# Multi-resolution-diffusion-recommender/SDRM

Measured on AMD Instinct MI355X. Metric: denoising-steps/sec (train+sample) on ML-1M latents, higher is better.
Workload: dtype f32; 1 GPU; ML-1M/MLP shaped synthetic latents (C3/C4); latent=340, width=340, hidden_layers=1, global_batch=8192, n_sample=5429, step_mix=15 train : 78 sample per job cycle, rng=philox4x32-10 on device, sampler_row_chains=2, parallelism=user-sharded dp1, collectives=none

## Files before the change

### include/sdrm_hip_debug.h

```cpp
#ifndef SDRM_HIP_DEBUG_H
#define SDRM_HIP_DEBUG_H

#include "sdrm_hip.h"

#ifdef __cplusplus
extern "C" {
#endif

int sdrm_debug_device_check(const char* gcn_arch, int compute_units);

enum { SDRM_TILE_AUTO = -1, SDRM_TILE_COUNT = 5 };

int sdrm_debug_set_tile(sdrm_engine* e, int cfg);
int sdrm_debug_set_nt32_rows(sdrm_engine* e, int max_rows, int max_rows_train);
int sdrm_debug_set_skinny(sdrm_engine* e, int on);
int sdrm_debug_set_rowchain(sdrm_engine* e, int mode);
int sdrm_debug_set_rows48(sdrm_engine* e, int mode);
int sdrm_debug_set_rows48_split(sdrm_engine* e, int mode);
int sdrm_debug_rows48_split_available(const sdrm_engine* e);
int sdrm_debug_set_rows48_share(sdrm_engine* e, int on);
int sdrm_debug_set_sample_persist(sdrm_engine* e, int mode);
int sdrm_debug_split_skew(sdrm_engine* e, unsigned skew);
int sdrm_debug_set_wgrad_strips(sdrm_engine* e, int on);
int sdrm_debug_set_dgrad_rows(sdrm_engine* e, int mode);
int sdrm_debug_rowchain_available(const sdrm_engine* e);
int sdrm_debug_set_fused_reverse(sdrm_engine* e, int mode);
int sdrm_debug_set_chains(sdrm_engine* e, int chains);
int sdrm_debug_chains(const sdrm_engine* e);

int sdrm_debug_set_gradient_buckets(sdrm_engine* e, int buckets);

int sdrm_debug_philox_draws(sdrm_engine* e, uint64_t seed, uint32_t purpose, uint32_t step, int64_t row0, int rows, int quads,
                            float* normals, uint8_t* lowbits, void* stream);

void* sdrm_debug_comm_handle(const sdrm_engine* e);

int sdrm_debug_plan_wgrad(int rows, int n_out, int k_in, int* slices, int* rows_per_slice);

int sdrm_debug_gemm(int variant, int cfg, const float* A, const float* B, float* C, int M, int N, int K, void* stream);
int sdrm_debug_gemm_time(int variant, int cfg, int M, int N, int K, int reps, float* us_out, void* stream);

#ifdef __cplusplus
}
#endif
#endif
```

### sdrm_amd/_lib.py

```python
from __future__ import annotations

import ctypes as C
import os

from . import _build

_LIB = None

c_void_p, c_int, c_int64, c_uint64, c_float = C.c_void_p, C.c_int, C.c_int64, C.c_uint64, C.c_float


class TrainRandoms(C.Structure):
    _fields_ = [("noise", c_void_p), ("t", c_void_p), ("keep", c_void_p)]


class VaeDecoder(C.Structure):
    _fields_ = [("w1", c_void_p), ("b1", c_void_p), ("w2", c_void_p), ("b2", c_void_p), ("latent", c_int), ("hidden", c_int),
                ("n_items", c_int)]


SIGNATURES = {
    "sdrm_create": (c_int, [c_int, c_int, c_int, c_int, c_int, c_int, C.POINTER(c_void_p)]),
    "sdrm_destroy": (c_int, [c_void_p]),
    "sdrm_last_error": (C.c_char_p, [c_void_p]),
    "sdrm_param_count": (c_int64, [c_void_p]),
    "sdrm_set_schedule": (c_int, [c_void_p, c_float, c_float]),
    "sdrm_get_schedule": (c_int, [c_void_p, c_void_p, c_void_p, c_void_p]),
    "sdrm_set_params": (c_int, [c_void_p, c_void_p, c_void_p]),
    "sdrm_get_params": (c_int, [c_void_p, c_void_p, c_void_p]),
    "sdrm_params_ptr": (c_void_p, [c_void_p]),
    "sdrm_get_grads": (c_int, [c_void_p, c_void_p, c_void_p]),
    "sdrm_get_adam_state": (c_int, [c_void_p, c_void_p, c_void_p, C.POINTER(c_int64), c_void_p]),
    "sdrm_set_adam_state": (c_int, [c_void_p, c_void_p, c_void_p, c_int64, c_void_p]),
    "sdrm_adam_reset": (c_int, [c_void_p, c_void_p]),
    "sdrm_train_forward": (c_int, [c_void_p, c_void_p, c_int, c_int64, c_int, C.POINTER(TrainRandoms), c_uint64,
                                   c_uint64, c_float, c_void_p, c_void_p]),
    "sdrm_train_backward": (c_int, [c_void_p, c_void_p, c_void_p, c_void_p, c_void_p]),
    "sdrm_train_backward_begin": (c_int, [c_void_p, c_void_p, c_void_p, c_void_p, c_void_p]),
    "sdrm_train_backward_finish": (c_int, [c_void_p, c_void_p, c_void_p]),
    "sdrm_grad_buckets": (c_int, [c_void_p, C.POINTER(c_int64), C.POINTER(c_int64), C.POINTER(c_int64), C.POINTER(c_int64)]),
    "sdrm_adam_step": (c_int, [c_void_p, c_void_p, c_float, c_void_p]),
    "sdrm_train_step": (c_int, [c_void_p, c_void_p, c_int, c_float, c_int, C.POINTER(TrainRandoms), c_uint64, c_uint64,
                                c_float, c_void_p, c_void_p]),
    "sdrm_comm_unique_id": (c_int, [c_void_p]),
    "sdrm_comm_available": (c_int, []),
    "sdrm_comm_init_rank": (c_int, [c_void_p, c_int, c_int, c_void_p]),
    "sdrm_allreduce_init": (c_int, [c_void_p, c_void_p, c_void_p]),
    "sdrm_comm_info": (c_int, [c_void_p, C.POINTER(c_int), C.POINTER(c_int)]),
    "sdrm_comm_destroy": (c_int, [c_void_p]),
    "sdrm_train_step_sharded": (c_int, [c_void_p, c_void_p, c_int, c_int64, c_float, c_int, C.POINTER(TrainRandoms), c_uint64,
                                        c_uint64, c_float, c_void_p, c_void_p]),
    "sdrm_get_train_outputs": (c_int, [c_void_p, c_void_p, c_void_p]),
    "sdrm_forward": (c_int, [c_void_p, c_void_p, c_void_p, c_int, c_int, c_void_p, c_uint64, c_uint64, c_int64,
                             c_void_p, c_void_p]),
    "sdrm_sample": (c_int, [c_void_p, c_int, c_float, c_int, c_int, c_void_p, c_void_p, c_void_p, c_void_p, c_uint64,
                            c_uint64, c_int64, c_void_p, c_void_p, c_void_p]),
    "sdrm_sample_begin": (c_int, [c_void_p, c_int, c_float, c_int, c_int, c_void_p, c_void_p, c_void_p, c_void_p,
                                  c_uint64, c_uint64, c_int64, c_void_p, c_void_p]),
    "sdrm_sample_steps": (c_int, [c_void_p, c_int, c_void_p]),
    "sdrm_sample_remaining": (c_int, [c_void_p]),
    "sdrm_sample_end": (c_int, [c_void_p, c_void_p, c_void_p]),
    "sdrm_reverse_step": (c_int, [c_void_p, c_void_p, c_int, c_int, c_void_p, c_void_p, c_void_p]),
    "sdrm_perturb_input": (c_int, [c_void_p, c_void_p, c_void_p, c_void_p, c_int, c_void_p, c_void_p]),
    "sdrm_get_preacts": (c_int, [c_void_p, c_int, c_void_p, c_void_p]),
    "sdrm_profile_begin": (c_int, [c_void_p, c_int]),
    "sdrm_debug_set_gradient_buckets": (c_int, [c_void_p, c_int]),
    "sdrm_profile_only": (c_int, [c_void_p, c_int]),
    "sdrm_profile_end": (c_int, [c_void_p, c_void_p]),
    "sdrm_profile_classes": (c_int, []),
    "sdrm_profile_name": (C.c_char_p, [c_int]),
    "sdrm_profile_get": (c_int, [c_void_p, c_int, C.POINTER(C.c_double), C.POINTER(c_int64), C.POINTER(C.c_double)]),
    "sdrm_launch_count": (c_int64, [c_void_p]),
    "sdrm_build_info": (C.c_char_p, []),
    "sdrm_csr_rows_to_dense": (c_int, [c_void_p, c_void_p, c_void_p, c_void_p, c_int64, c_void_p, c_int64, c_int, c_int, c_void_p, c_void_p]),
    "sdrm_feed_status": (c_int, [c_void_p, c_void_p]),
    "sdrm_vae_decode": (c_int, [c_void_p, C.POINTER(VaeDecoder), c_void_p, c_int, c_void_p, c_void_p]),
    "sdrm_equal_sparsity": (c_int, [c_void_p, c_void_p, c_int64, C.c_double, c_void_p, c_void_p, c_void_p]),
    "sdrm_rank_metrics": (c_int, [c_void_p, c_void_p, c_int, c_int, c_void_p, c_void_p, c_void_p, c_void_p, c_void_p, c_int,
                                  c_void_p, c_void_p, c_void_p, c_void_p, c_void_p]),
    "sdrm_source_hash": (C.c_char_p, []),
    "sdrm_debug_philox_draws": (c_int, [c_void_p, c_uint64, C.c_uint32, C.c_uint32, c_int64, c_int, c_int, c_void_p, c_void_p, c_void_p]),
    "sdrm_debug_device_check": (c_int, [C.c_char_p, c_int]),
    "sdrm_debug_set_tile": (c_int, [c_void_p, c_int]),
    "sdrm_debug_set_nt32_rows": (c_int, [c_void_p, c_int, c_int]),
    "sdrm_debug_set_chains": (c_int, [c_void_p, c_int]),
    "sdrm_debug_chains": (c_int, [c_void_p]),
    "sdrm_debug_set_fused_reverse": (c_int, [c_void_p, c_int]),
    "sdrm_debug_set_skinny": (c_int, [c_void_p, c_int]),
    "sdrm_debug_set_rowchain": (c_int, [c_void_p, c_int]),
    "sdrm_debug_set_rows48": (c_int, [c_void_p, c_int]),
    "sdrm_debug_set_rows48_split": (c_int, [c_void_p, c_int]),
    "sdrm_debug_rows48_split_available": (c_int, [c_void_p]),
    "sdrm_debug_split_skew": (c_int, [c_void_p, C.c_uint32]),
    "sdrm_debug_set_sample_persist": (c_int, [c_void_p, c_int]),
    "sdrm_debug_set_rows48_share": (c_int, [c_void_p, c_int]),
    "sdrm_debug_rowchain_available": (c_int, [c_void_p]),
    "sdrm_debug_set_wgrad_strips": (c_int, [c_void_p, c_int]),
    "sdrm_debug_set_dgrad_rows": (c_int, [c_void_p, c_int]),
    "sdrm_debug_comm_handle": (c_void_p, [c_void_p]),
    "sdrm_debug_plan_wgrad": (c_int, [c_int, c_int, c_int, C.POINTER(c_int), C.POINTER(c_int)]),
    "sdrm_debug_gemm_time": (c_int, [c_int, c_int, c_int, c_int, c_int, c_int, C.POINTER(c_float), c_void_p]),
    "sdrm_debug_gemm": (c_int, [c_int, c_int, c_void_p, c_void_p, c_void_p, c_int, c_int, c_int, c_void_p]),
}

RNG_EXPLICIT, RNG_PHILOX = 0, 1
STATUS = {0: "SDRM_OK", -1: "SDRM_ERR_ARG", -2: "SDRM_ERR_SHAPE", -3: "SDRM_ERR_HIP", -4: "SDRM_ERR_STATE",
          -5: "SDRM_ERR_NOMEM", -6: "SDRM_ERR_RCCL", -7: "SDRM_ERR_DEVICE"}


def lib_path() -> str:
    return _build.LIB_PATH


def load(build_if_missing: bool = True):
    global _LIB
    if _LIB is not None:
        return _LIB
    try:
        import torch
    except ImportError:
        pass
    path = lib_path()
    override = os.environ.get("SDRM_LIB")
    if override:
        lib = C.CDLL(os.path.abspath(override))
        missing = [name for name in SIGNATURES if not hasattr(lib, name)]
        if missing:
            raise RuntimeError(f"SDRM_LIB={override}: not this ABI, missing {', '.join(missing[:6])}{' ...' if len(missing) > 6 else ''}")
        for name, (res, args) in SIGNATURES.items():
            fn = getattr(lib, name)
            fn.restype, fn.argtypes = res, args
        import sys
        print(f"sdrm_amd: SDRM_LIB override {override} (sources {lib.sdrm_source_hash().decode()[:16]}; in-tree sources "
              f"{_build.source_hash()[:16]})", file=sys.stderr)
        _LIB = lib
        return lib
    if _build.is_stale():
        if not build_if_missing:
            what = "is missing" if not os.path.exists(path) else "was built from different sources than csrc/ + include/"
            raise RuntimeError(f"{path} {what}: run `python -c 'import __graft_entry__ as g; g.build()'`")
        _build.build_library()
    try:
        lib = C.CDLL(path)
    except OSError as exc:
        raise RuntimeError(f"cannot load {path}: {exc}") from exc
    for name, (res, args) in SIGNATURES.items():
        fn = getattr(lib, name)
        fn.restype, fn.argtypes = res, args
    got, want = lib.sdrm_source_hash().decode(), _build.source_hash()
    if got != want:
        raise RuntimeError(f"{path} carries source hash {got[:16]}, the sources hash to {want[:16]}")
    _LIB = lib
    return lib
```

### sdrm_amd/csrc/sdrm_hip.hip

```cpp
#include <hip/hip_runtime.h>

#include <algorithm>
#include <cmath>
#include <cstdio>
#include <cstdlib>
#include <cstring>
#include <mutex>
#include <set>
#include <string>
#include <vector>

#include "../../include/sdrm_hip.h"
#include "../../include/sdrm_hip_debug.h"
#include "decode.h"
#include "elementwise.h"
#include "exchange.h"
#include "feed.h"
#include "gemm.h"
#include "rank.h"
#include "rowchain.h"
#include "rows48.h"
#include "sample_persist.h"
#include "select.h"
#include "skinny.h"
#include "skinny_step.h"
#include "skinny_fwd4.h"
#include "tail.h"
#include "dgrad_rows.h"
#include "wgrad2.h"

using namespace sdrm;

namespace {

constexpr int BM = 64;
constexpr int S_MAX = 64;
constexpr int LOSS_BLOCKS = 256;

inline int round_up(int v, int m) { return (v + m - 1) / m * m; }

}

struct Tuning {
  int force_cfg = -1;
  int chains = -1;
  int detach = 1;
  int hold_early = 1;
  int fuse_rev = 1;
  int skinny = 1;
  int nt32_max_rows = 4096;
  int nt32_max_rows_train = 8192;
  int wgrad_blocks = 2816;
  int wgrad_round = 1280;
  int wgrad_slices = 0;
  int ar_buckets = 1;
  int dgrad_rows = 1;
  int strips = 1;
  int rows48 = 1;
  int rows48_share = 7;
  int smp_persist = 1;
  int split = 1;
  int rowchain = 1;
};

struct sdrm_engine {
  int L, W, T, H, max_rows, device;
  Tuning tune;
  int LP, WP, TP, K0, MPmax;
  int64_t P;
  int64_t off_we, off_be, off_w0, off_b0, off_a0, off_wh, off_bh, off_ah, off_wo, off_bo;
  float *p = nullptr, *m = nullptr, *v = nullptr, *g = nullptr;
  float *W0c = nullptr, *b0c = nullptr, *Whc = nullptr, *bhc = nullptr, *Woc = nullptr, *boc = nullptr;
  float *WhcT = nullptr, *WocT = nullptr;
  float *WhfT = nullptr, *WofT = nullptr;
  float *W0f = nullptr, *Whf = nullptr, *Wof = nullptr;
  bool cur_grouped = false;
  bool cur_sk = false;
  bool cur_g16 = false;
  int cur_rows = 0;
  bool cur_skip_pre = false;
  int cur_parts = 1;
  unsigned *xcntF = nullptr, *xcntC = nullptr;
  unsigned *xabort_host = nullptr, *xabort_dev = nullptr;
  uint32_t xepochF = 0, xepochC = 0;
  int xgeoF = 0, xgeoC = 0;
  bool xcd_ok = false;
  unsigned* xcntS = nullptr;
  uint32_t xphaseS = 0;
  unsigned xskew = 0;
  int cur_sk_np = 0;
  bool tables_fresh = false;
  float* act = nullptr;
  bool cur_act = false;
  int ones_col = -1;
  bool bwd_strips = false;
  float *temb = nullptr, *tembP = nullptr, *B0tab = nullptr;
  float *sched = nullptr;
  float *Us = nullptr;
  float *smp_pre = nullptr, *smp_Y = nullptr;
  float *U = nullptr, *pre = nullptr, *Y = nullptr, *dY = nullptr, *dA = nullptr, *X = nullptr;
  float *slab0 = nullptr, *slabH = nullptr, *slabO = nullptr, *db0s = nullptr, *dbHs = nullptr, *dbOs = nullptr;
  float *alpha_part = nullptr;
  int alpha_part_stride = 0;
  double *loss_part = nullptr, *sums = nullptr;
  float *WeP = nullptr, *W0eP = nullptr;
  int TPe = 0;
  float *Mred = nullptr, *snap = nullptr;
  int *tdev = nullptr;
  int64_t *Tj_dev = nullptr;
  int *rowid_dev = nullptr;
  const float* grad_src = nullptr;
  float *rev_dev = nullptr;
  SelectState* sel = nullptr;
  float* one_dev = nullptr;
  unsigned* feed_flag = nullptr;
  std::vector<int> smp_nact, smp_perm;
  std::vector<int64_t> smp_tj_sorted, smp_tj_orig;
  std::vector<float> h_beta, h_alpha, h_alphabar;
  int64_t adam_t = 0;
  int cur_B = 0, cur_MP = 0;
  const float* cur_x0 = nullptr;
  bool fwd_done = false;
  int last_S = 1, last_dgrad_blocks = 0;
  bool bwd_begun = false;
  bool fold_sums = false;
  int bwd_S0 = 1, bwd_SH = 1, bwd_SO = 1, bwd_kc0 = 0, bwd_kcH = 0, bwd_kcO = 0, bwd_dgrad_blocks = 0;
  int bwd_hidden_apps = 0;
  int bwd_cfg_w = 0;
  float* dec_buf[6] = {nullptr, nullptr, nullptr, nullptr, nullptr, nullptr};
  size_t dec_cap[6] = {0, 0, 0, 0, 0, 0};
  Exchange xch;
  mutable int64_t n_launches = 0;
  float* smp_w = nullptr;
  size_t smp_off[7] = {0, 0, 0, 0, 0, 0, 0};
  struct SampleStateT {
    bool active; int n, MP, multires, mode, i_next; float nd; const float* z; const uint8_t* keep;
    uint64_t seed, call_id; int64_t row0;
    const float* xT; bool skinny; bool skinny_launched; int i_start;
  } smp = {false, 0, 0, 0, 0, 0, 1.f, nullptr, nullptr, 0, 0, 0, nullptr, false, false, 0};
  hipStream_t aux[3] = {nullptr, nullptr, nullptr};
  hipEvent_t ev_fork = nullptr, ev_join[3] = {nullptr, nullptr, nullptr};
  hipEvent_t ev_hold = nullptr;
  int n_chains = 1, chain_chunk = 0;
  int n_aux = 0;
  bool detach_armed = false;
  bool hold_needed = false;
  bool chains_pending = false;
  bool hold_recorded = false;
  bool train_since_sample = false;
  bool prof_on = false;
  int prof_cap = 0;
  int prof_only = -1;
  std::vector<hipEvent_t> prof_ev;
  std::vector<int> prof_cls;
  std::vector<double> prof_flops;
  double prof_ms[16] = {0};
  double prof_fl[16] = {0};
  int64_t prof_n[16] = {0};
  std::string err;
};

typedef sdrm_engine::SampleStateT SampleState;

enum ProfClass { PC_FWD_L0 = 0, PC_FWD_HIDDEN, PC_FWD_OUT, PC_DGRAD, PC_WGRAD, PC_WGRAD_L0, PC_SMP_L0, PC_SMP_HIDDEN,
                 PC_SMP_OUT, PC_ROW_FWD, PC_WGRAD_STRIPS, PC_DGRAD_ROWS, PC_SMP_PERSIST, PC_COUNT };
static const char* kProfNames[PC_COUNT] = {
    "train: gemm_kernel<0,0,0,0,9> fwd layer0 (row-table bias)", "train: gemm_kernel<0,0,1,0,0> fwd hidden (prelu-in, bias)",
    "train: gemm_kernel<0,0,1,0,1> fwd out (prelu-in, tanh)",
    "train: gemm_kernel<0,0,0,0,3> dgrad (prelu' epilogue)",
    "train: gemm_batch_kernel<1,1,0,1,4> wgrad of all layers in one launch (prelu-in, split-K slabs)",
    "train: gemm_kernel<1,1,0,0,4> wgrad layer0 (split-K slabs)",
    "sample: gemm_kernel<0,0,0,0,10> fwd layer0 (bias table, prelu epilogue)", "sample: gemm_kernel<0,0,0,0,10> fwd hidden (bias, prelu epilogue)",
    "sample: gemm_kernel<0,0,0,0,1> fwd out (tanh)",
    "train: k_row_fwd row-owned forward (staging + all layers + loss partial sums, one work-group per CU)",
    "train: k_wgrad_strips weight gradients of all layers (strip-owned split-K, one work-group per CU)",
    "train: k_dgrad_chain / k_dgrad_rows input gradients (row-owned, prelu' epilogue, one work-group per CU; the chain: loss seeds + every layer in one launch)",
    "sample: k_sample_persist reverse steps without kernel boundaries (all layers + reverse update per step, row tiles synchronised through one XCD's L2)"};

namespace {

#define HIP_TRY(e, call)                                                                   \
  do {                                                                                     \
    hipError_t _st = (call);                                                               \
    if (_st != hipSuccess) {                                                               \
      (e)->err = std::string(#call) + ": " + hipGetErrorString(_st);                       \
      return SDRM_ERR_HIP;                                                                 \
    }                                                                                      \
  } while (0)

#define SDRM_LAUNCH(eng, ...)                      \
  do {                                             \
    if (eng) ++(eng)->n_launches;                  \
    hipLaunchKernelGGL(__VA_ARGS__);               \
  } while (0)

int fail(sdrm_engine* e, int code, const std::string& msg) {
  if (e) e->err = msg;
  return code;
}

constexpr size_t SLACK = 4096;

constexpr int LDS_MAX_BYTES = 160 * 1024;
hipError_t allow_full_lds(const void* kernel) {
  static std::mutex mu;
  static std::set<const void*> done;
  std::lock_guard<std::mutex> lock(mu);
  if (done.count(kernel)) return hipSuccess;
  const hipError_t st = hipFuncSetAttribute(kernel, hipFuncAttributeMaxDynamicSharedMemorySize, LDS_MAX_BYTES);
  if (st == hipSuccess) done.insert(kernel);
  return st;
}

template <typename Tp>
hipError_t dalloc(Tp** p, size_t n) {
  hipError_t st = hipMalloc((void**)p, (n + SLACK) * sizeof(Tp));
  if (st != hipSuccess) return st;
  return hipMemset(*p, 0, (n + SLACK) * sizeof(Tp));
}

float* pre_buf(sdrm_engine* e, int k) { return e->pre + (size_t)k * e->MPmax * e->WP; }
float* smp_buf(sdrm_engine* e, int k) { return e->smp_pre + (size_t)k * e->MPmax * e->WP; }
float* dpre_buf(sdrm_engine* e, int k) { return e->dA + (size_t)k * e->MPmax * e->WP; }
const float* slope_ptr(sdrm_engine* e, int layer) { return e->p + (layer == 0 ? e->off_a0 : e->off_ah); }

struct Prof { sdrm_engine* e; int cls; double flops; };

#ifdef SDRM_STAMPS
unsigned long long* g_wgrad_stamps = nullptr;
int g_wgrad_stamps_cap = 0, g_wgrad_stamps_n = 0;
int g_stamp_class = -1;
#endif


typedef TileCfg<64, 64, 2, 2, 4, 16> Cfg0;
typedef TileCfg<64, 64, 2, 2, 4, 32, 32, 1> Cfg1;
typedef TileCfg<64, 128, 2, 2, 4, 16> Cfg2;
typedef TileCfg<128, 128, 2, 2, 4, 16> Cfg3;
typedef TileCfg<32, 32, 2, 2, 4, 32, 16> Cfg4;
constexpr int N_TILE_CFGS = 5;
const int kCfgBM[N_TILE_CFGS] = {64, 64, 64, 128, 32};
const int kCfgBN[N_TILE_CFGS] = {64, 64, 128, 128, 32};
constexpr int FUSE_REV_MAX_ROWS = 4096;

int pick_cfg(const Tuning& t) { return (t.force_cfg >= 0 && t.force_cfg < N_TILE_CFGS) ? t.force_cfg : 0; }

int choose_cfg(const Tuning& t, int M, int nt32_rows) {
  if (t.force_cfg >= 0 && t.force_cfg < N_TILE_CFGS) return t.force_cfg;
  return M <= nt32_rows ? 4 : 0;
}

int max_gemm_blocks(int M, int N) {
  int best = 0;
  for (int c = 0; c < N_TILE_CFGS; ++c) {
    const int b = ((M + kCfgBM[c] - 1) / kCfgBM[c]) * ((N + kCfgBN[c] - 1) / kCfgBN[c]);
    if (b > best) best = b;
  }
  return best;
}

template <class Cfg, int LA, int LB, int XA, int XB, int EPI>
hipError_t launch_gemm_cfg(GemmArgs& a, int M, int N, int splits, hipStream_t st, Prof pr) {
  const int tiles_m = (M + Cfg::BM - 1) / Cfg::BM, tiles_n = (N + Cfg::BN - 1) / Cfg::BN;
  if (!gemm_set_grid(a, tiles_m, tiles_n, splits)) return hipErrorInvalidValue;
  {
    const uint64_t kc = (uint64_t)std::max(a.kchunk, 1) + 64;
    const uint64_t spanA = LA == LD_KCONTIG ? ((uint64_t)Cfg::BM * a.lda + kc) : kc * a.lda;
    const uint64_t spanB = LB == LD_KCONTIG ? ((uint64_t)Cfg::BN * a.ldb + kc) : kc * a.ldb;
    if (spanA * 4 >= (1ull << 32) || spanB * 4 >= (1ull << 32)) return hipErrorInvalidValue;
  }
  dim3 grid(EPI == EPI_SLAB ? (unsigned)(a.nblocks * splits) : (unsigned)a.nblocks, 1, 1);
  sdrm_engine* e = pr.e;
  const bool rec = e && e->prof_on && (int)e->prof_cls.size() < e->prof_cap && (e->prof_only < 0 || e->prof_only == pr.cls);
  size_t slot = 0;
  if (rec) {
    slot = e->prof_cls.size();
    e->prof_cls.push_back(pr.cls);
    e->prof_flops.push_back(pr.flops);
    hipError_t st0 = hipEventRecord(e->prof_ev[2 * slot], st);
    if (st0 != hipSuccess) return st0;
  }
#ifdef SDRM_STAMPS
  if (g_wgrad_stamps && g_stamp_class >= 0 && pr.e && pr.cls == g_stamp_class && (int)grid.x <= g_wgrad_stamps_cap) {
    a.stamps = g_wgrad_stamps;
    g_wgrad_stamps_n = (int)grid.x;
  }
#endif
  SDRM_LAUNCH(pr.e, (gemm_kernel<Cfg, LA, LB, XA, XB, EPI>), grid, dim3(NTHREADS), 0, st, a);
  hipError_t rc = hipGetLastError();
  if (rec && rc == hipSuccess) rc = hipEventRecord(e->prof_ev[2 * slot + 1], st);
  return rc;
}

template <int LA, int LB, int XA, int XB, int EPI>
hipError_t launch_gemm(GemmArgs& a, int M, int N, int splits, hipStream_t st, Prof pr, int cfg) {
  switch (cfg) {
    case 1: return launch_gemm_cfg<Cfg1, LA, LB, XA, XB, EPI>(a, M, N, splits, st, pr);
    case 2: return launch_gemm_cfg<Cfg2, LA, LB, XA, XB, EPI>(a, M, N, splits, st, pr);
    case 3: return launch_gemm_cfg<Cfg3, LA, LB, XA, XB, EPI>(a, M, N, splits, st, pr);
    case 4: return launch_gemm_cfg<Cfg4, LA, LB, XA, XB, EPI>(a, M, N, splits, st, pr);
    default: return launch_gemm_cfg<Cfg0, LA, LB, XA, XB, EPI>(a, M, N, splits, st, pr);
  }
}

template <int XA, int EPI>
hipError_t gemm_forward(GemmArgs a, const float* A, int lda, const float* Wc, int ldw, int M, int N, int K,
                        hipStream_t st, Prof pr, int cfg) {
  a.A = A; a.lda = lda; a.limA = M;
  a.B = Wc; a.ldb = ldw; a.limB = N;
  a.K = K; a.kchunk = K;
  return launch_gemm<LD_KCONTIG, LD_KCONTIG, XA, XF_NONE, EPI>(a, M, N, 1, st, pr, cfg);
}

hipError_t gemm_dgrad(sdrm_engine* e, const float* dC, int lddc, const float* WT, int ldwt, int M, int Nout, int Kin,
                      float* out, const float* aux, const float* slopeE, float* partial, hipStream_t st, double flops,
                      int cfg) {
  GemmArgs a{};
  a.A = dC; a.lda = lddc; a.limA = M;
  a.B = WT; a.ldb = ldwt; a.limB = Kin;
  a.C = out; a.ldc = e->WP;
  a.K = Nout; a.kchunk = Nout;
  a.aux = aux; a.ldaux = e->WP; a.slopeE = slopeE; a.slope_partial = partial;
  return launch_gemm<LD_KCONTIG, LD_KCONTIG, XF_NONE, XF_NONE, EPI_DPRELU>(a, M, Kin, 1, st, Prof{e, PC_DGRAD, flops}, cfg);
}

template <int XB>
hipError_t gemm_wgrad(const float* dC, int lddc, int Nout, const float* Act, int ldact, int Kin, const float* slopeB,
                      int Mrows, int S, int kchunk, float* slab, float* dbias, hipStream_t st, Prof pr, int cfg) {
  GemmArgs a{};
  a.A = dC; a.lda = lddc; a.limA = Nout;
  a.B = Act; a.ldb = ldact; a.limB = Kin;
  a.C = slab; a.ldc = Kin;
  a.K = Mrows; a.kchunk = kchunk;
  a.slopeB = slopeB;
  a.slab_stride = (size_t)Nout * Kin;
  a.dbias = dbias; a.dbias_stride = Nout;
  return launch_gemm<LD_MCONTIG, LD_MCONTIG, XF_NONE, XB, EPI_SLAB>(a, Nout, Kin, S, st, pr, cfg);
}

struct WgradSpec {
  const float* dC; int lddc, Nout; const float* Act; int ldact, Kin; const float* slopeB; int S, kchunk; float* slab; float* dbias;
};

hipError_t launch_wgrad_batch(sdrm_engine* e, const WgradSpec* w, int n, int Mrows, hipStream_t st, Prof pr, bool plain_b = false) {
  GemmBatch b{};
  b.n = n;
  int grid = 0;
  for (int k = 0; k < n; ++k) {
    GemmArgs& a = b.p[k];
    a.A = w[k].dC; a.lda = w[k].lddc; a.limA = w[k].Nout;
    a.B = w[k].Act; a.ldb = w[k].ldact; a.limB = w[k].Kin;
    a.C = w[k].slab; a.ldc = w[k].Kin;
    a.K = Mrows; a.kchunk = w[k].kchunk;
    a.slopeB = w[k].slopeB;
    a.slab_stride = (size_t)w[k].Nout * w[k].Kin;
    a.dbias = w[k].dbias; a.dbias_stride = w[k].Nout;
    const int tiles_m = (w[k].Nout + Cfg0::BM - 1) / Cfg0::BM, tiles_n = (w[k].Kin + Cfg0::BN - 1) / Cfg0::BN;
    if (!gemm_set_grid(a, tiles_m, tiles_n, w[k].S)) return hipErrorInvalidValue;
    if (((uint64_t)std::max(a.kchunk, 1) + 64) * (uint64_t)std::max(a.lda, a.ldb) * 4 >= (1ull << 32)) return hipErrorInvalidValue;
    b.start[k] = grid;
#ifdef SDRM_STAMPS
    a.stamps = (g_wgrad_stamps && g_stamp_class < 0) ? g_wgrad_stamps + 8 * (size_t)grid : nullptr;
#endif
    grid += round_up(a.nblocks * w[k].S, 8);
  }
  b.start[n] = grid;
#ifdef SDRM_STAMPS
  if (grid > g_wgrad_stamps_cap) for (int k = 0; k < n; ++k) b.p[k].stamps = nullptr;
  else if (g_stamp_class < 0) g_wgrad_stamps_n = grid;
#endif
  const bool rec = e->prof_on && (int)e->prof_cls.size() < e->prof_cap && (e->prof_only < 0 || e->prof_only == pr.cls);
  size_t slot = 0;
  if (rec) {
    slot = e->prof_cls.size();
    e->prof_cls.push_back(pr.cls);
    e->prof_flops.push_back(pr.flops);
    hipError_t st0 = hipEventRecord(e->prof_ev[2 * slot], st);
    if (st0 != hipSuccess) return st0;
  }
  if (plain_b)
    SDRM_LAUNCH(e, (gemm_batch_kernel<Cfg0, LD_MCONTIG, LD_MCONTIG, XF_NONE, XF_NONE, EPI_SLAB>), dim3((unsigned)grid),
                       dim3(NTHREADS), 0, st, b);
  else
    SDRM_LAUNCH(e, (gemm_batch_kernel<Cfg0, LD_MCONTIG, LD_MCONTIG, XF_NONE, XF_PRELU, EPI_SLAB>), dim3((unsigned)grid),
                       dim3(NTHREADS), 0, st, b);
  hipError_t rc = hipGetLastError();
  if (rec && rc == hipSuccess) rc = hipEventRecord(e->prof_ev[2 * slot + 1], st);
  return rc;
}

void pick_splits(const Tuning& tn, int Mrows, int tiles_total, int& S, int& kchunk) {
  const int BK = 32;
  int max_by_rows = Mrows / (4 * BK);
  if (max_by_rows < 1) max_by_rows = 1;
  const int tiles = tiles_total < 1 ? 1 : tiles_total;
  S = tn.wgrad_round / tiles;
  if (S < 8 || round_up((Mrows + S - 1) / S, BK) > 1024) S = tn.wgrad_blocks / tiles;
  if (S < 1) S = 1;
  if (tn.wgrad_slices > 0) S = tn.wgrad_slices;
  if (S > S_MAX) S = S_MAX;
  if (S > max_by_rows) S = max_by_rows;
  kchunk = round_up((Mrows + S - 1) / S, BK);
  S = (Mrows + kchunk - 1) / kchunk;
}

int wgrad_tiles(const Tuning& tn, int Nout, int Kin) {
  const int c = pick_cfg(tn);
  return ((Nout + kCfgBM[c] - 1) / kCfgBM[c]) * ((Kin + kCfgBN[c] - 1) / kCfgBN[c]);
}

void build_jobs(sdrm_engine* e, JobTable& tab) {
  const int L = e->L, W = e->W, T = e->T, H = e->H;
  int n = 0;
  auto add = [&](int64_t off, int rows, int cols, int flat_ld, int ncols, float* dst, int dst_ld, float* dstT = nullptr, int dstT_ld = 0) -> Job& {
    Job& j = tab.j[n++];
    j.flat_off = off; j.rows = rows; j.cols = cols; j.flat_ld = flat_ld; j.ncols = ncols;
    j.dst = dst; j.dst_ld = dst_ld; j.dstT = dstT; j.dstT_ld = dstT_ld; j.dst2 = nullptr; j.dst2_ld = 0;
    j.dstF = nullptr; j.dstFT = nullptr; j.fnct = e->WP / 16; j.fklast = -1; j.fklastT = -1;
    return j;
  };
  add(e->off_we, T, T, T, e->WeP ? T : 0, e->WeP, e->TPe);
  add(e->off_be, 1, T, T, 0, nullptr, 0);
  {
    Job& j = add(e->off_w0, W, L + T, L + T, L, e->W0c, e->K0);
    j.dstF = e->W0f; j.fklast = rc_light_klast(L, e->LP);
    j.dst2 = e->W0eP; j.dst2_ld = e->TPe;
  }
  add(e->off_b0, 1, W, W, W, e->b0c, 0);
  add(e->off_a0, 1, 1, 1, 1, nullptr, 0);
  if (H >= 1) {
    Job& j = add(e->off_wh, W, W, W, W, e->Whc, e->WP, e->WhcT, e->WP);
    j.dstF = e->Whf; j.dstFT = e->WhfT; j.fklast = j.fklastT = rc_light_klast(W, e->WP);
    add(e->off_bh, 1, W, W, W, e->bhc, 0);
    add(e->off_ah, 1, 1, 1, 1, nullptr, 0);
  }
  {
    Job& j = add(e->off_wo, L, W, W, W, e->Woc, e->WP, e->WocT, e->LP);
    j.dstF = e->Wof; j.dstFT = e->WofT; j.fklast = rc_light_klast(W, e->WP); j.fklastT = rc_light_klast(L, e->LP);
  }
  add(e->off_bo, 1, L, L, L, e->boc, 0);
  tab.n = n;
}

void adam_scalars(const sdrm_engine* e, float lr, float& step_size, float& bc2_sqrt) {
  const double k = (double)e->adam_t;
  const double bc1 = 1.0 - std::pow(0.9, k), bc2 = 1.0 - std::pow(0.999, k);
  step_size = (float)((double)lr / bc1);
  bc2_sqrt = (float)std::sqrt(bc2);
}

int launch_adam(sdrm_engine* e, const float* grad, float lr, int update, hipStream_t st) {
  JobTable tab;
  build_jobs(e, tab);
  AdamArgs a{};
  a.p = e->p; a.m = e->m; a.v = e->v; a.g = grad ? grad : e->g;
  a.b1 = 0.9f; a.b2 = 0.999f; a.eps = 1e-8f; a.wd = 1e-4f; a.update = update;
  if (update) adam_scalars(e, lr, a.step_size, a.bc2_sqrt);
  int64_t biggest = 0;
  for (int k = 0; k < tab.n; ++k) biggest = std::max<int64_t>(biggest, (int64_t)tab.j[k].rows * tab.j[k].cols);
  const int gx = (int)std::min<int64_t>(1024, std::max<int64_t>(1, (biggest + 511) / 512));
  dim3 grid(gx, tab.n);
  SDRM_LAUNCH(e, k_adam, grid, dim3(256), 0, st, tab, a);
  HIP_TRY(e, hipGetLastError());
  e->tables_fresh = false;
  return SDRM_OK;
}

bool use_strips(const sdrm_engine* e) {
  return (e->cur_grouped || e->cur_g16) && e->cur_act && e->ones_col >= 0 && e->tune.strips > 0 && e->H + 2 <= WG2_MAX_PROBLEMS && e->WP >= 128 && e->WP <= 352;
}

template <int NT>
int launch_wgrad_strips_nt(sdrm_engine* e, const Wg2Args& a, double flops, hipStream_t st) {
  const bool rec = e->prof_on && (int)e->prof_cls.size() < e->prof_cap && (e->prof_only < 0 || e->prof_only == PC_WGRAD_STRIPS);
  size_t slot = 0;
  if (rec) {
    slot = e->prof_cls.size();
    e->prof_cls.push_back(PC_WGRAD_STRIPS);
    e->prof_flops.push_back(flops);
    HIP_TRY(e, hipEventRecord(e->prof_ev[2 * slot], st));
  }
  SDRM_LAUNCH(e, (k_wgrad_strips<NT>), dim3((unsigned)(a.units * a.slices)), dim3(NTHREADS), 0, st, a);
  HIP_TRY(e, hipGetLastError());
  if (rec) HIP_TRY(e, hipEventRecord(e->prof_ev[2 * slot + 1], st));
  return SDRM_OK;
}

int launch_wgrad_strips(sdrm_engine* e, int MP, double flops, hipStream_t st) {
  const int H = e->H;
  Wg2Args a{};
  int ktiles[WG2_MAX_PROBLEMS], n = 0;
  auto problem = [&](const float* A, int lda, const float* B, int ldb, float* slab, int kin, size_t slab_rows) {
    a.p[n].A = A; a.p[n].lda = lda; a.p[n].B = B; a.p[n].ldb = ldb; a.p[n].slab = slab; a.p[n].ldc = kin;
    a.p[n].slab_stride = slab_rows * (size_t)kin;
    ktiles[n++] = kin / 32;
  };
  auto actk = [&](int k) { return e->act + (size_t)k * e->MPmax * e->WP; };
  problem(dpre_buf(e, 0), e->WP, e->U, e->K0, e->slab0, e->K0, (size_t)e->WP);
  problem(e->dY, e->LP, actk(H), e->WP, e->slabO, e->WP, (size_t)e->LP);
  const int units = [&] { int t = e->K0 / 32 + (H + 1) * (e->WP / 32); return (t + 3) / 4; }();
  int S = 256 / units;
  if (S < 1) S = 1;
  if (S > S_MAX) S = S_MAX;
  MP = e->cur_rows;
  const int kchunk = round_up((MP + S - 1) / S, WG2_BK);
  const int slices = (MP + kchunk - 1) / kchunk;
  for (int k = H; k >= 1; --k)
    problem(dpre_buf(e, k), e->WP, actk(k - 1), e->WP, e->slabH + (size_t)(k - 1) * slices * e->WP * e->WP, e->WP, (size_t)e->WP);
  if (wg2_plan(ktiles, n, a) != units) return fail(e, SDRM_ERR_SHAPE, "strip-owned weight gradients: plan does not fit");
  a.slices = slices; a.rows = MP; a.kchunk = kchunk;
  e->bwd_S0 = e->bwd_SH = e->bwd_SO = slices;
  e->bwd_strips = true;
  switch (e->WP / 32) {
    case 4: return launch_wgrad_strips_nt<4>(e, a, flops, st);
    case 5: return launch_wgrad_strips_nt<5>(e, a, flops, st);
    case 6: return launch_wgrad_strips_nt<6>(e, a, flops, st);
    case 7: return launch_wgrad_strips_nt<7>(e, a, flops, st);
    case 8: return launch_wgrad_strips_nt<8>(e, a, flops, st);
    case 9: return launch_wgrad_strips_nt<9>(e, a, flops, st);
    case 10: return launch_wgrad_strips_nt<10>(e, a, flops, st);
    default: return launch_wgrad_strips_nt<11>(e, a, flops, st);
  }
}

EmbTabArgs emb_args(sdrm_engine* e) {
  EmbTabArgs a{};
  a.temb = e->temb; a.We = e->p + e->off_we; a.be = e->p + e->off_be; a.W0 = e->p + e->off_w0; a.b0 = e->p + e->off_b0;
  a.W0c = e->W0c; a.B0tab = e->B0tab;
  a.L = e->L; a.W = e->W; a.T = e->T; a.LP = e->LP; a.WP = e->WP; a.K0 = e->K0;
  a.ones_col = e->ones_col;
  return a;
}

int emb_tables(sdrm_engine* e, hipStream_t st, const float* warm = nullptr, size_t warm_floats = 0) {
  EmbTabArgs a = emb_args(e);
  a.warm = warm; a.warm_lines = warm ? (unsigned)std::min<size_t>(warm_floats / 32, 1u << 24) : 0u;
  SDRM_LAUNCH(e, k_emb_tables, dim3(e->T + 1), dim3(1024), 2 * e->T * sizeof(float), st, a);
  HIP_TRY(e, hipGetLastError());
  e->tables_fresh = true;
  return SDRM_OK;
}
int ensure_tables(sdrm_engine* e, hipStream_t st) { return e->tables_fresh ? SDRM_OK : emb_tables(e, st); }

bool skinny_net(const sdrm_engine* e) { return e->tune.skinny && e->LP <= 64 && e->WP <= 64; }

bool row_dgrads_follow(const sdrm_engine* e, bool g16, int MP) {
  if (!e->WhfT || e->tune.dgrad_rows <= 0 || e->LP != e->WP || e->WP < 128 || e->WP > 352) return false;
  return g16 ? e->H + 1 <= DR_MAX_LAYERS : MP % RC_ROWS == 0;
}
bool use_dgrad_rows(const sdrm_engine* e, int MP) {
  return e->cur_grouped && e->WhfT && e->tune.dgrad_rows > 0 && e->LP == e->WP && MP % RC_ROWS == 0 && e->WP >= 128 && e->WP <= 352;
}

template <int CT>
int launch_dgrad_rows_ct(sdrm_engine* e, const DgradRowsArgs& a, int G, double flops, hipStream_t st) {
  const bool rec = e->prof_on && (int)e->prof_cls.size() < e->prof_cap && (e->prof_only < 0 || e->prof_only == PC_DGRAD_ROWS);
  size_t slot = 0;
  if (rec) {
    slot = e->prof_cls.size();
    e->prof_cls.push_back(PC_DGRAD_ROWS);
    e->prof_flops.push_back(flops);
    HIP_TRY(e, hipEventRecord(e->prof_ev[2 * slot], st));
  }
  if (rc_light_klast(e->W, e->WP) >= 0) SDRM_LAUNCH(e, (k_dgrad_rows<CT, true>), dim3((unsigned)G), dim3(NTHREADS), 0, st, a);
  else SDRM_LAUNCH(e, (k_dgrad_rows<CT, false>), dim3((unsigned)G), dim3(NTHREADS), 0, st, a);
  HIP_TRY(e, hipGetLastError());
  if (rec) HIP_TRY(e, hipEventRecord(e->prof_ev[2 * slot + 1], st));
  return SDRM_OK;
}

DgradRowsArgs dgrad_rows_args(const sdrm_engine* e, const float* G, const float* WfT, const float* pre, const float* slope, float* out,
                              float* partial) {
  DgradRowsArgs a{};
  a.G = G; a.ldg = e->WP; a.WfT = WfT; a.pre = pre; a.ldp = e->WP; a.slope = slope; a.out = out; a.ldo = e->WP; a.slope_part = partial;
  a.act = e->act ? e->act + (pre - e->pre) : nullptr; a.from_act = (e->cur_act && e->cur_skip_pre && a.act) ? 1 : 0;
  return a;
}

int launch_dgrad_rows(sdrm_engine* e, const float* G, const float* WfT, const float* pre, const float* slope, float* out, float* partial,
                      int MP, double flops, hipStream_t st) {
  const DgradRowsArgs a = dgrad_rows_args(e, G, WfT, pre, slope, out, partial);
  const int Gn = MP / RC_ROWS;
  switch (e->WP / 32) {
    case 4: return launch_dgrad_rows_ct<4>(e, a, Gn, flops, st);
    case 5: return launch_dgrad_rows_ct<5>(e, a, Gn, flops, st);
    case 6: return launch_dgrad_rows_ct<6>(e, a, Gn, flops, st);
    case 7: return launch_dgrad_rows_ct<7>(e, a, Gn, flops, st);
    case 8: return launch_dgrad_rows_ct<8>(e, a, Gn, flops, st);
    case 9: return launch_dgrad_rows_ct<9>(e, a, Gn, flops, st);
    case 10: return launch_dgrad_rows_ct<10>(e, a, Gn, flops, st);
    default: return launch_dgrad_rows_ct<11>(e, a, Gn, flops, st);
  }
}

template <int CT>
int launch_dgrad_chain_ct(sdrm_engine* e, const DgradChainArgs& a, int G, double flops, hipStream_t st) {
  const bool rec = e->prof_on && (int)e->prof_cls.size() < e->prof_cap && (e->prof_only < 0 || e->prof_only == PC_DGRAD_ROWS);
  size_t slot = 0;
  if (rec) {
    slot = e->prof_cls.size();
    e->prof_cls.push_back(PC_DGRAD_ROWS);
    e->prof_flops.push_back(flops);
    HIP_TRY(e, hipEventRecord(e->prof_ev[2 * slot], st));
  }
  if (rc_light_klast(e->W, e->WP) >= 0) SDRM_LAUNCH(e, (k_dgrad_chain<CT, true>), dim3((unsigned)G), dim3(NTHREADS), 0, st, a);
  else SDRM_LAUNCH(e, (k_dgrad_chain<CT, false>), dim3((unsigned)G), dim3(NTHREADS), 0, st, a);
  HIP_TRY(e, hipGetLastError());
  if (rec) HIP_TRY(e, hipEventRecord(e->prof_ev[2 * slot + 1], st));
  return SDRM_OK;
}

int launch_dgrad_chain(sdrm_engine* e, const DgradChainArgs& a, int MP, double flops, hipStream_t st) {
  const int Gn = MP / RC_ROWS;
  switch (e->WP / 32) {
    case 4: return launch_dgrad_chain_ct<4>(e, a, Gn, flops, st);
    case 5: return launch_dgrad_chain_ct<5>(e, a, Gn, flops, st);
    case 6: return launch_dgrad_chain_ct<6>(e, a, Gn, flops, st);
    case 7: return launch_dgrad_chain_ct<7>(e, a, Gn, flops, st);
    case 8: return launch_dgrad_chain_ct<8>(e, a, Gn, flops, st);
    case 9: return launch_dgrad_chain_ct<9>(e, a, Gn, flops, st);
    case 10: return launch_dgrad_chain_ct<10>(e, a, Gn, flops, st);
    default: return launch_dgrad_chain_ct<11>(e, a, Gn, flops, st);
  }
}

bool use_rowchain(const sdrm_engine* e, int B) {
  if (!e->W0f || e->tune.rowchain <= 0 || e->tune.force_cfg >= 0) return false;
  if (e->tune.rowchain >= 2) return true;
  const int G = (B + RC_USERS - 1) / RC_USERS;
  const int rounds = (G + 255) / 256;
  return rounds == 1 ? G >= 154 : G * 6 >= rounds * 256 * 5;
}

inline unsigned xabort_read(const sdrm_engine* e) { return e->xabort_host ? *(volatile const unsigned*)e->xabort_host : 0u; }

int rows48_grid(int groups, int parts) { return parts == 1 ? groups : 8 * parts * ((groups + 7) / 8); }
int rows48_parts(const sdrm_engine* e, int B) {
  if (!e->W0f || e->tune.rows48 <= 0 || e->tune.force_cfg >= 0 || e->tune.rowchain >= 2) return 0;
  const int G = (B + R48_USERS - 1) / R48_USERS;
  const bool can_split = e->xcd_ok && e->tune.split > 0 && e->xabort_host && xabort_read(e) == 0u;
  if (can_split && e->tune.split >= 2) {
    const int parts = e->tune.split >= 4 ? 4 : 2;
    if (rows48_grid(G, parts) <= 256) return parts;
    if (parts == 4 && rows48_grid(G, 2) <= 256) return 2;
  }
  if (e->tune.rows48 >= 2) return 1;
  const bool beside_sampler = e->smp.active && (e->detach_armed || (e->chains_pending && e->n_aux == e->n_chains));
  if (can_split && e->tune.split == 1 && G > 80 && rows48_grid(G, 2) <= 256) return beside_sampler ? 0 : 2;
  return (G >= 160 && G <= 256) ? 1 : 0;
}

int split_sync(sdrm_engine* e, bool chain, int groups, int parts, int phases, hipStream_t st, unsigned** cnt, unsigned* base) {
  unsigned*& c = chain ? e->xcntC : e->xcntF;
  uint32_t& epoch = chain ? e->xepochC : e->xepochF;
  int& geo = chain ? e->xgeoC : e->xgeoF;
  const int now = (parts << 16) | groups | (phases << 24);
  if (geo != now || epoch >= 0x7fffffffu / (uint32_t)(phases * parts + 1)) {
    HIP_TRY(e, hipMemsetAsync(c, 0, (size_t)256 * 32 * sizeof(unsigned), st));
    epoch = 0; geo = now;
  }
  *cnt = c;
  *base = epoch * (uint32_t)(phases * parts) + e->xskew;
  if (e->xskew) { e->xskew = 0; geo = 0; }
  ++epoch;
  return SDRM_OK;
}

int split_status(sdrm_engine* e) {
  if (xabort_read(e) == 0u) return SDRM_OK;
  *(volatile unsigned*)e->xabort_host = 0u;
  e->xgeoF = e->xgeoC = 0;
  e->tune.split = 0;
  e->fwd_done = false;
  return fail(e, SDRM_ERR_HIP, "a column-split row-group launch (csrc/rows48.h) timed out waiting for a work-group of its group: the results of "
                               "that train step are invalid; the path is switched off for this handle");
}

template <int CT, int PARTS>
int launch_rows48_forward_ctp(sdrm_engine* e, const RowChainArgs& a, int grid, hipStream_t st) {
  if constexpr (PARTS == 1 && CT % 2 == 1) {
    if (e->tune.rows48_share & 1) {
      if (a.light) SDRM_LAUNCH(e, (k_rows48_fwd<CT, true, 1, true>), dim3((unsigned)grid), dim3(NTHREADS), 0, st, a);
      else SDRM_LAUNCH(e, (k_rows48_fwd<CT, false, 1, true>), dim3((unsigned)grid), dim3(NTHREADS), 0, st, a);
      return SDRM_OK;
    }
  }
  if (a.light) SDRM_LAUNCH(e, (k_rows48_fwd<CT, true, PARTS>), dim3((unsigned)grid), dim3(NTHREADS), 0, st, a);
  else SDRM_LAUNCH(e, (k_rows48_fwd<CT, false, PARTS>), dim3((unsigned)grid), dim3(NTHREADS), 0, st, a);
  return SDRM_OK;
}

template <int CT>
int launch_rows48_forward_ct(sdrm_engine* e, RowChainArgs& a, int G, int parts, hipStream_t st) {
  const double flops = 2.0 * 3 * a.B * ((double)e->W * e->L + (double)e->H * e->W * e->W + (double)e->L * e->W);
  const bool rec = e->prof_on && (int)e->prof_cls.size() < e->prof_cap && (e->prof_only < 0 || e->prof_only == PC_ROW_FWD);
  size_t slot = 0;
  if (parts > 1) {
    if (int rc = split_sync(e, false, G, parts, e->H + 1, st, &a.xcnt, &a.xbase)) return rc;
    a.xabort = e->xabort_dev; a.ngroups = G;
  }
  if (rec) {
    slot = e->prof_cls.size();
    e->prof_cls.push_back(PC_ROW_FWD);
    e->prof_flops.push_back(flops);
    HIP_TRY(e, hipEventRecord(e->prof_ev[2 * slot], st));
  }
  const int grid = rows48_grid(G, parts);
  if (parts == 4) launch_rows48_forward_ctp<CT, 4>(e, a, grid, st);
  else if (parts == 2) launch_rows48_forward_ctp<CT, 2>(e, a, grid, st);
  else launch_rows48_forward_ctp<CT, 1>(e, a, grid, st);
  HIP_TRY(e, hipGetLastError());
  if (rec) HIP_TRY(e, hipEventRecord(e->prof_ev[2 * slot + 1], st));
  return SDRM_OK;
}

template <int CT, int PARTS>
int launch_rows48_chain_ctp(sdrm_engine* e, const DgradChain48Args& a, int grid, hipStream_t st) {
  if constexpr (PARTS == 1 && CT % 2 == 1) {
    if (e->tune.rows48_share & 2) {
      if (rc_light_klast(e->W, e->WP) >= 0) SDRM_LAUNCH(e, (k_rows48_dgrad_chain<CT, true, 1, true>), dim3((unsigned)grid), dim3(NTHREADS), 0, st, a);
      else SDRM_LAUNCH(e, (k_rows48_dgrad_chain<CT, false, 1, true>), dim3((unsigned)grid), dim3(NTHREADS), 0, st, a);
      return SDRM_OK;
    }
  }
  if (rc_light_klast(e->W, e->WP) >= 0) SDRM_LAUNCH(e, (k_rows48_dgrad_chain<CT, true, PARTS>), dim3((unsigned)grid), dim3(NTHREADS), 0, st, a);
  else SDRM_LAUNCH(e, (k_rows48_dgrad_chain<CT, false, PARTS>), dim3((unsigned)grid), dim3(NTHREADS), 0, st, a);
  return SDRM_OK;
}

template <int CT>
int launch_rows48_chain_ct(sdrm_engine* e, DgradChain48Args& a, int G, int parts, double flops, hipStream_t st) {
  const bool rec = e->prof_on && (int)e->prof_cls.size() < e->prof_cap && (e->prof_only < 0 || e->prof_only == PC_DGRAD_ROWS);
  size_t slot = 0;
  if (parts > 1) {
    if (int rc = split_sync(e, true, G, parts, std::max(1, a.c.nlayers - 1), st, &a.xcnt, &a.xbase)) return rc;
    a.xabort = e->xabort_dev; a.ngroups = G;
  }
  if (rec) {
    slot = e->prof_cls.size();
    e->prof_cls.push_back(PC_DGRAD_ROWS);
    e->prof_flops.push_back(flops);
    HIP_TRY(e, hipEventRecord(e->prof_ev[2 * slot], st));
  }
  const int grid = rows48_grid(G, parts);
  if (parts == 4) launch_rows48_chain_ctp<CT, 4>(e, a, grid, st);
  else if (parts == 2) launch_rows48_chain_ctp<CT, 2>(e, a, grid, st);
  else launch_rows48_chain_ctp<CT, 1>(e, a, grid, st);
  HIP_TRY(e, hipGetLastError());
  if (rec) HIP_TRY(e, hipEventRecord(e->prof_ev[2 * slot + 1], st));
  return SDRM_OK;
}

int launch_rows48_chain(sdrm_engine* e, DgradChain48Args& a, int G, int parts, double flops, hipStream_t st) {
  switch (e->WP / 32) {
    case 4: return launch_rows48_chain_ct<4>(e, a, G, parts, flops, st);
    case 5: return launch_rows48_chain_ct<5>(e, a, G, parts, flops, st);
    case 6: return launch_rows48_chain_ct<6>(e, a, G, parts, flops, st);
    case 7: return launch_rows48_chain_ct<7>(e, a, G, parts, flops, st);
    case 8: return launch_rows48_chain_ct<8>(e, a, G, parts, flops, st);
    case 9: return launch_rows48_chain_ct<9>(e, a, G, parts, flops, st);
    case 10: return launch_rows48_chain_ct<10>(e, a, G, parts, flops, st);
    default: return launch_rows48_chain_ct<11>(e, a, G, parts, flops, st);
  }
}

template <int CT>
int launch_row_forward_ct(sdrm_engine* e, const RowChainArgs& a, int G, hipStream_t st) {
  const double flops = 2.0 * 3 * a.B * ((double)e->W * e->L + (double)e->H * e->W * e->W + (double)e->L * e->W);
  const bool rec = e->prof_on && (int)e->prof_cls.size() < e->prof_cap && (e->prof_only < 0 || e->prof_only == PC_ROW_FWD);
  size_t slot = 0;
  if (rec) {
    slot = e->prof_cls.size();
    e->prof_cls.push_back(PC_ROW_FWD);
    e->prof_flops.push_back(flops);
    HIP_TRY(e, hipEventRecord(e->prof_ev[2 * slot], st));
  }
  if (a.light) SDRM_LAUNCH(e, (k_row_fwd<CT, true>), dim3((unsigned)G), dim3(NTHREADS), 0, st, a);
  else SDRM_LAUNCH(e, (k_row_fwd<CT, false>), dim3((unsigned)G), dim3(NTHREADS), 0, st, a);
  HIP_TRY(e, hipGetLastError());
  if (rec) HIP_TRY(e, hipEventRecord(e->prof_ev[2 * slot + 1], st));
  return SDRM_OK;
}

int launch_row_forward(sdrm_engine* e, const float* x0, int B, int64_t row0, int mode, const sdrm_train_randoms* rnd, uint64_t seed,
                       uint64_t step, float nd, int G, hipStream_t st, int rows48_parts_ = 0) {
  const int n = e->T + 1;
  RowChainArgs a{};
  a.x0 = x0;
  if (mode == SDRM_RNG_EXPLICIT) { a.noise = rnd->noise; a.t = rnd->t; a.keep = rnd->keep; }
  a.sqrt_ab = e->sched + 3 * n; a.one_minus_ab = e->sched + 4 * n; a.tembP = e->tembP;
  a.B = B; a.L = e->L; a.T = e->T; a.H = e->H;
  a.mode = mode; a.seed_lo = (uint32_t)seed; a.seed_hi = (uint32_t)(seed >> 32); a.step = (uint32_t)step; a.row0 = row0; a.nd = nd;
  a.W0f = e->W0f; a.Whf = e->Whf; a.Wof = e->Wof; a.bh = e->bhc; a.bo = e->boc; a.B0tab = e->B0tab; a.ldtab = e->WP;
  a.slope0 = slope_ptr(e, 0); a.slopeh = e->H > 0 ? slope_ptr(e, 1) : slope_ptr(e, 0);
  a.U = e->U; a.K0 = e->K0; a.LPs = e->LP; a.tdev = e->tdev; a.ones_col = e->ones_col;
  a.light = rc_light_klast(e->W, e->WP) >= 0 ? 1 : 0;
  a.pre = e->pre; a.pre_stride = (size_t)e->MPmax * e->WP; a.ldp = e->WP; a.Y = e->Y; a.ldy = e->LP;
  a.act = e->act;
  a.loss_part = e->loss_part;
  a.sweep = (e->tune.rows48_share & 4) ? 1 : 0;
  {
    const int MPg = rows48_parts_ > 0 ? round_up(G * R48_ROWS, BM) : round_up(G * RC_ROWS, BM);
    a.skip_pre = row_dgrads_follow(e, rows48_parts_ > 0, MPg) ? 1 : 0;
    e->cur_skip_pre = a.skip_pre != 0;
  }
  if (rows48_parts_ > 0) {
    switch (e->WP / 32) {
      case 4: return launch_rows48_forward_ct<4>(e, a, G, rows48_parts_, st);
      case 5: return launch_rows48_forward_ct<5>(e, a, G, rows48_parts_, st);
      case 6: return launch_rows48_forward_ct<6>(e, a, G, rows48_parts_, st);
      case 7: return launch_rows48_forward_ct<7>(e, a, G, rows48_parts_, st);
      case 8: return launch_rows48_forward_ct<8>(e, a, G, rows48_parts_, st);
      case 9: return launch_rows48_forward_ct<9>(e, a, G, rows48_parts_, st);
      case 10: return launch_rows48_forward_ct<10>(e, a, G, rows48_parts_, st);
      case 11: return launch_rows48_forward_ct<11>(e, a, G, rows48_parts_, st);
      default: return fail(e, SDRM_ERR_SHAPE, "row-owned forward: padded width outside 128..352");
    }
  }
  switch (e->WP / 32) {
    case 4: return launch_row_forward_ct<4>(e, a, G, st);
    case 5: return launch_row_forward_ct<5>(e, a, G, st);
    case 6: return launch_row_forward_ct<6>(e, a, G, st);
    case 7: return launch_row_forward_ct<7>(e, a, G, st);
    case 8: return launch_row_forward_ct<8>(e, a, G, st);
    case 9: return launch_row_forward_ct<9>(e, a, G, st);
    case 10: return launch_row_forward_ct<10>(e, a, G, st);
    case 11: return launch_row_forward_ct<11>(e, a, G, st);
    default: return fail(e, SDRM_ERR_SHAPE, "row-owned forward: padded width outside 128..352");
  }
}

SkStepArgs sk_step_args(sdrm_engine* e, int B) {
  SkStepArgs a{};
  const int n = e->T + 1;
  a.W0c = e->W0c; a.K0 = e->K0; a.Whc = e->Whc; a.Woc = e->Woc; a.bh = e->bhc; a.bo = e->boc;
  a.WhcT = e->WhcT; a.WocT = e->WocT; a.B0tab = e->B0tab;
  a.WeP = e->WeP; a.W0eP = e->W0eP; a.be = e->p + e->off_be; a.b0 = e->b0c; a.TPe = e->TPe; a.intab = e->WeP ? 1 : 0;
  a.slope0 = slope_ptr(e, 0); a.slopeh = e->H > 0 ? slope_ptr(e, 1) : slope_ptr(e, 0);
  a.sqrt_ab = e->sched + 3 * n; a.one_minus_ab = e->sched + 4 * n; a.tembP = e->tembP;
  a.B = B; a.L = e->L; a.W = e->W; a.T = e->T; a.H = e->H; a.G = (B + SK_USERS - 1) / SK_USERS;
  a.LPs = e->LP; a.WPs = e->WP; a.TPs = e->TP;
  a.U = e->U; a.tdev = e->tdev; a.pre = e->pre; a.pre_stride = (size_t)e->MPmax * e->WP; a.Y = e->Y;
  a.loss_part = e->loss_part; a.NP = a.G;
  a.slab0 = e->slab0; a.slabH = e->slabH; a.slabO = e->slabO; a.db0s = e->db0s; a.dbHs = e->dbHs; a.dbOs = e->dbOs;
  a.alpha_part = e->alpha_part; a.alpha_part_stride = e->alpha_part_stride;
  return a;
}

template <int NL, int NW>
int launch_sk_step_nlnw(sdrm_engine* e, const SkStepArgs& ka, int which, int grid, hipStream_t st) {
  typedef SkCfg<NL, NW> C;
  const size_t lds = (which == 0 ? sk_fwd_lds_floats<NL, NW>(ka.intab ? ka.TPe : 0) : sk_bwd_lds_floats<NL, NW>(ka.TPs)) * sizeof(float);
  if (lds > 48 * 1024) HIP_TRY(e, allow_full_lds(which == 0 ? (const void*)k_skinny_fwd<NL, NW> : (const void*)k_skinny_bwd<NL, NW>));
  if (which == 0) SDRM_LAUNCH(e, (k_skinny_fwd<NL, NW>), dim3((unsigned)grid), dim3(C::NTHR), lds, st, ka);
  else SDRM_LAUNCH(e, (k_skinny_bwd<NL, NW>), dim3((unsigned)grid), dim3(C::NTHR), lds, st, ka);
  HIP_TRY(e, hipGetLastError());
  return SDRM_OK;
}

template <int NL, int NW>
int launch_sk_fwd4_nlnw(sdrm_engine* e, const SkStepArgs& ka, hipStream_t st, bool* done) {
  const size_t lds = sk4_fwd_lds_floats<NL, NW>(ka.intab ? ka.TPe : 0) * sizeof(float);
  *done = false;
  if (lds > 160 * 1024) return SDRM_OK;
  if (lds > 48 * 1024) HIP_TRY(e, allow_full_lds((const void*)k_skinny_fwd4<NL, NW>));
  SDRM_LAUNCH(e, (k_skinny_fwd4<NL, NW>), dim3((unsigned)std::min(ka.NP, 8192)), dim3(SK4_THREADS), lds, st, ka);
  HIP_TRY(e, hipGetLastError());
  *done = true;
  return SDRM_OK;
}

int launch_sk_fwd4(sdrm_engine* e, const SkStepArgs& ka, hipStream_t st, bool* done) {
  const int NL = (e->L + 15) / 16, NW = (e->W + 15) / 16;
#define SK4_ROW(nl)                                                           \
  switch (NW) {                                                               \
    case 1: return launch_sk_fwd4_nlnw<nl, 1>(e, ka, st, done);               \
    case 2: return launch_sk_fwd4_nlnw<nl, 2>(e, ka, st, done);               \
    case 3: return launch_sk_fwd4_nlnw<nl, 3>(e, ka, st, done);               \
    default: return launch_sk_fwd4_nlnw<nl, 4>(e, ka, st, done);              \
  }
  switch (NL) {
    case 1: SK4_ROW(1)
    case 2: SK4_ROW(2)
    case 3: SK4_ROW(3)
    default: SK4_ROW(4)
  }
#undef SK4_ROW
}

int launch_sk_step(sdrm_engine* e, const SkStepArgs& ka, int which, int grid, hipStream_t st) {
  const int NL = (e->L + 15) / 16, NW = (e->W + 15) / 16;
#define SK_ROW(nl)                                                                  \
  switch (NW) {                                                                     \
    case 1: return launch_sk_step_nlnw<nl, 1>(e, ka, which, grid, st);              \
    case 2: return launch_sk_step_nlnw<nl, 2>(e, ka, which, grid, st);              \
    case 3: return launch_sk_step_nlnw<nl, 3>(e, ka, which, grid, st);              \
    default: return launch_sk_step_nlnw<nl, 4>(e, ka, which, grid, st);             \
  }
  switch (NL) {
    case 1: SK_ROW(1)
    case 2: SK_ROW(2)
    case 3: SK_ROW(3)
    default: SK_ROW(4)
  }
#undef SK_ROW
}

struct NetView { const float *W0c, *Whc, *Woc, *bhc, *boc, *B0tab, *slope0, *slopeh; };
NetView snapshot_view(const sdrm_engine* e) {
  const float* b = e->smp_w;
  return NetView{b + e->smp_off[0], b + e->smp_off[1], b + e->smp_off[2], b + e->smp_off[3], b + e->smp_off[4], b + e->smp_off[5],
                 b + e->smp_off[6], b + e->smp_off[6] + 1};
}

int hidden_forward(sdrm_engine* e, int MP, int rows, hipStream_t st, int cfg, int r0 = 0, int cls = PC_FWD_HIDDEN,
                   bool post_act = false, const NetView* nv = nullptr) {
  const double fl = 2.0 * rows * (double)e->W * e->W;
  const size_t ro = (size_t)r0 * e->WP;
  for (int k = 1; k <= e->H; ++k) {
    if (post_act) {
      GemmArgs a{};
      a.C = (nv ? smp_buf(e, k) : pre_buf(e, k)) + ro; a.ldc = e->WP; a.bias = nv ? nv->bhc : e->bhc; a.slopeE = nv ? nv->slopeh : slope_ptr(e, k);
      HIP_TRY(e, (gemm_forward<XF_NONE, EPI_BIAS_PRELU>(a, (nv ? smp_buf(e, k - 1) : pre_buf(e, k - 1)) + ro, e->WP, nv ? nv->Whc : e->Whc, e->WP, MP, e->WP, e->WP,
                                                         st, Prof{e, cls, fl}, cfg)));
      continue;
    }
    GemmArgs a{};
    a.C = pre_buf(e, k) + ro; a.ldc = e->WP; a.bias = e->bhc; a.slopeA = slope_ptr(e, k - 1);
    HIP_TRY(e, (gemm_forward<XF_PRELU, EPI_BIAS>(a, pre_buf(e, k - 1) + ro, e->WP, e->Whc, e->WP, MP, e->WP, e->WP, st,
                                                 Prof{e, cls, fl}, cfg)));
  }
  return SDRM_OK;
}

int join_chains(sdrm_engine* e, hipStream_t st) {
  e->bwd_begun = false;
  if (!e->chains_pending) return SDRM_OK;
  for (int c = 0; c < e->n_aux; ++c) {
    HIP_TRY(e, hipEventRecord(e->ev_join[c], e->aux[c]));
    HIP_TRY(e, hipStreamWaitEvent(st, e->ev_join[c], 0));
  }
  e->chains_pending = false;
  return SDRM_OK;
}

int hold_chains(sdrm_engine* e, hipStream_t st) {
  if (!e->chains_pending) return SDRM_OK;
  if (e->hold_recorded) {
    for (int c = 0; c < e->n_aux; ++c) HIP_TRY(e, hipStreamWaitEvent(e->aux[c], e->ev_hold, 0));
    e->hold_recorded = false;
    return SDRM_OK;
  }
  HIP_TRY(e, hipEventRecord(e->ev_fork, st));
  for (int c = 0; c < e->n_aux; ++c) HIP_TRY(e, hipStreamWaitEvent(e->aux[c], e->ev_fork, 0));
  return SDRM_OK;
}
int hold_point(sdrm_engine* e, hipStream_t st) {
  if (!e->chains_pending || !e->tune.hold_early || !e->hold_needed) return SDRM_OK;
  HIP_TRY(e, hipEventRecord(e->ev_hold, st));
  e->hold_recorded = true;
  return SDRM_OK;
}

int chains_for(const Tuning& t, int n, int WP) {
  if (t.chains >= 1) return t.chains > 4 ? 4 : t.chains;
  return (size_t)n * (size_t)WP >= (size_t)2560 * 352 ? 2 : 1;
}

int upload_schedule(sdrm_engine* e, float beta1, float beta2) {
  const int T = e->T, n = T + 1;
  std::vector<float> b(n), al(n), ab(n), sq(n), om(n);
  const float step = 1.0f / (float)T;
  float run = 0.f;
  for (int i = 0; i < n; ++i) {
    const float lin = (i < n / 2) ? (0.f + step * (float)i) : (1.f - step * (float)(n - 1 - i));
    b[i] = (beta2 - beta1) * lin + beta1;
    al[i] = 1.f - b[i];
    run += std::log(al[i]);
    ab[i] = std::exp(run);
  }
  ab[0] = 1.f;
  for (int i = 0; i < n; ++i) { sq[i] = std::sqrt(ab[i]); om[i] = 1.f - ab[i]; }
  e->h_beta = b; e->h_alpha = al; e->h_alphabar = ab;
  HIP_TRY(e, hipMemcpy(e->sched + 0 * n, b.data(), n * 4, hipMemcpyHostToDevice));
  HIP_TRY(e, hipMemcpy(e->sched + 1 * n, al.data(), n * 4, hipMemcpyHostToDevice));
  HIP_TRY(e, hipMemcpy(e->sched + 2 * n, ab.data(), n * 4, hipMemcpyHostToDevice));
  HIP_TRY(e, hipMemcpy(e->sched + 3 * n, sq.data(), n * 4, hipMemcpyHostToDevice));
  HIP_TRY(e, hipMemcpy(e->sched + 4 * n, om.data(), n * 4, hipMemcpyHostToDevice));
  if (e->rev_dev) {
    std::vector<float> rev(3 * (size_t)n, 0.f);
    for (int i = 1; i < n; ++i) {
      rev[i] = (1.f - al[i]) / std::sqrt(1.f - ab[i]);
      rev[n + i] = std::sqrt(al[i]);
      rev[2 * n + i] = std::sqrt(b[i]);
    }
    HIP_TRY(e, hipMemcpy(e->rev_dev, rev.data(), rev.size() * 4, hipMemcpyHostToDevice));
  }
  return SDRM_OK;
}

int upload_temb(sdrm_engine* e) {
  const int T = e->T, half = T / 2;
  std::vector<float> tab((size_t)(T + 1) * T, 0.f), freqs(half);
  const float nl = -(float)std::log(10000.0);
  for (int k = 0; k < half; ++k) freqs[k] = std::exp(nl * (float)k / (float)half);
  for (int t = 0; t <= T; ++t)
    for (int k = 0; k < half; ++k) {
      const float arg = (float)t * freqs[k];
      tab[(size_t)t * T + k] = std::cos(arg);
      tab[(size_t)t * T + half + k] = std::sin(arg);
    }
  HIP_TRY(e, hipMemcpy(e->temb, tab.data(), tab.size() * 4, hipMemcpyHostToDevice));
  HIP_TRY(e, hipMemcpy2D(e->tembP, (size_t)e->TP * 4, tab.data(), (size_t)T * 4, (size_t)T * 4, (size_t)(T + 1), hipMemcpyHostToDevice));
  return SDRM_OK;
}

void reverse_coeffs(const sdrm_engine* e, int i, float& c1, float& sa, float& sb) {
  const float a = e->h_alpha[i], ab = e->h_alphabar[i], b = e->h_beta[i];
  c1 = (1.f - a) / std::sqrt(1.f - ab);
  sa = std::sqrt(a);
  sb = std::sqrt(b);
}

}

extern "C" {

int sdrm_debug_set_rowchain(sdrm_engine* e, int mode) {
  if (!e) return SDRM_ERR_ARG;
  if (e->bwd_begun) return fail(e, SDRM_ERR_STATE, "sdrm_debug_set_rowchain: a two-call backward is in progress");
  e->fwd_done = false;
  e->tune.rowchain = mode < 0 ? 0 : (mode > 2 ? 2 : mode);
  return SDRM_OK;
}

int sdrm_debug_set_rows48(sdrm_engine* e, int mode) {
  if (!e) return SDRM_ERR_ARG;
  if (e->bwd_begun) return fail(e, SDRM_ERR_STATE, "sdrm_debug_set_rows48: between sdrm_train_backward_begin and _finish");
  e->fwd_done = false;
  e->tune.rows48 = mode < 0 ? 0 : (mode > 2 ? 2 : mode);
  return SDRM_OK;
}

int sdrm_debug_set_rows48_split(sdrm_engine* e, int mode) {
  if (!e) return SDRM_ERR_ARG;
  if (e->bwd_begun) return fail(e, SDRM_ERR_STATE, "sdrm_debug_set_rows48_split: between sdrm_train_backward_begin and _finish");
  if (mode != 0 && mode != 1 && mode != 2 && mode != 4) return fail(e, SDRM_ERR_ARG, "sdrm_debug_set_rows48_split: 0, 1, 2 or 4");
  e->fwd_done = false;
  e->tune.split = mode;
  return SDRM_OK;
}

int sdrm_debug_rows48_split_available(const sdrm_engine* e) { return e && e->W0f && e->xcd_ok ? 1 : 0; }

int sdrm_debug_set_rows48_share(sdrm_engine* e, int on) {
  if (!e) return SDRM_ERR_ARG;
  e->tune.rows48_share = on == 1 ? 7 : (on == 2 ? 5 : (on == 3 ? 2 : 0));
  return SDRM_OK;
}

int sdrm_debug_set_sample_persist(sdrm_engine* e, int mode) {
  if (!e) return SDRM_ERR_ARG;
  if (e->smp.active) return fail(e, SDRM_ERR_STATE, "sdrm_debug_set_sample_persist: inside a sampling call");
  e->tune.smp_persist = mode < 0 ? 0 : (mode > 2 ? 2 : mode);
  return SDRM_OK;
}

int sdrm_debug_split_skew(sdrm_engine* e, unsigned skew) {
  if (!e) return SDRM_ERR_ARG;
  e->xskew = skew;
  return SDRM_OK;
}

int sdrm_debug_rowchain_available(const sdrm_engine* e) { return e && e->W0f ? 1 : 0; }

int sdrm_debug_set_wgrad_strips(sdrm_engine* e, int on) {
  if (!e) return SDRM_ERR_ARG;
  e->tune.strips = on ? 1 : 0;
  return SDRM_OK;
}

int sdrm_debug_set_dgrad_rows(sdrm_engine* e, int on) {
  if (!e) return SDRM_ERR_ARG;
  e->fwd_done = false;
  e->tune.dgrad_rows = on < 0 ? 0 : (on > 2 ? 2 : on);
  return SDRM_OK;
}

int sdrm_debug_set_skinny(sdrm_engine* e, int on) {
  if (!e) return SDRM_ERR_ARG;
  e->tune.skinny = on < 0 ? 0 : (on > 2 ? 2 : on);
  return SDRM_OK;
}

int sdrm_debug_plan_wgrad(int rows, int n_out, int k_in, int* slices, int* rows_per_slice) {
  if (!slices || !rows_per_slice || rows < 1 || n_out < 1 || k_in < 1) return SDRM_ERR_ARG;
  pick_splits(Tuning{}, rows, wgrad_tiles(Tuning{}, n_out, k_in), *slices, *rows_per_slice);
  return SDRM_OK;
}

int sdrm_debug_philox_draws(sdrm_engine* e, uint64_t seed, uint32_t purpose, uint32_t step, int64_t row0, int rows, int quads,
                            float* normals, uint8_t* lowbits, void* stream) {
  if (!e || !normals || rows < 1 || quads < 1) return fail(e, SDRM_ERR_ARG, "sdrm_debug_philox_draws: bad argument");
  const size_t total = (size_t)rows * quads;
  SDRM_LAUNCH(e, k_philox_draws, dim3((unsigned)std::min<size_t>(8192, (total + 255) / 256)), dim3(256), 0, (hipStream_t)stream,
              (uint32_t)seed, (uint32_t)(seed >> 32), purpose, step, row0, rows, quads, normals, lowbits);
  HIP_TRY(e, hipGetLastError());
  return SDRM_OK;
}

int sdrm_debug_set_fused_reverse(sdrm_engine* e, int mode) {
  if (!e) return SDRM_ERR_ARG;
  e->tune.fuse_rev = mode < 0 ? 0 : (mode > 2 ? 2 : mode);
  return SDRM_OK;
}

int sdrm_debug_set_gradient_buckets(sdrm_engine* e, int buckets) {
  if (!e || (buckets != 1 && buckets != 2)) return SDRM_ERR_ARG;
  e->tune.ar_buckets = buckets;
  return SDRM_OK;
}

int sdrm_debug_set_chains(sdrm_engine* e, int chains) {
  if (!e) return SDRM_ERR_ARG;
  e->tune.chains = chains;
  return SDRM_OK;
}

int sdrm_debug_chains(const sdrm_engine* e) { return e ? e->n_chains : 0; }

int sdrm_debug_set_tile(sdrm_engine* e, int cfg) {
  if (!e) return SDRM_ERR_ARG;
  if (e->bwd_begun || e->smp.active)
    return fail(e, SDRM_ERR_STATE, "sdrm_debug_set_tile: a two-call backward or a sampling call is in progress");
  e->fwd_done = false;
  e->tune.force_cfg = cfg;
  return SDRM_OK;
}

int sdrm_debug_set_nt32_rows(sdrm_engine* e, int max_rows, int max_rows_train) {
  if (!e) return SDRM_ERR_ARG;
  if (max_rows >= 0) e->tune.nt32_max_rows = max_rows;
  if (max_rows_train >= 0) e->tune.nt32_max_rows_train = max_rows_train;
  return SDRM_OK;
}

#ifndef SDRM_SOURCE_HASH
#define SDRM_SOURCE_HASH "unhashed"
#endif
static const char kSourceHashMarker[] = "SDRM_SOURCE_HASH=" SDRM_SOURCE_HASH;
const char* sdrm_source_hash(void) { return kSourceHashMarker + sizeof("SDRM_SOURCE_HASH=") - 1; }

const char* sdrm_build_info(void) {
  return "gfx950 fp32 v_mfma_f32_32x32x2_f32; block tile 64x64x16 (32x32x32 on v_mfma_f32_16x16x4_f32 for NT launches of at "
         "most 4096 rows, 8192 stacked rows in the train step), 4 waves, two LDS stages + register-double-buffered fragments, "
         "pipeline pieces in the MFMA shadows, k-minor LDS + ds_read_b128 for NT; split-K slabs for wgrad; persistent "
         "LDS-resident kernels for widths <= 64; one-round grids sized for 256 compute units in 8 XCDs (sdrm_create refuses any "
         "other device); sources " SDRM_SOURCE_HASH;
}

const char* sdrm_last_error(const sdrm_engine* e) { return e ? e->err.c_str() : "null engine"; }

constexpr int SDRM_TARGET_CUS = 256;
int sdrm_debug_device_check(const char* gcn_arch, int compute_units) {
  if (!gcn_arch) return SDRM_ERR_ARG;
  if (std::strncmp(gcn_arch, "gfx950", 6) != 0 || (gcn_arch[6] != '\0' && gcn_arch[6] != ':')) return SDRM_ERR_DEVICE;
  return compute_units == SDRM_TARGET_CUS ? SDRM_OK : SDRM_ERR_DEVICE;
}
int64_t sdrm_param_count(const sdrm_engine* e) { return e ? e->P : -1; }

int sdrm_create(int L, int W, int T, int H, int max_rows, int device_id, sdrm_engine** out) {
  if (!out) return SDRM_ERR_ARG;
  *out = nullptr;
  if (L < 1 || L > 4096 || W < 1 || W > 4096 || T < 2 || T > 1024 || H < 0 || H > 16 || max_rows < 1 ||
      max_rows > (1 << 22))
    return SDRM_ERR_SHAPE;
  if (tail_emb_lds_floats(T, round_up(T + 1, 32)) * sizeof(float) > 160 * 1024) return SDRM_ERR_SHAPE;
  sdrm_engine* e = new sdrm_engine();
  if (const char* env = std::getenv("SDRM_TILE")) e->tune.force_cfg = std::atoi(env);
  if (const char* env = std::getenv("SDRM_CHAINS")) e->tune.chains = std::atoi(env);
  if (const char* env = std::getenv("SDRM_HOLD_EARLY")) e->tune.hold_early = std::atoi(env);
  if (const char* env = std::getenv("SDRM_DETACH")) e->tune.detach = std::atoi(env);
  if (const char* env = std::getenv("SDRM_FUSE_REV")) e->tune.fuse_rev = std::atoi(env);
  if (const char* env = std::getenv("SDRM_NT32_MAX_ROWS")) e->tune.nt32_max_rows = std::atoi(env);
  if (const char* env = std::getenv("SDRM_NT32_MAX_ROWS_TRAIN")) e->tune.nt32_max_rows_train = std::atoi(env);
  if (const char* env = std::getenv("SDRM_WGRAD_BLOCKS")) e->tune.wgrad_blocks = std::max(1, std::atoi(env));
  if (const char* env = std::getenv("SDRM_WGRAD_ROUND")) e->tune.wgrad_round = std::max(1, std::atoi(env));
  if (const char* env = std::getenv("SDRM_AR_BUCKETS")) e->tune.ar_buckets = std::atoi(env);
  if (const char* env = std::getenv("SDRM_WGRAD_SLICES")) e->tune.wgrad_slices = std::min(S_MAX, std::max(0, std::atoi(env)));
  if (const char* env = std::getenv("SDRM_ROWCHAIN")) e->tune.rowchain = std::atoi(env);
  if (const char* env = std::getenv("SDRM_ROWS48")) e->tune.rows48 = std::atoi(env);
  if (const char* env = std::getenv("SDRM_ROWS48_SPLIT")) e->tune.split = std::atoi(env);
  if (const char* env = std::getenv("SDRM_SAMPLE_PERSIST")) e->tune.smp_persist = std::atoi(env);
  if (const char* env = std::getenv("SDRM_ROWS48_SHARE")) e->tune.rows48_share = std::atoi(env);
  if (const char* env = std::getenv("SDRM_WGRAD_STRIPS")) e->tune.strips = std::atoi(env);
  if (const char* env = std::getenv("SDRM_DGRAD_ROWS")) e->tune.dgrad_rows = std::atoi(env);
  e->L = L; e->W = W; e->T = T; e->H = H; e->max_rows = max_rows; e->device = device_id;
  e->LP = round_up(L, 32); e->WP = round_up(W, 32); e->TP = round_up(T + 1, 32); e->K0 = e->LP + e->TP;
  e->MPmax = round_up(RC_ROWS * ((max_rows + RC_USERS - 1) / RC_USERS), 128);
  int64_t o = 0;
  e->off_we = o; o += (int64_t)T * T;
  e->off_be = o; o += T;
  e->off_w0 = o; o += (int64_t)W * (L + T);
  e->off_b0 = o; o += W;
  e->off_a0 = o; o += 1;
  if (H >= 1) {
    e->off_wh = o; o += (int64_t)W * W;
    e->off_bh = o; o += W;
    e->off_ah = o; o += 1;
  } else {
    e->off_wh = e->off_bh = e->off_ah = -1;
  }
  e->off_wo = o; o += (int64_t)L * W;
  e->off_bo = o; o += L;
  e->P = o;
  *out = e;
  HIP_TRY(e, hipSetDevice(device_id));
  {
    hipDeviceProp_t prop;
    HIP_TRY(e, hipGetDeviceProperties(&prop, device_id));
    const char* any = std::getenv("SDRM_ALLOW_ANY_DEVICE");
    const bool lifted = any && std::atoi(any) != 0;
    if (sdrm_debug_device_check(prop.gcnArchName, lifted ? SDRM_TARGET_CUS : prop.multiProcessorCount) != SDRM_OK)
      return fail(e, SDRM_ERR_DEVICE, std::string("sdrm_create: device ") + std::to_string(device_id) + " is " + prop.gcnArchName + " with " +
                                          std::to_string(prop.multiProcessorCount) + " compute units; this library is built for gfx950 with " +
                                          std::to_string(SDRM_TARGET_CUS) + " (MI355X, SPX mode): its one-round grids and XCD mapping assume them");
  }
  const size_t MP = e->MPmax;
  const int n = T + 1;
  HIP_TRY(e, dalloc(&e->p, e->P)); HIP_TRY(e, dalloc(&e->m, e->P));
  HIP_TRY(e, dalloc(&e->v, e->P)); HIP_TRY(e, dalloc(&e->g, e->P));
  HIP_TRY(e, dalloc(&e->W0c, (size_t)round_up(e->WP, 128) * e->K0)); HIP_TRY(e, dalloc(&e->b0c, e->WP));
  HIP_TRY(e, dalloc(&e->Whc, (size_t)round_up(e->WP, 128) * e->WP)); HIP_TRY(e, dalloc(&e->bhc, e->WP));
  HIP_TRY(e, dalloc(&e->Woc, (size_t)round_up(e->LP, 128) * e->WP)); HIP_TRY(e, dalloc(&e->boc, e->LP));
  HIP_TRY(e, dalloc(&e->WhcT, (size_t)round_up(e->WP, 128) * e->WP)); HIP_TRY(e, dalloc(&e->WocT, (size_t)round_up(e->WP, 128) * e->LP));
  if (L == W && e->WP >= 128 && e->WP <= 352) {
    HIP_TRY(e, dalloc(&e->W0f, (size_t)e->WP * e->WP)); HIP_TRY(e, dalloc(&e->Whf, (size_t)e->WP * e->WP));
    HIP_TRY(e, dalloc(&e->Wof, (size_t)e->WP * e->WP));
    HIP_TRY(e, dalloc(&e->WhfT, (size_t)e->WP * e->WP)); HIP_TRY(e, dalloc(&e->WofT, (size_t)e->WP * e->WP));
    HIP_TRY(e, dalloc(&e->act, (size_t)(H + 1) * e->MPmax * e->WP));
    if (round_up(W, 4) < e->WP) e->ones_col = round_up(W, 4);
  }
  HIP_TRY(e, dalloc(&e->temb, (size_t)n * T)); HIP_TRY(e, dalloc(&e->tembP, (size_t)n * e->TP));
  HIP_TRY(e, dalloc(&e->B0tab, (size_t)n * e->WP)); HIP_TRY(e, dalloc(&e->sched, (size_t)8 * n));
  HIP_TRY(e, dalloc(&e->rev_dev, (size_t)3 * n));
  {
    const size_t sz[7] = {(size_t)round_up(e->WP, 128) * e->K0, (size_t)round_up(e->WP, 128) * e->WP, (size_t)round_up(e->LP, 128) * e->WP,
                          (size_t)e->WP, (size_t)e->LP, (size_t)n * e->WP, 4};
    size_t tot = 0;
    for (int k = 0; k < 7; ++k) { e->smp_off[k] = tot; tot += (sz[k] + 63) / 64 * 64; }
    HIP_TRY(e, dalloc(&e->smp_w, tot));
  }
  HIP_TRY(e, dalloc(&e->sel, 1));
  HIP_TRY(e, dalloc(&e->one_dev, 4));
  HIP_TRY(e, dalloc(&e->feed_flag, 4));
  if (e->W0f) {
    HIP_TRY(e, dalloc(&e->xcntF, (size_t)256 * 32)); HIP_TRY(e, dalloc(&e->xcntC, (size_t)256 * 32));
    HIP_TRY(e, dalloc(&e->xcntS, (size_t)256 * 32));
    HIP_TRY(e, hipHostMalloc((void**)&e->xabort_host, sizeof(unsigned), hipHostMallocMapped));
    *e->xabort_host = 0u;
    HIP_TRY(e, hipHostGetDevicePointer((void**)&e->xabort_dev, e->xabort_host, 0));
    unsigned* probe = nullptr;
    constexpr int NPROBE = 512;
    HIP_TRY(e, dalloc(&probe, NPROBE));
    hipLaunchKernelGGL(k_xcc_probe, dim3(NPROBE), dim3(64), 0, 0, probe);
    std::vector<unsigned> xcc(NPROBE);
    HIP_TRY(e, hipMemcpy(xcc.data(), probe, NPROBE * sizeof(unsigned), hipMemcpyDeviceToHost));
    HIP_TRY(e, hipFree(probe));
    bool ok = true;
    std::set<unsigned> ids;
    for (int b = 0; b < NPROBE; ++b) ok = ok && (xcc[b] & 0xfu) == (xcc[b & 7] & 0xfu);
    for (int x = 0; x < 8; ++x) ids.insert(xcc[x] & 0xfu);
    e->xcd_ok = ok && ids.size() == 8;
  }
  {
    const float one = 1.0f;
    HIP_TRY(e, hipMemcpy(e->one_dev, &one, 4, hipMemcpyHostToDevice));
    if (e->ones_col >= 0) HIP_TRY(e, hipMemcpy(e->bhc + e->ones_col, &one, 4, hipMemcpyHostToDevice));
  }
  HIP_TRY(e, dalloc(&e->U, MP * e->K0)); HIP_TRY(e, dalloc(&e->pre, (size_t)(H + 1) * MP * e->WP));
  HIP_TRY(e, dalloc(&e->Y, MP * e->LP)); HIP_TRY(e, dalloc(&e->dY, MP * e->LP));
  HIP_TRY(e, dalloc(&e->dA, (size_t)(H + 1) * MP * e->WP));
  HIP_TRY(e, dalloc(&e->X, MP * e->LP)); HIP_TRY(e, dalloc(&e->Us, MP * e->LP));
  HIP_TRY(e, dalloc(&e->smp_pre, (size_t)(H + 1) * MP * e->WP)); HIP_TRY(e, dalloc(&e->smp_Y, MP * e->LP));
  HIP_TRY(e, dalloc(&e->slab0, (size_t)S_MAX * e->WP * e->K0)); HIP_TRY(e, dalloc(&e->db0s, (size_t)S_MAX * e->WP));
  HIP_TRY(e, dalloc(&e->slabO, (size_t)S_MAX * e->LP * e->WP)); HIP_TRY(e, dalloc(&e->dbOs, (size_t)S_MAX * e->LP));
  if (H >= 1) {
    HIP_TRY(e, dalloc(&e->slabH, (size_t)H * S_MAX * e->WP * e->WP));
    HIP_TRY(e, dalloc(&e->dbHs, (size_t)H * S_MAX * e->WP));
  }
  e->alpha_part_stride = std::max(max_gemm_blocks((int)MP, e->WP), (int)MP / 16);
  HIP_TRY(e, dalloc(&e->alpha_part, (size_t)(H + 1) * e->alpha_part_stride));
  HIP_TRY(e, dalloc(&e->loss_part, (size_t)4 * std::max<size_t>(LOSS_BLOCKS, 4 * (MP / SK_ROWS + 1)))); HIP_TRY(e, dalloc(&e->sums, 8));
  if (e->LP <= 64 && e->WP <= 64 && T <= 128) {
    e->TPe = round_up(T, 16);
    HIP_TRY(e, dalloc(&e->WeP, (size_t)e->TPe * e->TPe)); HIP_TRY(e, dalloc(&e->W0eP, (size_t)e->WP * e->TPe));
  }
  HIP_TRY(e, dalloc(&e->Mred, (size_t)W * e->TP)); HIP_TRY(e, dalloc(&e->snap, (size_t)T * T + T + (size_t)W * T));
  HIP_TRY(e, allow_full_lds((const void*)k_tail_emb));
  HIP_TRY(e, dalloc(&e->tdev, max_rows)); HIP_TRY(e, dalloc(&e->Tj_dev, max_rows)); HIP_TRY(e, dalloc(&e->rowid_dev, max_rows));
  HIP_TRY(e, hipEventCreateWithFlags(&e->ev_fork, hipEventDisableTiming));
  HIP_TRY(e, hipEventCreateWithFlags(&e->ev_hold, hipEventDisableTiming));
  for (int c = 0; c < 3; ++c) {
    HIP_TRY(e, hipStreamCreateWithFlags(&e->aux[c], hipStreamNonBlocking));
    HIP_TRY(e, hipEventCreateWithFlags(&e->ev_join[c], hipEventDisableTiming));
  }
  int rc = upload_schedule(e, 1e-4f, 0.02f);
  if (rc) return rc;
  rc = upload_temb(e);
  if (rc) return rc;
  HIP_TRY(e, hipDeviceSynchronize());
  return SDRM_OK;
}

int sdrm_destroy(sdrm_engine* e) {
  if (!e) return SDRM_ERR_ARG;
  (void)hipSetDevice(e->device);
  void* bufs[] = {e->p, e->m, e->v, e->g, e->W0c, e->b0c, e->Whc, e->bhc, e->Woc, e->boc, e->temb, e->tembP, e->B0tab,
                  e->sched, e->U, e->pre, e->Y, e->dY, e->dA, e->X, e->slab0, e->slabH, e->slabO, e->db0s,
                  e->dbHs, e->dbOs, e->alpha_part, e->loss_part, e->sums, e->Mred, e->snap, e->WeP, e->W0eP, e->tdev, e->Tj_dev, e->rowid_dev, e->rev_dev, e->Us, e->WhcT, e->WocT, e->sel, e->one_dev, e->feed_flag, e->smp_w, e->W0f, e->Whf, e->Wof, e->act, e->WhfT, e->WofT, e->smp_pre, e->smp_Y};
  for (void* b : bufs)
    if (b) (void)hipFree(b);
  if (e->xcntF) (void)hipFree(e->xcntF);
  if (e->xcntC) (void)hipFree(e->xcntC);
  if (e->xcntS) (void)hipFree(e->xcntS);
  for (hipEvent_t ev : e->prof_ev) (void)hipEventDestroy(ev);
  (void)hipDeviceSynchronize();
  if (e->xabort_host) (void)hipHostFree(e->xabort_host);
  (void)sdrm_comm_destroy(e);
  for (float* b : e->dec_buf)
    if (b) (void)hipFree(b);
  if (e->ev_fork) (void)hipEventDestroy(e->ev_fork);
  if (e->ev_hold) (void)hipEventDestroy(e->ev_hold);
  for (int c = 0; c < 3; ++c) {
    if (e->ev_join[c]) (void)hipEventDestroy(e->ev_join[c]);
    if (e->aux[c]) (void)hipStreamDestroy(e->aux[c]);
  }
  delete e;
  return SDRM_OK;
}

int sdrm_set_schedule(sdrm_engine* e, float beta1, float beta2) {
  if (!e) return SDRM_ERR_ARG;
  HIP_TRY(e, hipSetDevice(e->device));
  HIP_TRY(e, hipDeviceSynchronize());
  return upload_schedule(e, beta1, beta2);
}

int sdrm_get_schedule(const sdrm_engine* e, float* b, float* a, float* ab) {
  if (!e || !b || !a || !ab) return SDRM_ERR_ARG;
  const size_t n = (size_t)e->T + 1;
  std::memcpy(b, e->h_beta.data(), n * 4);
  std::memcpy(a, e->h_alpha.data(), n * 4);
  std::memcpy(ab, e->h_alphabar.data(), n * 4);
  return SDRM_OK;
}

int sdrm_set_params(sdrm_engine* e, const float* flat, void* stream) {
  if (!e || !flat) return fail(e, SDRM_ERR_ARG, "sdrm_set_params: null pointer");
  hipStream_t st = (hipStream_t)stream;
  if (int jr = join_chains(e, st)) return jr;
  HIP_TRY(e, hipMemcpyAsync(e->p, flat, e->P * 4, hipMemcpyDeviceToDevice, st));
  return launch_adam(e, nullptr, 0.f, 0, st);
}

int sdrm_get_params(const sdrm_engine* e, float* flat, void* stream) {
  if (!e || !flat) return SDRM_ERR_ARG;
  sdrm_engine* me = const_cast<sdrm_engine*>(e);
  HIP_TRY(me, hipMemcpyAsync(flat, e->p, e->P * 4, hipMemcpyDeviceToDevice, (hipStream_t)stream));
  return SDRM_OK;
}

const float* sdrm_params_ptr(const sdrm_engine* e) { return e ? e->p : nullptr; }

int sdrm_get_grads(const sdrm_engine* e, float* flat, void* stream) {
  if (!e || !flat) return SDRM_ERR_ARG;
  sdrm_engine* me = const_cast<sdrm_engine*>(e);
  HIP_TRY(me, hipMemcpyAsync(flat, e->grad_src ? e->grad_src : e->g, e->P * 4, hipMemcpyDeviceToDevice, (hipStream_t)stream));
  return SDRM_OK;
}

int sdrm_get_adam_state(const sdrm_engine* e, float* m, float* v, int64_t* step_host, void* stream) {
  if (!e) return SDRM_ERR_ARG;
  sdrm_engine* me = const_cast<sdrm_engine*>(e);
  if (m) HIP_TRY(me, hipMemcpyAsync(m, e->m, e->P * 4, hipMemcpyDeviceToDevice, (hipStream_t)stream));
  if (v) HIP_TRY(me, hipMemcpyAsync(v, e->v, e->P * 4, hipMemcpyDeviceToDevice, (hipStream_t)stream));
  if (step_host) *step_host = e->adam_t;
  return SDRM_OK;
}

int sdrm_set_adam_state(sdrm_engine* e, const float* m, const float* v, int64_t step, void* stream) {
  if (!e || step < 0) return fail(e, SDRM_ERR_ARG, "sdrm_set_adam_state: bad argument");
  if (m) HIP_TRY(e, hipMemcpyAsync(e->m, m, e->P * 4, hipMemcpyDeviceToDevice, (hipStream_t)stream));
  if (v) HIP_TRY(e, hipMemcpyAsync(e->v, v, e->P * 4, hipMemcpyDeviceToDevice, (hipStream_t)stream));
  e->adam_t = step;
  return SDRM_OK;
}

int sdrm_adam_reset(sdrm_engine* e, void* stream) {
  if (!e) return SDRM_ERR_ARG;
  HIP_TRY(e, hipMemsetAsync(e->m, 0, e->P * 4, (hipStream_t)stream));
  HIP_TRY(e, hipMemsetAsync(e->v, 0, e->P * 4, (hipStream_t)stream));
  e->adam_t = 0;
  return SDRM_OK;
}

namespace {
bool sample_persist_fits(const sdrm_engine* e, const SampleState& s);
}
int sdrm_train_forward(sdrm_engine* e, const float* x0, int B, int64_t row0, int mode, const sdrm_train_randoms* rnd,
                       uint64_t seed, uint64_t step, float nd, double* sums, void* stream) {
  if (!e || !x0) return fail(e, SDRM_ERR_ARG, "sdrm_train_forward: null pointer");
  if (B < 1 || B > e->max_rows) return fail(e, SDRM_ERR_SHAPE, "sdrm_train_forward: B outside [1, max_rows]");
  if (mode == SDRM_RNG_EXPLICIT && (!rnd || !rnd->noise || !rnd->t || !rnd->keep))
    return fail(e, SDRM_ERR_ARG, "sdrm_train_forward: EXPLICIT mode needs noise, t and keep");
  if (mode != SDRM_RNG_EXPLICIT && mode != SDRM_RNG_PHILOX) return fail(e, SDRM_ERR_ARG, "bad rng mode");
  hipStream_t st = (hipStream_t)stream;
  e->bwd_begun = false;
  if (!e->train_since_sample) e->hold_needed = false;
  e->train_since_sample = true; e->hold_recorded = false;
  if (e->tune.detach > 0 && e->smp.active && !e->smp.skinny && e->smp.i_next >= 1 && e->n_chains == 1 && e->n_aux == 0 && !e->detach_armed &&
      !e->prof_on && !sample_persist_fits(e, e->smp)) {
    HIP_TRY(e, hipEventRecord(e->ev_fork, st));
    e->detach_armed = true;
  }
  const int MP = round_up(3 * B, BM), n = e->T + 1;
  const int cfg = choose_cfg(e->tune, MP, e->tune.nt32_max_rows_train);
  e->fwd_done = false;

  e->cur_grouped = false; e->cur_act = false; e->cur_sk = false; e->cur_g16 = false; e->cur_rows = MP; e->cur_parts = 1; e->cur_skip_pre = false;
  if (int xs = split_status(e)) return xs;
  if (skinny_net(e)) {
    int rc = e->WeP ? SDRM_OK : ensure_tables(e, st);
    if (rc) return rc;
    SkStepArgs ka = sk_step_args(e, B);
    ka.x0 = x0;
    if (mode == SDRM_RNG_EXPLICIT) { ka.noise = rnd->noise; ka.t = rnd->t; ka.keep = rnd->keep; }
    ka.mode = mode; ka.seed_lo = (uint32_t)seed; ka.seed_hi = (uint32_t)(seed >> 32); ka.step = (uint32_t)step;
    ka.row0 = row0; ka.nd = nd;
    bool done4 = false;
    if (e->tune.skinny == 1) {
      ka.NP = 4 * ka.G;
      rc = launch_sk_fwd4(e, ka, st, &done4);
      if (rc) return rc;
    }
    if (!done4) {
      ka.NP = ka.G;
      rc = launch_sk_step(e, ka, 0, ka.G, st);
      if (rc) return rc;
    }
    e->cur_sk_np = ka.NP;
    if (!e->fold_sums) {
      SDRM_LAUNCH(e, k_loss_sums, dim3(1), dim3(256), 0, st, (const double*)e->loss_part, ka.NP, (double)B * (double)e->L,
                         sums ? sums : e->sums);
      HIP_TRY(e, hipGetLastError());
    }
    e->cur_B = B; e->cur_MP = round_up(SK_ROWS * ka.G, BM); e->cur_rows = SK_ROWS * ka.G; e->cur_x0 = x0; e->cur_sk = true; e->fwd_done = true;
    return SDRM_OK;
  }

  if (use_rowchain(e, B)) {
    int rc = emb_tables(e, st, x0, (size_t)B * e->L);
    if (rc) return rc;
    const int G = (B + RC_USERS - 1) / RC_USERS, MPg = round_up(G * RC_ROWS, BM);
    rc = launch_row_forward(e, x0, B, row0, mode, rnd, seed, step, nd, G, st);
    if (rc) return rc;
    if (!e->fold_sums) {
      SDRM_LAUNCH(e, k_loss_sums, dim3(1), dim3(256), 0, st, (const double*)e->loss_part, G, (double)B * (double)e->L,
                         sums ? sums : e->sums);
      HIP_TRY(e, hipGetLastError());
    }
    e->cur_B = B; e->cur_MP = MPg; e->cur_rows = G * RC_ROWS; e->cur_x0 = x0; e->cur_grouped = true; e->cur_act = true; e->fwd_done = true;
    e->hold_needed = true;
    return SDRM_OK;
  }

  if (const int parts = rows48_parts(e, B)) {
    int rc = emb_tables(e, st, x0, (size_t)B * e->L);
    if (rc) return rc;
    const int G = (B + R48_USERS - 1) / R48_USERS, MPg = round_up(G * R48_ROWS, BM);
    rc = launch_row_forward(e, x0, B, row0, mode, rnd, seed, step, nd, G, st, parts);
    if (rc) return rc;
    if (!e->fold_sums) {
      SDRM_LAUNCH(e, k_loss_sums, dim3(1), dim3(256), 0, st, (const double*)e->loss_part, G * parts, (double)B * (double)e->L,
                         sums ? sums : e->sums);
      HIP_TRY(e, hipGetLastError());
    }
    e->cur_B = B; e->cur_MP = MPg; e->cur_rows = G * R48_ROWS; e->cur_x0 = x0; e->cur_g16 = true; e->cur_parts = parts; e->cur_act = true;
    e->hold_needed = true;
    e->fwd_done = true;
    return SDRM_OK;
  }

  PrepTrainArgs pa{};
  pa.x0 = x0;
  if (mode == SDRM_RNG_EXPLICIT) { pa.noise = rnd->noise; pa.t = rnd->t; pa.keep = rnd->keep; }
  pa.sqrt_ab = e->sched + 3 * n; pa.one_minus_ab = e->sched + 4 * n; pa.tembP = e->tembP;
  pa.U = e->U; pa.tdev = e->tdev;
  pa.B = B; pa.L = e->L; pa.LP = e->LP; pa.K0 = e->K0; pa.T = e->T; pa.MP = MP;
  pa.mode = mode; pa.seed_lo = (uint32_t)seed; pa.seed_hi = (uint32_t)(seed >> 32); pa.step = (uint32_t)step;
  pa.row0 = row0; pa.nd = nd;
  {
    pa.emb = emb_args(e);
    e->tables_fresh = true;
    pa.emb_row0 = B + (MP - 3 * B);
    pa.emb_chunks = (e->WP + 63) / 64;
    pa.emb_blocks = (e->T + 1) * pa.emb_chunks;
    const int main_blocks = (int)(((int64_t)pa.emb_row0 * (e->K0 / 4) + 255) / 256);
    SDRM_LAUNCH(e, k_prep_train, dim3(pa.emb_blocks + main_blocks), dim3(256), 2 * e->T * sizeof(float), st, pa);
    HIP_TRY(e, hipGetLastError());
  }
  {
    GemmArgs a{};
    a.C = pre_buf(e, 0); a.ldc = e->WP; a.bias = e->B0tab; a.ldtab = e->WP; a.trow = e->tdev; a.trow_B = B;
    HIP_TRY(e, (gemm_forward<XF_NONE, EPI_BIAS_ROWTAB>(a, e->U, e->K0, e->W0c, e->K0, MP, e->WP, e->LP, st,
                                                       Prof{e, PC_FWD_L0, 2.0 * 3 * B * (double)e->W * e->L}, cfg)));
  }
  int rc = hidden_forward(e, MP, 3 * B, st, cfg);
  if (rc) return rc;
  {
    GemmArgs a{};
    a.C = e->Y; a.ldc = e->LP; a.bias = e->boc; a.slopeA = slope_ptr(e, e->H);
    a.rows_valid = MP; a.cols_valid = e->LP;
    HIP_TRY(e, (gemm_forward<XF_PRELU, EPI_BIAS_TANH>(a, pre_buf(e, e->H), e->WP, e->Woc, e->WP, MP, e->LP, e->WP, st,
                                                      Prof{e, PC_FWD_OUT, 2.0 * 3 * B * (double)e->L * e->W}, cfg)));
  }
  LossArgs la{};
  la.Y = e->Y; la.x0 = x0; la.B = B; la.L = e->L; la.LP = e->LP; la.part = e->loss_part;
  SDRM_LAUNCH(e, k_loss_partials, dim3(LOSS_BLOCKS), dim3(1024), 0, st, la);
  HIP_TRY(e, hipGetLastError());
  if (!e->fold_sums) {
    SDRM_LAUNCH(e, k_loss_sums, dim3(1), dim3(256), 0, st, (const double*)e->loss_part, LOSS_BLOCKS,
                       (double)B * (double)e->L, sums ? sums : e->sums);
    HIP_TRY(e, hipGetLastError());
  }
  e->cur_B = B; e->cur_MP = MP; e->cur_x0 = x0; e->fwd_done = true;
  return SDRM_OK;
}

namespace {

int backward_chain(sdrm_engine* e, const double* sums, float* loss, hipStream_t st, bool with_wgrad0) {
  const int B = e->cur_B, MP = e->cur_MP, H = e->H;
  e->bwd_strips = false;
  SeedArgs sa{};
  sa.sums = e->fold_sums ? nullptr : (sums ? sums : e->sums); sa.Y = e->Y; sa.x0 = e->cur_x0; sa.dY = e->dY; sa.loss = loss;
  sa.B = B; sa.L = e->L; sa.LP = e->LP; sa.MP = MP; sa.grouped = (e->cur_sk || e->cur_g16) ? 2 : (e->cur_grouped ? 1 : 0);
  sa.part = e->loss_part;
  sa.nblk = e->cur_grouped ? (B + RC_USERS - 1) / RC_USERS : (e->cur_g16 ? e->cur_parts * ((B + R48_USERS - 1) / R48_USERS) : LOSS_BLOCKS);
  sa.count = (double)B * (double)e->L;
  const bool chain48 = e->cur_g16 && e->WhfT && e->tune.dgrad_rows > 0 && e->LP == e->WP && H + 1 <= DR_MAX_LAYERS;
  const bool chain = chain48 || (use_dgrad_rows(e, MP) && e->tune.dgrad_rows == 1 && H + 1 <= DR_MAX_LAYERS);
  if (!chain && !e->cur_sk) {
    const int nslots = e->cur_grouped ? RC_USERS * ((B + RC_USERS - 1) / RC_USERS) : (e->cur_g16 ? R48_USERS * ((B + R48_USERS - 1) / R48_USERS) : B);
    const unsigned need = (unsigned)(((size_t)(nslots + (MP - 3 * nslots)) * (e->LP / 4) + 255) / 256);
    dim3 grid(std::min(need, 2048u));
    SDRM_LAUNCH(e, k_loss_seed, grid, dim3(256), 0, st, sa);
    HIP_TRY(e, hipGetLastError());
  }
  int S0, SH, SO, kc0, kcH, kcO;
  pick_splits(e->tune, MP, wgrad_tiles(e->tune, e->WP, e->K0) + H * wgrad_tiles(e->tune, e->WP, e->WP) + wgrad_tiles(e->tune, e->LP, e->WP),
              S0, kc0);
  SH = SO = S0; kcH = kcO = kc0;
  const int cfg_d = choose_cfg(e->tune, MP, e->tune.nt32_max_rows_train);
  const int cfg_w = pick_cfg(e->tune);
  e->bwd_cfg_w = cfg_w;
  const int dgrad_blocks = ((MP + kCfgBM[cfg_d] - 1) / kCfgBM[cfg_d]) * ((e->WP + kCfgBN[cfg_d] - 1) / kCfgBN[cfg_d]);
  const double flO = 2.0 * 3 * B * (double)e->L * e->W, flH = 2.0 * 3 * B * (double)e->W * e->W;
  const double fl0 = 2.0 * 3 * B * (double)e->W * (e->L + e->T);
  e->bwd_hidden_apps = H;
  if (e->cur_sk) {
    SkStepArgs ka = sk_step_args(e, B);
    ka.NP = e->cur_sk_np;
    ka.x0 = e->cur_x0; ka.sums = sa.sums; ka.count = sa.count; ka.loss = loss;
    const int S = std::min(ka.G, S_MAX);
    int rc = launch_sk_step(e, ka, 1, S, st);
    if (rc) return rc;
    e->bwd_S0 = e->bwd_SH = e->bwd_SO = S; e->bwd_hidden_apps = 1; e->bwd_dgrad_blocks = S;
    e->bwd_kc0 = e->bwd_kcH = e->bwd_kcO = 0;
    return SDRM_OK;
  }
  if (chain48) {
    DgradChain48Args c8{};
    DgradChainArgs& ca = c8.c;
    ca.seed = sa; ca.nlayers = H + 1;
    ca.layer[0] = dgrad_rows_args(e, e->dY, e->WofT, pre_buf(e, H), slope_ptr(e, H), dpre_buf(e, H), e->alpha_part + (size_t)H * e->alpha_part_stride);
    for (int k = H; k >= 1; --k)
      ca.layer[H + 1 - k] = dgrad_rows_args(e, dpre_buf(e, k), e->WhfT, pre_buf(e, k - 1), slope_ptr(e, k - 1), dpre_buf(e, k - 1),
                                            e->alpha_part + (size_t)(k - 1) * e->alpha_part_stride);
    const int Gn = e->cur_rows / R48_ROWS;
    c8.pad_rows = MP - e->cur_rows;
    int rc = launch_rows48_chain(e, c8, Gn, e->cur_parts, flO + H * flH, st);
    if (rc) return rc;
    if (with_wgrad0)
      HIP_TRY(e, (gemm_wgrad<XF_NONE>(dpre_buf(e, 0), e->WP, e->WP, e->U, e->K0, e->K0, nullptr, MP, S0, kc0, e->slab0, e->db0s, st,
                                      Prof{e, PC_WGRAD_L0, fl0}, cfg_w)));
    e->bwd_kc0 = kc0;
    e->bwd_S0 = S0; e->bwd_SH = SH; e->bwd_SO = SO; e->bwd_dgrad_blocks = Gn * e->cur_parts;
    e->bwd_kcH = kcH; e->bwd_kcO = kcO;
    return SDRM_OK;
  }
  if (use_dgrad_rows(e, MP)) {
    int rc = SDRM_OK;
    if (chain) {
      DgradChainArgs ca{};
      ca.seed = sa; ca.nlayers = H + 1;
      ca.layer[0] = dgrad_rows_args(e, e->dY, e->WofT, pre_buf(e, H), slope_ptr(e, H), dpre_buf(e, H), e->alpha_part + (size_t)H * e->alpha_part_stride);
      for (int k = H; k >= 1; --k)
        ca.layer[H + 1 - k] = dgrad_rows_args(e, dpre_buf(e, k), e->WhfT, pre_buf(e, k - 1), slope_ptr(e, k - 1), dpre_buf(e, k - 1),
                                              e->alpha_part + (size_t)(k - 1) * e->alpha_part_stride);
      rc = launch_dgrad_chain(e, ca, MP, flO + H * flH, st);
    } else {
      rc = launch_dgrad_rows(e, e->dY, e->WofT, pre_buf(e, H), slope_ptr(e, H), dpre_buf(e, H),
                             e->alpha_part + (size_t)H * e->alpha_part_stride, MP, flO, st);
      for (int k = H; k >= 1 && !rc; --k)
        rc = launch_dgrad_rows(e, dpre_buf(e, k), e->WhfT, pre_buf(e, k - 1), slope_ptr(e, k - 1), dpre_buf(e, k - 1),
                               e->alpha_part + (size_t)(k - 1) * e->alpha_part_stride, MP, flH, st);
    }
    if (rc) return rc;
    if (with_wgrad0)
      HIP_TRY(e, (gemm_wgrad<XF_NONE>(dpre_buf(e, 0), e->WP, e->WP, e->U, e->K0, e->K0, nullptr, MP, S0, kc0, e->slab0, e->db0s, st,
                                      Prof{e, PC_WGRAD_L0, fl0}, cfg_w)));
    e->bwd_kc0 = kc0;
    e->bwd_S0 = S0; e->bwd_SH = SH; e->bwd_SO = SO; e->bwd_dgrad_blocks = MP / RC_ROWS;
    e->bwd_kcH = kcH; e->bwd_kcO = kcO;
    return SDRM_OK;
  }
  HIP_TRY(e, gemm_dgrad(e, e->dY, e->LP, e->WocT, e->LP, MP, e->LP, e->WP, dpre_buf(e, H), pre_buf(e, H), slope_ptr(e, H),
                        e->alpha_part + (size_t)H * e->alpha_part_stride, st, flO, cfg_d));
  for (int k = H; k >= 1; --k)
    HIP_TRY(e, gemm_dgrad(e, dpre_buf(e, k), e->WP, e->WhcT, e->WP, MP, e->WP, e->WP, dpre_buf(e, k - 1), pre_buf(e, k - 1),
                          slope_ptr(e, k - 1), e->alpha_part + (size_t)(k - 1) * e->alpha_part_stride, st, flH, cfg_d));
  if (with_wgrad0)
    HIP_TRY(e, (gemm_wgrad<XF_NONE>(dpre_buf(e, 0), e->WP, e->WP, e->U, e->K0, e->K0, nullptr, MP, S0, kc0, e->slab0, e->db0s, st,
                                    Prof{e, PC_WGRAD_L0, fl0}, cfg_w)));
  e->bwd_kc0 = kc0;
  e->bwd_S0 = S0; e->bwd_SH = SH; e->bwd_SO = SO; e->bwd_dgrad_blocks = dgrad_blocks;
  e->bwd_kcH = kcH; e->bwd_kcO = kcO;
  return SDRM_OK;
}

int backward_wgrads(sdrm_engine* e, hipStream_t st, bool with_wgrad0) {
  if (e->cur_sk) return SDRM_OK;
  const int B = e->cur_B, MP = e->cur_MP, H = e->H, SH = e->bwd_SH, SO = e->bwd_SO;
  const double flO = 2.0 * 3 * B * (double)e->L * e->W, flH = 2.0 * 3 * B * (double)e->W * e->W;
  const double fl0 = 2.0 * 3 * B * (double)e->W * (e->L + e->T);
  if (e->bwd_cfg_w > 0) {
    const int cfg_w = e->bwd_cfg_w;
    if (with_wgrad0)
      HIP_TRY(e, (gemm_wgrad<XF_NONE>(dpre_buf(e, 0), e->WP, e->WP, e->U, e->K0, e->K0, nullptr, MP, e->bwd_S0, e->bwd_kc0, e->slab0,
                                      e->db0s, st, Prof{e, PC_WGRAD_L0, fl0}, cfg_w)));
    HIP_TRY(e, (gemm_wgrad<XF_PRELU>(e->dY, e->LP, e->LP, pre_buf(e, H), e->WP, e->WP, slope_ptr(e, H), MP, SO, e->bwd_kcO,
                                     e->slabO, e->dbOs, st, Prof{e, PC_WGRAD, flO}, cfg_w)));
    for (int k = H; k >= 1; --k)
      HIP_TRY(e, (gemm_wgrad<XF_PRELU>(dpre_buf(e, k), e->WP, e->WP, pre_buf(e, k - 1), e->WP, e->WP, slope_ptr(e, k - 1), MP, SH,
                                       e->bwd_kcH, e->slabH + (size_t)(k - 1) * SH * e->WP * e->WP,
                                       e->dbHs + (size_t)(k - 1) * SH * e->WP, st, Prof{e, PC_WGRAD, flH}, cfg_w)));
    return SDRM_OK;
  }
  if (with_wgrad0 && use_strips(e)) return launch_wgrad_strips(e, MP, fl0 + flO + H * flH, st);
  std::vector<WgradSpec> w;
  std::vector<double> fl;
  if (with_wgrad0) {
    w.push_back(WgradSpec{dpre_buf(e, 0), e->WP, e->WP, e->U, e->K0, e->K0, e->one_dev, e->bwd_S0, e->bwd_kc0, e->slab0, e->db0s});
    fl.push_back(fl0);
  }
  const bool plain = e->cur_act;
  auto opnd = [&](int k) { return plain ? e->act + (size_t)k * e->MPmax * e->WP : pre_buf(e, k); };
  w.push_back(WgradSpec{e->dY, e->LP, e->LP, opnd(H), e->WP, e->WP, slope_ptr(e, H), SO, e->bwd_kcO, e->slabO, e->dbOs});
  fl.push_back(flO);
  for (int k = H; k >= 1; --k) {
    w.push_back(WgradSpec{dpre_buf(e, k), e->WP, e->WP, opnd(k - 1), e->WP, e->WP, slope_ptr(e, k - 1), SH, e->bwd_kcH,
                          e->slabH + (size_t)(k - 1) * SH * e->WP * e->WP, e->dbHs + (size_t)(k - 1) * SH * e->WP});
    fl.push_back(flH);
  }
  for (size_t lo = 0; lo < w.size(); lo += GEMM_BATCH_MAX) {
    const int n = (int)std::min<size_t>(GEMM_BATCH_MAX, w.size() - lo);
    double f = 0.0;
    for (int k = 0; k < n; ++k) f += fl[lo + k];
    HIP_TRY(e, launch_wgrad_batch(e, w.data() + lo, n, MP, st, Prof{e, PC_WGRAD, f}, plain));
  }
  return SDRM_OK;
}

enum { BUCKET_FIRST = 1, BUCKET_SECOND = 2, BUCKET_BOTH = 3 };

int backward_tail(sdrm_engine* e, float* gout, int which, bool update, float lr, hipStream_t st) {
  const int L = e->L, W = e->W, T = e->T, H = e->H;
  const int S0 = e->bwd_S0, SH = e->bwd_SH, SO = e->bwd_SO;
  const int bias_col = e->bwd_strips ? e->ones_col : -1;
  TailArgs a{};
  int n = 0, blocks = 0;
  auto add = [&](int kind, int64_t off, int rows, int cols, int flat_ld, const float* src, int src_ld, size_t slab_stride, int nslabs,
                 int nblocks) -> TailJob& {
    TailJob& j = a.j[n];
    j.kind = kind; j.flat_off = off; j.rows = rows; j.cols = cols; j.flat_ld = flat_ld;
    j.src = src; j.src_ld = src_ld; j.slab_stride = slab_stride; j.nslabs = nslabs; j.inner = 1; j.nblocks = nblocks; j.lanes = 4;
    j.red = nullptr; j.red_ld = 0;
    j.dst = j.dstT = j.dstF = j.dstFT = nullptr; j.dst_ld = j.dstT_ld = 0; j.fnct = e->WP / 16; j.fklast = j.fklastT = -1;
    a.start[n++] = blocks;
    blocks += nblocks;
    return j;
  };
  auto mat = [&](int64_t off, int rows, int cols, int flat_ld, const float* src, int src_ld, size_t slab_stride, int nslabs) -> TailJob& {
    const int lanes = nslabs > 32 ? 4 : (nslabs > 8 ? 2 : 1), tsr = lanes == 1 ? 32 : 16, tsc = lanes == 4 ? 16 : 32;
    TailJob& j = add(TJ_MAT, off, rows, cols, flat_ld, src, src_ld, slab_stride, nslabs, ((rows + tsr - 1) / tsr) * ((cols + tsc - 1) / tsc));
    j.lanes = lanes;
    return j;
  };
  auto vec = [&](int64_t off, int len, const float* col_src, int col_ld, size_t col_stride, const float* sum_src, size_t sum_stride, int nslabs,
                 float* dst) -> TailJob& {
    TailJob& j = bias_col >= 0 ? add(TJ_VEC, off, len, 1, 1, col_src + bias_col, col_ld, col_stride, nslabs, (len + 63) / 64)
                               : add(TJ_VEC, off, len, 1, 1, sum_src, 1, sum_stride, nslabs, (len + 63) / 64);
    j.dst = dst;
    return j;
  };
  auto snap = [&](int64_t off, int rows, int cols, int flat_ld, float* dst, int dst_ld) {
    TailJob& j = add(TJ_SNAP, off, rows, cols, flat_ld, nullptr, 0, 0, 0, rows * ((cols + TAIL_THREADS * 8 - 1) / (TAIL_THREADS * 8)));
    j.red = dst; j.red_ld = dst_ld;
  };
  if (which & BUCKET_FIRST) {
    {
      TailJob& j = mat(e->off_w0, W, L, L + T, e->slab0, e->K0, (size_t)e->WP * e->K0, S0);
      j.dst = e->W0c; j.dst_ld = e->K0; j.dstF = e->W0f; j.fklast = rc_light_klast(L, e->LP);
    }
    vec(e->off_b0, W, e->slab0, e->K0, (size_t)e->WP * e->K0, e->db0s, (size_t)e->WP, S0, e->b0c);
    {
      TailJob& j = mat(0, W, T, 0, e->slab0 + e->LP, e->K0, (size_t)e->WP * e->K0, S0);
      j.red = e->Mred; j.red_ld = e->TP;
    }
    snap(e->off_we, 1, T * T + T, 0, e->snap, 0);
    snap(e->off_w0 + L, W, T, L + T, e->snap + (size_t)T * T + T, T);
  }
  if (which & BUCKET_SECOND) {
    {
      TailJob& j = add(TJ_SCALAR, e->off_a0, 1, 1, 1, e->alpha_part, 0, (size_t)e->alpha_part_stride, 1, 1);
      j.inner = e->bwd_dgrad_blocks;
    }
    if (H >= 1) {
      const int HS = e->bwd_hidden_apps * SH;
      TailJob& j = mat(e->off_wh, W, W, W, e->slabH, e->WP, (size_t)e->WP * e->WP, HS);
      j.dst = e->Whc; j.dst_ld = e->WP; j.dstT = e->WhcT; j.dstT_ld = e->WP; j.dstF = e->Whf; j.dstFT = e->WhfT;
      j.fklast = j.fklastT = rc_light_klast(W, e->WP);
      vec(e->off_bh, W, e->slabH, e->WP, (size_t)e->WP * e->WP, e->dbHs, (size_t)e->WP, HS, e->bhc);
      TailJob& s = add(TJ_SCALAR, e->off_ah, 1, 1, 1, e->alpha_part + e->alpha_part_stride, 0, (size_t)e->alpha_part_stride, H, 1);
      s.inner = e->bwd_dgrad_blocks;
    }
    {
      TailJob& j = mat(e->off_wo, L, W, W, e->slabO, e->WP, (size_t)e->LP * e->WP, SO);
      j.dst = e->Woc; j.dst_ld = e->WP; j.dstT = e->WocT; j.dstT_ld = e->LP; j.dstF = e->Wof; j.dstFT = e->WofT;
      j.fklast = rc_light_klast(W, e->WP); j.fklastT = rc_light_klast(L, e->LP);
    }
    vec(e->off_bo, L, e->slabO, e->WP, (size_t)e->LP * e->WP, e->dbOs, (size_t)e->LP, SO, e->boc);
  }
  a.start[n] = blocks;
  a.n = n;
  a.p = e->p; a.m = e->m; a.v = e->v; a.g = gout;
  a.L = L; a.W = W; a.T = T; a.LP = e->LP; a.TP = e->TP;
  a.off_we = e->off_we; a.off_be = e->off_be; a.off_w0 = e->off_w0; a.off_b0 = e->off_b0;
  a.Mred = e->Mred; a.snap = e->snap; a.WeP = e->WeP; a.W0eP = e->W0eP; a.TPe = e->TPe;
  a.b1 = 0.9f; a.b2 = 0.999f; a.eps = 1e-8f; a.wd = 1e-4f; a.update = update ? 1 : 0;
  if (update) adam_scalars(e, lr, a.step_size, a.bc2_sqrt);
  int per_lane = 0;
  for (int q = 0; q < n; ++q)
    if (a.j[q].kind == TJ_MAT) per_lane = std::max(per_lane, (a.j[q].nslabs + a.j[q].lanes - 1) / a.j[q].lanes);
  if (per_lane <= 8) SDRM_LAUNCH(e, k_tail<8>, dim3((unsigned)blocks), dim3(TAIL_THREADS), 0, st, a);
  else SDRM_LAUNCH(e, k_tail<16>, dim3((unsigned)blocks), dim3(TAIL_THREADS), 0, st, a);
  HIP_TRY(e, hipGetLastError());
  if (update) e->tables_fresh = false;
  if (which & BUCKET_FIRST) {
    const int eb = tail_emb_blocks_a(W, T) + tail_emb_blocks_b(T) + tail_emb_blocks_c(T);
    SDRM_LAUNCH(e, k_tail_emb, dim3((unsigned)eb), dim3(256), tail_emb_lds_floats(T, e->TP) * sizeof(float), st, a);
    HIP_TRY(e, hipGetLastError());
  }
  return SDRM_OK;
}

}

int sdrm_train_backward_begin(sdrm_engine* e, const double* sums, float* grad, float* loss, void* stream) {
  if (!e) return SDRM_ERR_ARG;
  if (!e->fwd_done) return fail(e, SDRM_ERR_STATE, "sdrm_train_backward: no forward to back-propagate");
  hipStream_t st = (hipStream_t)stream;
  e->bwd_begun = false;
  float* gout = grad ? grad : e->g;
  e->grad_src = gout;
  int rc = backward_chain(e, sums, loss, st, true);
  if (!rc) rc = backward_tail(e, gout, BUCKET_FIRST, false, 0.f, st);
  if (rc) return rc;
  e->bwd_begun = true;
  return SDRM_OK;
}

int sdrm_train_backward_finish(sdrm_engine* e, float* grad, void* stream) {
  if (!e) return SDRM_ERR_ARG;
  if (!e->fwd_done || !e->bwd_begun) return fail(e, SDRM_ERR_STATE, "sdrm_train_backward_finish: sdrm_train_backward_begin not run");
  hipStream_t st = (hipStream_t)stream;
  float* gout = grad ? grad : e->g;
  if (gout != e->grad_src) return fail(e, SDRM_ERR_ARG, "sdrm_train_backward_finish: different gradient buffer than begin");
  int rc = backward_wgrads(e, st, false);
  if (!rc) rc = hold_point(e, st);
  if (!rc) rc = backward_tail(e, gout, BUCKET_SECOND, false, 0.f, st);
  e->bwd_begun = false;
  return rc;
}

static int train_backward_impl(sdrm_engine* e, const double* sums, float* grad, float* loss, hipStream_t st, const float* fused_lr) {
  e->bwd_begun = false;
  float* gout = grad ? grad : e->g;
  e->grad_src = gout;
  int rc = backward_chain(e, sums, loss, st, false);
  if (!rc) rc = backward_wgrads(e, st, true);
  if (!rc) rc = hold_point(e, st);
  if (!rc) rc = backward_tail(e, gout, BUCKET_BOTH, fused_lr != nullptr, fused_lr ? *fused_lr : 0.f, st);
  return rc;
}

int sdrm_train_backward(sdrm_engine* e, const double* sums, float* grad, float* loss, void* stream) {
  if (!e) return SDRM_ERR_ARG;
  if (!e->fwd_done) return fail(e, SDRM_ERR_STATE, "sdrm_train_backward: no forward to back-propagate");
  return train_backward_impl(e, sums, grad, loss, (hipStream_t)stream, nullptr);
}

int sdrm_grad_buckets(const sdrm_engine* e, int64_t* first_off, int64_t* first_len, int64_t* second_off, int64_t* second_len) {
  if (!e || !first_off || !first_len || !second_off || !second_len) return SDRM_ERR_ARG;
  *first_off = 0; *first_len = e->off_a0;
  *second_off = e->off_a0; *second_len = e->P - e->off_a0;
  return SDRM_OK;
}

int sdrm_adam_step(sdrm_engine* e, const float* grad, float lr, void* stream) {
  if (!e) return SDRM_ERR_ARG;
  if (int jr = join_chains(e, (hipStream_t)stream)) return jr;
  e->adam_t += 1;
  return launch_adam(e, grad, lr, 1, (hipStream_t)stream);
}

int sdrm_train_step(sdrm_engine* e, const float* x0, int B, float lr, int mode, const sdrm_train_randoms* rnd,
                    uint64_t seed, uint64_t step, float nd, float* loss, void* stream) {
  if (!e) return SDRM_ERR_ARG;
  e->fold_sums = true;
  int rc = sdrm_train_forward(e, x0, B, 0, mode, rnd, seed, step, nd, nullptr, stream);
  e->fold_sums = false;
  if (rc) return rc;
  e->fold_sums = true;
  e->adam_t += 1;
  rc = train_backward_impl(e, nullptr, nullptr, loss, (hipStream_t)stream, &lr);
  e->fold_sums = false;
  if (rc) e->adam_t -= 1;
  return rc;
}

#define NCCL_TRY(e, api, call)                                                                  \
  do {                                                                                          \
    ncclResult_t _r = (call);                                                                   \
    if (_r != ncclSuccess) {                                                                    \
      (e)->err = std::string(#call) + ": " + (api)->GetErrorString(_r);                         \
      return SDRM_ERR_RCCL;                                                                     \
    }                                                                                           \
  } while (0)

int sdrm_comm_available(void) { return rccl_api(nullptr) != nullptr ? 1 : 0; }

int sdrm_comm_unique_id(void* id_host) {
  if (!id_host) return SDRM_ERR_ARG;
  const RcclApi* api = rccl_api(nullptr);
  if (!api) return SDRM_ERR_RCCL;
  static_assert(sizeof(ncclUniqueId) == SDRM_COMM_ID_BYTES, "ncclUniqueId size");
  ncclUniqueId id;
  if (api->GetUniqueId(&id) != ncclSuccess) return SDRM_ERR_RCCL;
  std::memcpy(id_host, &id, sizeof(id));
  return SDRM_OK;
}

namespace {
int exchange_streams(sdrm_engine* e, void* aux_stream) {
  Exchange& x = e->xch;
  if (aux_stream) { x.aux = (hipStream_t)aux_stream; x.aux_owned = false; }
  else { HIP_TRY(e, hipStreamCreateWithFlags(&x.aux, hipStreamNonBlocking)); x.aux_owned = true; }
  HIP_TRY(e, hipEventCreateWithFlags(&x.ev_bucket, hipEventDisableTiming));
  HIP_TRY(e, hipEventCreateWithFlags(&x.ev_done, hipEventDisableTiming));
  return SDRM_OK;
}
}

int sdrm_comm_init_rank(sdrm_engine* e, int nranks, int rank, const void* id_host) {
  if (!e || !id_host || nranks < 1 || rank < 0 || rank >= nranks) return fail(e, SDRM_ERR_ARG, "sdrm_comm_init_rank: bad argument");
  if (e->xch.comm) return fail(e, SDRM_ERR_STATE, "sdrm_comm_init_rank: this engine already has a communicator");
  std::string why;
  const RcclApi* api = rccl_api(&why);
  if (!api) return fail(e, SDRM_ERR_RCCL, why);
  HIP_TRY(e, hipSetDevice(e->device));
  ncclUniqueId id;
  std::memcpy(&id, id_host, sizeof(id));
  ncclComm_t comm = nullptr;
  NCCL_TRY(e, api, api->CommInitRank(&comm, nranks, id, rank));
  e->xch.comm = comm; e->xch.comm_owned = true; e->xch.nranks = nranks; e->xch.rank = rank;
  return exchange_streams(e, nullptr);
}

int sdrm_allreduce_init(sdrm_engine* e, void* rccl_comm, void* aux_stream) {
  if (!e || !rccl_comm) return fail(e, SDRM_ERR_ARG, "sdrm_allreduce_init: null pointer");
  if (e->xch.comm) return fail(e, SDRM_ERR_STATE, "sdrm_allreduce_init: this engine already has a communicator");
  std::string why;
  const RcclApi* api = rccl_api(&why);
  if (!api) return fail(e, SDRM_ERR_RCCL, why);
  ncclComm_t comm = (ncclComm_t)rccl_comm;
  int n = 0, r = -1;
  NCCL_TRY(e, api, api->CommCount(comm, &n));
  NCCL_TRY(e, api, api->CommUserRank(comm, &r));
  e->xch.comm = comm; e->xch.comm_owned = false; e->xch.nranks = n; e->xch.rank = r;
  return exchange_streams(e, aux_stream);
}

int sdrm_comm_info(const sdrm_engine* e, int* nranks, int* rank) {
  if (!e) return SDRM_ERR_ARG;
  if (nranks) *nranks = e->xch.comm ? e->xch.nranks : 0;
  if (rank) *rank = e->xch.comm ? e->xch.rank : -1;
  return SDRM_OK;
}

void* sdrm_debug_comm_handle(const sdrm_engine* e) { return e ? (void*)e->xch.comm : nullptr; }

int sdrm_comm_destroy(sdrm_engine* e) {
  if (!e) return SDRM_ERR_ARG;
  Exchange& x = e->xch;
  if (!x.comm) return SDRM_OK;
  (void)hipSetDevice(e->device);
  (void)hipDeviceSynchronize();
  if (x.comm_owned)
    if (const RcclApi* api = rccl_api(nullptr)) (void)api->CommDestroy(x.comm);
  if (x.ev_bucket) (void)hipEventDestroy(x.ev_bucket);
  if (x.ev_done) (void)hipEventDestroy(x.ev_done);
  if (x.aux && x.aux_owned) (void)hipStreamDestroy(x.aux);
  x = Exchange{};
  return SDRM_OK;
}

int sdrm_train_step_sharded(sdrm_engine* e, const float* x0, int B, int64_t row0, float lr, int mode,
                            const sdrm_train_randoms* rnd, uint64_t seed, uint64_t step, float nd, float* loss, void* stream) {
  if (!e) return SDRM_ERR_ARG;
  Exchange& x = e->xch;
  if (!x.comm) return fail(e, SDRM_ERR_STATE, "sdrm_train_step_sharded: no communicator (sdrm_comm_init_rank / sdrm_allreduce_init)");
  const RcclApi* api = rccl_api(nullptr);
  if (!api) return fail(e, SDRM_ERR_RCCL, "librccl is gone");
  hipStream_t st = (hipStream_t)stream;
  int rc = sdrm_train_forward(e, x0, B, row0, mode, rnd, seed, step, nd, e->sums, stream);
  if (rc) return rc;
  NCCL_TRY(e, api, api->AllReduce(e->sums, e->sums, 5, ncclDouble, ncclSum, x.comm, st));
  const int buckets = e->tune.ar_buckets == 2 ? 2 : 1;
  if (buckets == 1) {
    rc = sdrm_train_backward(e, e->sums, nullptr, loss, stream);
    if (rc) return rc;
    NCCL_TRY(e, api, api->AllReduce(e->g, e->g, (size_t)e->P, ncclFloat, ncclSum, x.comm, st));
    return sdrm_adam_step(e, nullptr, lr, stream);
  }
  rc = sdrm_train_backward_begin(e, e->sums, nullptr, loss, stream);
  if (rc) return rc;
  const int64_t n0 = e->off_a0, n1 = e->P - e->off_a0;
  HIP_TRY(e, hipEventRecord(x.ev_bucket, st));
  HIP_TRY(e, hipStreamWaitEvent(x.aux, x.ev_bucket, 0));
  NCCL_TRY(e, api, api->AllReduce(e->g, e->g, (size_t)n0, ncclFloat, ncclSum, x.comm, x.aux));
  rc = sdrm_train_backward_finish(e, nullptr, stream);
  if (rc) return rc;
  HIP_TRY(e, hipEventRecord(x.ev_bucket, st));
  HIP_TRY(e, hipStreamWaitEvent(x.aux, x.ev_bucket, 0));
  NCCL_TRY(e, api, api->AllReduce(e->g + n0, e->g + n0, (size_t)n1, ncclFloat, ncclSum, x.comm, x.aux));
  HIP_TRY(e, hipEventRecord(x.ev_done, x.aux));
  HIP_TRY(e, hipStreamWaitEvent(st, x.ev_done, 0));
  return sdrm_adam_step(e, nullptr, lr, stream);
}

int sdrm_get_train_outputs(const sdrm_engine* e, float* psq, void* stream) {
  if (!e || !psq) return SDRM_ERR_ARG;
  sdrm_engine* me = const_cast<sdrm_engine*>(e);
  if (!e->fwd_done) return fail(me, SDRM_ERR_STATE, "sdrm_get_train_outputs: no forward yet");
  SDRM_LAUNCH(e, k_unpad_psq, dim3(256), dim3(256), 0, (hipStream_t)stream, (const float*)e->Y, e->cur_B, e->L,
                     e->LP, (e->cur_sk || e->cur_g16) ? 2 : (e->cur_grouped ? 1 : 0), psq);
  HIP_TRY(me, hipGetLastError());
  return SDRM_OK;
}

static int forward_rows(sdrm_engine* e, const float* x, const int64_t* t, int t_uniform, int n, int mode,
                        const uint8_t* keep, uint64_t seed, uint64_t step, int64_t row0, float* out, int ldout,
                        int cols_valid, hipStream_t st) {
  if (int jr = join_chains(e, st)) return jr;
  const int MP = round_up(n, BM);
  const int cfg = choose_cfg(e->tune, MP, e->tune.nt32_max_rows);
  PrepFwdArgs pa{};
  pa.x = x; pa.t = t; pa.t_uniform = t_uniform; pa.keep = keep; pa.U = e->U;
  pa.n = n; pa.L = e->L; pa.LP = e->LP; pa.K0 = e->K0; pa.T = e->T; pa.MP = MP;
  pa.mode = mode; pa.seed_lo = (uint32_t)seed; pa.seed_hi = (uint32_t)(seed >> 32); pa.step = (uint32_t)step;
  pa.row0 = row0;
  pa.bpr = (e->K0 / 2 + 255) / 256;
  dim3 grid((unsigned)((size_t)pa.bpr * MP));
  SDRM_LAUNCH(e, k_prep_forward, grid, dim3(256), 0, st, pa);
  HIP_TRY(e, hipGetLastError());
  int rc = ensure_tables(e, st);
  if (rc) return rc;
  {
    GemmArgs a{};
    a.C = pre_buf(e, 0); a.ldc = e->WP; a.bias = e->b0c;
    HIP_TRY(e, (gemm_forward<XF_NONE, EPI_BIAS>(a, e->U, e->K0, e->W0c, e->K0, MP, e->WP, e->K0, st,
                                                Prof{e, PC_FWD_L0, 2.0 * n * (double)e->W * (e->L + e->T)}, cfg)));
  }
  rc = hidden_forward(e, MP, n, st, cfg);
  if (rc) return rc;
  GemmArgs a{};
  a.C = out; a.ldc = ldout; a.bias = e->boc; a.slopeA = slope_ptr(e, e->H);
  a.rows_valid = n; a.cols_valid = cols_valid;
  HIP_TRY(e, (gemm_forward<XF_PRELU, EPI_BIAS_TANH_G>(a, pre_buf(e, e->H), e->WP, e->Woc, e->WP, MP, e->LP, e->WP, st,
                                                    Prof{e, PC_FWD_OUT, 2.0 * n * (double)e->L * e->W}, cfg)));
  return SDRM_OK;
}

int sdrm_forward(sdrm_engine* e, const float* x, const int64_t* t, int n, int mode, const uint8_t* keep, uint64_t seed,
                 uint64_t step, int64_t row0, float* out, void* stream) {
  if (!e || !x || !t || !out) return fail(e, SDRM_ERR_ARG, "sdrm_forward: null pointer");
  if (n < 1 || n > 3 * e->max_rows) return fail(e, SDRM_ERR_SHAPE, "sdrm_forward: n outside [1, 3*max_rows]");
  if (mode == SDRM_RNG_EXPLICIT && !keep) return fail(e, SDRM_ERR_ARG, "sdrm_forward: EXPLICIT mode needs keep");
  e->fwd_done = false;
  return forward_rows(e, x, t, 0, n, mode, keep, seed, step, row0, out, e->L, e->L, (hipStream_t)stream);
}

int sdrm_reverse_step(sdrm_engine* e, float* x, int n, int i, const float* z, const uint8_t* keep, void* stream) {
  if (!e || !x || !keep) return fail(e, SDRM_ERR_ARG, "sdrm_reverse_step: null pointer");
  if (n < 1 || n > 3 * e->max_rows) return fail(e, SDRM_ERR_SHAPE, "sdrm_reverse_step: n outside [1, 3*max_rows]");
  if (i < 1 || i > e->T) return fail(e, SDRM_ERR_ARG, "sdrm_reverse_step: step outside [1, T]");
  hipStream_t st = (hipStream_t)stream;
  e->fwd_done = false;
  int rc = forward_rows(e, x, nullptr, i, n, SDRM_RNG_EXPLICIT, keep, 0, 0, 0, e->Y, e->LP, e->LP, st);
// ... 676 lines not shown
```

### sdrm_amd/csrc/wgrad2.h

```cpp
#pragma once
#include <hip/hip_runtime.h>
#include <stdint.h>

#include "bufres.h"
#include "gemm.h"

#ifndef WG2_DIAG
#define WG2_DIAG 0
#endif

namespace sdrm {

constexpr int WG2_MAX_PROBLEMS = 8;
constexpr int WG2_MAX_UNITS = 32;
constexpr int WG2_BK = 16;

struct Wg2Problem {
  const float* A; int lda;
  const float* B; int ldb;
  float* slab; int ldc;
  size_t slab_stride;
};

struct Wg2Strip { int8_t problem; int8_t ktile; };

struct Wg2Args {
  Wg2Problem p[WG2_MAX_PROBLEMS];
  Wg2Strip strip[WG2_MAX_UNITS][4];
  int units, slices, rows, kchunk;
};

__device__ __forceinline__ Wg2Problem wg2_problem(const Wg2Args& a, int idx) {
  Wg2Problem r = a.p[0];
#pragma unroll
  for (int p = 1; p < WG2_MAX_PROBLEMS; ++p)
    if (p == idx) r = a.p[p];
  return r;
}

template <int NT>
struct Wg2Cfg {
  static constexpr int WP = 32 * NT, LDA = WP + 4, LDB = 32 + 4;
  static constexpr int A_TILE = WG2_BK * LDA, B_TILE = WG2_BK * LDB;
  static constexpr int STAGE = 2 * A_TILE + 4 * B_TILE;
  static constexpr size_t LDS_BYTES = 2 * (size_t)STAGE * 4;
  static constexpr int NA4 = WG2_BK * WP / 4, NB4 = 4 * WG2_BK * 32 / 4;
  static constexpr int NLA = (NA4 + NTHREADS - 1) / NTHREADS, NLB = NB4 / NTHREADS;
  static_assert(NLB == 2, "two B blocks per half work-group");
  static_assert(LDS_BYTES <= 160 * 1024, "stages do not fit LDS");
};

template <int NT>
__global__ __launch_bounds__(NTHREADS, 1) void k_wgrad_strips(const Wg2Args a) {
  typedef Wg2Cfg<NT> C;
  constexpr int WP = C::WP, LDA = C::LDA, LDB = C::LDB, BK = WG2_BK;
  __shared__ __attribute__((aligned(16))) float smem[2 * C::STAGE];
  const int tid = threadIdx.x, lane = tid & 63;
  const int wave = __builtin_amdgcn_readfirstlane(tid >> 6);
  const int l31 = lane & 31, lhi = lane >> 5;
  const int logical = xcd_remap((int)blockIdx.x, a.units * a.slices);
  const int slice = logical / a.units, unit = logical - slice * a.units;
  const int m_begin = slice * a.kchunk, m_end = min(m_begin + a.kchunk, a.rows);
  const int nt = (m_end - m_begin) / BK;

  const Wg2Strip st = a.strip[unit][wave];
  const int pa = a.strip[unit][0].problem;
  int pb = pa;
#pragma unroll
  for (int w = 1; w < 4; ++w)
    if (a.strip[unit][w].problem >= 0) pb = a.strip[unit][w].problem;
  const bool two = pb != pa;
  const int ai = (st.problem == pa || st.problem < 0) ? 0 : 1;
  const bool active = st.problem >= 0;

  constexpr int QA = WP / 4;
  const Wg2Problem Pa = wg2_problem(a, pa), Pb = wg2_problem(a, pb);
  const int lda_a = Pa.lda, lda_b = Pb.lda;
  auto span = [&](int ld, int skip) __attribute__((always_inline)) {
    const size_t b = ((size_t)(a.rows - m_begin) * (size_t)ld - (size_t)skip) * 4;
    return (uint32_t)(b < 0xffffffffull ? b : 0xffffffffull);
  };
  const brsrc Ra = make_brsrc(Pa.A + (size_t)m_begin * lda_a, span(lda_a, 0)), Rb = make_brsrc(Pb.A + (size_t)m_begin * lda_b, span(lda_b, 0));
  brsrc RB0, RB1; int Bld[2];
  {
    const Wg2Strip s0 = a.strip[unit][(wave >> 1)], s1 = a.strip[unit][(wave >> 1) + 2];
    const Wg2Problem P0 = wg2_problem(a, s0.problem < 0 ? pa : s0.problem), P1 = wg2_problem(a, s1.problem < 0 ? pa : s1.problem);
    Bld[0] = P0.ldb; Bld[1] = P1.ldb;
    const int c0 = 32 * (s0.problem < 0 ? 0 : s0.ktile), c1 = 32 * (s1.problem < 0 ? 0 : s1.ktile);
    RB0 = make_brsrc(P0.B + (size_t)m_begin * P0.ldb + c0, span(P0.ldb, c0));
    RB1 = make_brsrc(P1.B + (size_t)m_begin * P1.ldb + c1, span(P1.ldb, c1));
  }
  struct RSet { float4 a[C::NLA], a2[C::NLA], b[C::NLB]; };
  RSet r0, r1, r2;
  auto zero = [&](RSet& r) __attribute__((always_inline)) {
#pragma unroll
    for (int j = 0; j < C::NLA; ++j) r.a[j] = r.a2[j] = make_float4(0.f, 0.f, 0.f, 0.f);
#pragma unroll
    for (int j = 0; j < C::NLB; ++j) r.b[j] = make_float4(0.f, 0.f, 0.f, 0.f);
  };
  zero(r0); zero(r1); zero(r2);
  int rowA[C::NLA], quadA[C::NLA];
#pragma unroll
  for (int j = 0; j < C::NLA; ++j) {
    const int f = min(tid + j * NTHREADS, C::NA4 - 1);
    rowA[j] = f / QA; quadA[j] = f - rowA[j] * QA;
  }
  const int rowB = (tid & 127) >> 3, quadB = tid & 7;
  uint32_t voA[C::NLA], voA2[C::NLA], voB[2];
#pragma unroll
  for (int j = 0; j < C::NLA; ++j) {
    voA[j] = (uint32_t)((rowA[j] * lda_a + 4 * quadA[j]) * 4);
    voA2[j] = (uint32_t)((rowA[j] * lda_b + 4 * quadA[j]) * 4);
  }
#pragma unroll
  for (int j = 0; j < 2; ++j) voB[j] = (uint32_t)((rowB * Bld[j] + 4 * quadB) * 4);
  auto as4 = [](f32x4_b v) __attribute__((always_inline)) { return make_float4(v[0], v[1], v[2], v[3]); };
  auto gload_piece = [&](auto two_tag, RSet& r, int m0, int k) __attribute__((always_inline)) {
    constexpr bool TWO = decltype(two_tag)::value;
    constexpr int NA = TWO ? 2 * C::NLA : C::NLA;
    if (k < C::NLA) r.a[k] = as4(bload4(Ra, voA[k], (uint32_t)((m0 - m_begin) * lda_a) * 4u));
    else if (TWO && k < NA) r.a2[k - C::NLA] = as4(bload4(Rb, voA2[k - C::NLA], (uint32_t)((m0 - m_begin) * lda_b) * 4u));
    else if (k == NA) r.b[0] = as4(bload4(RB0, voB[0], (uint32_t)((m0 - m_begin) * Bld[0]) * 4u));
    else if (k == NA + 1) r.b[1] = as4(bload4(RB1, voB[1], (uint32_t)((m0 - m_begin) * Bld[1]) * 4u));
  };
  auto lstore_piece = [&](auto two_tag, const RSet& r, float* S, int k) __attribute__((always_inline)) {
    constexpr bool TWO = decltype(two_tag)::value;
    constexpr int NA = TWO ? 2 * C::NLA : C::NLA;
    if (k < C::NLA) *reinterpret_cast<float4*>(S + rowA[k] * LDA + 4 * quadA[k]) = r.a[k];
    else if (TWO && k < NA) *reinterpret_cast<float4*>(S + C::A_TILE + rowA[k - C::NLA] * LDA + 4 * quadA[k - C::NLA]) = r.a2[k - C::NLA];
    else if (k < NA + C::NLB)
      *reinterpret_cast<float4*>(S + 2 * C::A_TILE + ((wave >> 1) + 2 * (k - NA)) * C::B_TILE + rowB * LDB + 4 * quadB) = r.b[k - NA];
  };
  auto gload = [&](auto two_tag, RSet& r, int step) __attribute__((always_inline)) {
    constexpr int NPC = (decltype(two_tag)::value ? 2 * C::NLA : C::NLA) + C::NLB;
    const int m0 = m_begin + min(step, nt - 1) * BK;
#pragma unroll
    for (int k = 0; k < NPC; ++k) gload_piece(two_tag, r, m0, k);
  };
  auto lstore = [&](auto two_tag, const RSet& r, int stage) __attribute__((always_inline)) {
    constexpr int NPC = (decltype(two_tag)::value ? 2 * C::NLA : C::NLA) + C::NLB;
#pragma unroll
    for (int k = 0; k < NPC; ++k) lstore_piece(two_tag, r, smem + stage * C::STAGE, k);
  };

  f32x16 acc[NT];
#pragma unroll
  for (int t = 0; t < NT; ++t)
#pragma unroll
    for (int r = 0; r < 16; ++r) acc[t][r] = 0.f;

  const int aoff = ai * C::A_TILE + lhi * LDA + l31;
  const int boff = 2 * C::A_TILE + wave * C::B_TILE + lhi * LDB + l31;

  auto kstep = [&](auto two_tag, int i, RSet& nx) __attribute__((always_inline)) {
    constexpr int NPC = (decltype(two_tag)::value ? 2 * C::NLA : C::NLA) + C::NLB;
    constexpr int NSLOT = (BK / 2) * NT, HALF = NSLOT / 2;
    constexpr int STRIDE = HALF / NPC >= 1 ? HALF / NPC : 1;
    static_assert(NPC <= HALF, "more staging pieces than MFMA slots");
    const float* S = smem + (i & 1) * C::STAGE;
    float* Sn = smem + ((i + 1) & 1) * C::STAGE;
    const int m4 = m_begin + min(i + 4, nt - 1) * BK;
    float fa0[NT], fa1[NT], fb0 = 0.f, fb1 = 0.f;
#pragma unroll
    for (int t = 0; t < NT; ++t) fa0[t] = S[aoff + 32 * t];
    fb0 = S[boff];
#pragma unroll
    for (int g = 0; g < BK / 2; ++g) {
      float (&ca)[NT] = (g & 1) ? fa1 : fa0;
      float (&na)[NT] = (g & 1) ? fa0 : fa1;
      const float cb = (g & 1) ? fb1 : fb0;
      float& nb = (g & 1) ? fb0 : fb1;
#pragma unroll
      for (int t = 0; t < NT; ++t) {
        if (!(WG2_DIAG & 1)) acc[t] = __builtin_amdgcn_mfma_f32_32x32x2f32(ca[t], cb, acc[t], 0, 0, 0);
        if (g + 1 < BK / 2 && !(WG2_DIAG & 8)) {
          if (t == 0) nb = S[boff + 2 * (g + 1) * LDB];
          na[t] = S[aoff + 2 * (g + 1) * LDA + 32 * t];
        }
        const int slot = g * NT + t;
        if (slot < HALF) {
          if (slot % STRIDE == 0 && slot / STRIDE < NPC && !(WG2_DIAG & 2)) lstore_piece(two_tag, nx, Sn, slot / STRIDE);
        } else {
          const int s2 = slot - HALF;
          if (s2 % STRIDE == 0 && s2 / STRIDE < NPC && !(WG2_DIAG & 4)) gload_piece(two_tag, nx, m4, s2 / STRIDE);
        }
        __builtin_amdgcn_sched_barrier(0);
      }
    }
    __syncthreads();
  };
  auto run = [&](auto two_tag) __attribute__((always_inline)) {
    gload(two_tag, r0, 0);
    lstore(two_tag, r0, 0);
    gload(two_tag, r1, 1); gload(two_tag, r2, 2); gload(two_tag, r0, 3);
    __syncthreads();
    int i = 0;
    for (; i + 2 < nt; i += 3) {
      kstep(two_tag, i, r1);
      kstep(two_tag, i + 1, r2);
      kstep(two_tag, i + 2, r0);
    }
    if (i < nt) kstep(two_tag, i, r1);
    if (i + 1 < nt) kstep(two_tag, i + 1, r2);
  };
  if (nt > 0) {
    if (two) run(std::true_type{});
    else run(std::false_type{});
  }

  if (!active) return;
  const Wg2Problem P = wg2_problem(a, st.problem);
  float* __restrict__ dst = P.slab + (size_t)slice * P.slab_stride + (size_t)(4 * lhi) * P.ldc + 32 * st.ktile + l31;
#pragma unroll
  for (int t = 0; t < NT; ++t)
#pragma unroll
    for (int r = 0; r < 16; ++r) dst[(size_t)(32 * t + (r & 3) + 8 * (r >> 2)) * P.ldc] = acc[t][r];
}

inline int wg2_plan(const int* ktiles, int nproblems, Wg2Args& a) {
  int n = 0;
  for (int p = 0; p < nproblems; ++p) n += ktiles[p];
  const int units = (n + 3) / 4;
  if (nproblems > WG2_MAX_PROBLEMS || units > WG2_MAX_UNITS) return 0;
  int u = 0, w = 0;
  for (int p = 0; p < nproblems; ++p)
    for (int k = 0; k < ktiles[p]; ++k) {
      a.strip[u][w].problem = (int8_t)p; a.strip[u][w].ktile = (int8_t)k;
      if (++w == 4) { w = 0; ++u; }
    }
  for (; w > 0 && w < 4; ++w) { a.strip[u][w].problem = -1; a.strip[u][w].ktile = 0; }
  a.units = units;
  return units;
}

}
```

### sdrm_amd/engine.py

```python
from __future__ import annotations

import ctypes as C
import os
import weakref

import numpy as np
import torch

from . import _lib, synth


class SdrmError(RuntimeError):
    pass


def _ptr(t):
    return None if t is None else C.c_void_p(t.data_ptr())


def _stream():
    return C.c_void_p(torch.cuda.current_stream().cuda_stream)


class _ParamSpan:

    def __init__(self, ptr, n):
        self.__cuda_array_interface__ = {"shape": (n,), "typestr": "<f4", "data": (ptr, False), "version": 2}


class Engine:

    def __init__(self, L, W, T, H, max_rows, device=None):
        if not torch.cuda.is_available():
            raise SdrmError("sdrm_amd needs a ROCm device: no GPU is visible and there is no CPU fallback")
        self.lib = _lib.load()
        self.L, self.W, self.T, self.H, self.max_rows = int(L), int(W), int(T), int(H), int(max_rows)
        self.device = torch.device("cuda", torch.cuda.current_device() if device is None else int(device))
        self._h = C.c_void_p()
        rc = self.lib.sdrm_create(self.L, self.W, self.T, self.H, self.max_rows, self.device.index, C.byref(self._h))
        if rc != 0:
            msg = self.lib.sdrm_last_error(self._h).decode() if self._h else ""
            if self._h:
                self.lib.sdrm_destroy(self._h)
                self._h = C.c_void_p()
            raise SdrmError(f"sdrm_create failed: {_lib.STATUS.get(rc, rc)} {msg}")
        self.P = int(self.lib.sdrm_param_count(self._h))
        assert self.P == synth.param_count(self.L, self.W, self.T, self.H)
        self._sums = torch.zeros(8, dtype=torch.float64, device=self.device)
        self._loss = torch.zeros(1, dtype=torch.float32, device=self.device)
        self.gradient_buckets = 2 if os.environ.get("SDRM_AR_BUCKETS", "1").strip() == "2" else 1
        self._keepalive = None
        self._n_views = 0
        self._close_pending = False

    def close(self):
        if not getattr(self, "_h", None):
            return
        if self._n_views > 0:
            self._close_pending = True
            return
        torch.cuda.synchronize(self.device)
        self.lib.sdrm_destroy(self._h)
        self._h = C.c_void_p()
        self._close_pending = False

    @property
    def closed(self):
        return not getattr(self, "_h", None)

    @staticmethod
    def _view_released(eng):
        eng._n_views -= 1
        if eng._close_pending and eng._n_views <= 0:
            eng.close()

    def __del__(self):
        try:
            self.close()
        except Exception:
            pass

    def _check(self, rc, what):
        if rc != 0:
            raise SdrmError(f"{what}: {_lib.STATUS.get(rc, rc)}: {self.lib.sdrm_last_error(self._h).decode()}")

    def _dev(self, a, dtype):
        if isinstance(a, torch.Tensor):
            t = a.to(device=self.device, dtype=dtype)
        else:
            t = torch.from_numpy(np.ascontiguousarray(a)).to(device=self.device, dtype=dtype)
        return t.contiguous()

    def debug_set(self, tile=None, skinny=None, fused_reverse=None, chains=None, nt32_rows=None, nt32_rows_train=None,
                  gradient_buckets=None, rowchain=None, wgrad_strips=None, dgrad_rows=None, rows48=None, rows48_split=None, sample_persist=None, rows48_share=None):
        if rowchain is not None:
            self._check(self.lib.sdrm_debug_set_rowchain(self._h, int(rowchain)), "sdrm_debug_set_rowchain")
        if rows48_share is not None:
            self._check(self.lib.sdrm_debug_set_rows48_share(self._h, int(rows48_share)), "sdrm_debug_set_rows48_share")
        if sample_persist is not None:
            self._check(self.lib.sdrm_debug_set_sample_persist(self._h, int(sample_persist)), "sdrm_debug_set_sample_persist")
        if rows48_split is not None:
            self._check(self.lib.sdrm_debug_set_rows48_split(self._h, int(rows48_split)), "sdrm_debug_set_rows48_split")
        if rows48 is not None:
            self._check(self.lib.sdrm_debug_set_rows48(self._h, int(rows48)), "sdrm_debug_set_rows48")
        if wgrad_strips is not None:
            self._check(self.lib.sdrm_debug_set_wgrad_strips(self._h, int(bool(wgrad_strips))), "sdrm_debug_set_wgrad_strips")
        if dgrad_rows is not None:
            self._check(self.lib.sdrm_debug_set_dgrad_rows(self._h, int(dgrad_rows)), "sdrm_debug_set_dgrad_rows")
        if gradient_buckets is not None:
            self._check(self.lib.sdrm_debug_set_gradient_buckets(self._h, int(gradient_buckets)), "sdrm_debug_set_gradient_buckets")
            self.gradient_buckets = int(gradient_buckets)
        if tile is not None:
            self._check(self.lib.sdrm_debug_set_tile(self._h, int(tile)), "sdrm_debug_set_tile")
        if skinny is not None:
            self._check(self.lib.sdrm_debug_set_skinny(self._h, int(skinny)), "sdrm_debug_set_skinny")
        if fused_reverse is not None:
            self._check(self.lib.sdrm_debug_set_fused_reverse(self._h, int(fused_reverse)), "sdrm_debug_set_fused_reverse")
        if chains is not None:
            self._check(self.lib.sdrm_debug_set_chains(self._h, int(chains)), "sdrm_debug_set_chains")
        if nt32_rows is not None or nt32_rows_train is not None:
            self._check(self.lib.sdrm_debug_set_nt32_rows(self._h, -1 if nt32_rows is None else int(nt32_rows),
                                                          -1 if nt32_rows_train is None else int(nt32_rows_train)),
                        "sdrm_debug_set_nt32_rows")
        return self

    @property
    def sampler_chains(self):
        return int(self.lib.sdrm_debug_chains(self._h))

    @property
    def rows48_split_available(self):
        return bool(self.lib.sdrm_debug_rows48_split_available(self._h))

    @property
    def rowchain_available(self):
        return bool(self.lib.sdrm_debug_rowchain_available(self._h))

    def set_params(self, flat):
        flat = self._dev(flat, torch.float32).reshape(-1)
        if flat.numel() != self.P:
            raise SdrmError(f"set_params: expected {self.P} floats, got {flat.numel()}")
        self._check(self.lib.sdrm_set_params(self._h, _ptr(flat), _stream()), "sdrm_set_params")
        self._keepalive = flat

    def _flat_out(self, fn, name):
        out = torch.empty(self.P, dtype=torch.float32, device=self.device)
        self._check(fn(self._h, _ptr(out), _stream()), name)
        return out

    def get_params(self):
        return self._flat_out(self.lib.sdrm_get_params, "sdrm_get_params")

    def params_view(self):
        span = _ParamSpan(int(self.lib.sdrm_params_ptr(self._h)), self.P)
        self._n_views += 1
        weakref.finalize(span, Engine._view_released, self).atexit = False
        return torch.as_tensor(span, device=self.device)

    def philox_draws(self, seed, purpose, step, rows, quads, row0=0, with_bits=True):
        normals = torch.empty(rows, 4 * quads, dtype=torch.float32, device=self.device)
        bits = torch.empty(rows, 4 * quads, dtype=torch.uint8, device=self.device) if with_bits else None
        self._check(self.lib.sdrm_debug_philox_draws(self._h, int(seed), int(purpose), int(step), int(row0), int(rows), int(quads),
                                                     _ptr(normals), _ptr(bits), _stream()), "sdrm_debug_philox_draws")
        return normals, bits

    def get_grads(self):
        return self._flat_out(self.lib.sdrm_get_grads, "sdrm_get_grads")

    def get_adam_state(self):
        m = torch.empty(self.P, dtype=torch.float32, device=self.device)
        v = torch.empty(self.P, dtype=torch.float32, device=self.device)
        step = C.c_int64()
        self._check(self.lib.sdrm_get_adam_state(self._h, _ptr(m), _ptr(v), C.byref(step), _stream()), "sdrm_get_adam_state")
        return m, v, int(step.value)

    def set_adam_state(self, m, v, step):
        m, v = self._dev(m, torch.float32), self._dev(v, torch.float32)
        self._check(self.lib.sdrm_set_adam_state(self._h, _ptr(m), _ptr(v), int(step), _stream()), "sdrm_set_adam_state")
        self._keepalive = (m, v)

    def adam_reset(self):
        self._check(self.lib.sdrm_adam_reset(self._h, _stream()), "sdrm_adam_reset")

    def set_schedule(self, beta1=1e-4, beta2=0.02):
        self._check(self.lib.sdrm_set_schedule(self._h, beta1, beta2), "sdrm_set_schedule")

    def get_schedule(self):
        n = self.T + 1
        b, a, ab = (np.empty(n, np.float32) for _ in range(3))
        self._check(self.lib.sdrm_get_schedule(self._h, b.ctypes.data_as(C.c_void_p), a.ctypes.data_as(C.c_void_p),
                                               ab.ctypes.data_as(C.c_void_p)), "sdrm_get_schedule")
        return b, a, ab

    def _randoms(self, noise, t, keep, B):
        noise = self._dev(noise, torch.float32)
        t = self._dev(t, torch.int64)
        keep = self._dev(keep, torch.uint8)
        if tuple(noise.shape) != (B, self.L) or tuple(t.shape) != (B,) or tuple(keep.shape) != (3, B, self.L):
            raise SdrmError("explicit randoms: expected noise [B,L], t [B], keep [3,B,L]")
        self._keepalive = (noise, t, keep)
        return _lib.TrainRandoms(noise.data_ptr(), t.data_ptr(), keep.data_ptr())

    def train_forward(self, x0, noise=None, t=None, keep=None, seed=0, step=0, nd=1.0, row0=0, sums=None):
        x0 = self._dev(x0, torch.float32)
        B = x0.shape[0]
        if x0.dim() != 2 or x0.shape[1] != self.L:
            raise SdrmError(f"train_forward: x0 must be [B,{self.L}]")
        self._x0 = x0
        sums = self._sums if sums is None else sums
        if noise is not None:
            rnd = self._randoms(noise, t, keep, B)
            rc = self.lib.sdrm_train_forward(self._h, _ptr(x0), B, int(row0), _lib.RNG_EXPLICIT, C.byref(rnd), 0, 0,
                                             float(nd), _ptr(sums), _stream())
        else:
            rc = self.lib.sdrm_train_forward(self._h, _ptr(x0), B, int(row0), _lib.RNG_PHILOX, None, int(seed),
                                             int(step), float(nd), _ptr(sums), _stream())
        self._check(rc, "sdrm_train_forward")
        return sums

    def train_backward(self, sums=None, grad=None):
        sums = self._sums if sums is None else sums
        self._check(self.lib.sdrm_train_backward(self._h, _ptr(sums), _ptr(grad), _ptr(self._loss), _stream()),
                    "sdrm_train_backward")
        return self._loss

    def train_backward_begin(self, sums=None, grad=None):
        sums = self._sums if sums is None else sums
        self._check(self.lib.sdrm_train_backward_begin(self._h, _ptr(sums), _ptr(grad), _ptr(self._loss), _stream()),
                    "sdrm_train_backward_begin")
        return self._loss

    def train_backward_finish(self, grad=None):
        self._check(self.lib.sdrm_train_backward_finish(self._h, _ptr(grad), _stream()), "sdrm_train_backward_finish")

    def grad_buckets(self):
        v = [C.c_int64() for _ in range(4)]
        self._check(self.lib.sdrm_grad_buckets(self._h, *[C.byref(x) for x in v]), "sdrm_grad_buckets")
        return (int(v[0].value), int(v[1].value)), (int(v[2].value), int(v[3].value))

    def adam_step(self, lr, grad=None):
        self._check(self.lib.sdrm_adam_step(self._h, _ptr(grad), float(lr), _stream()), "sdrm_adam_step")

    def train_step(self, x0, lr, noise=None, t=None, keep=None, seed=0, step=0, nd=1.0):
        x0 = self._dev(x0, torch.float32)
        B = x0.shape[0]
        if x0.dim() != 2 or x0.shape[1] != self.L:
            raise SdrmError(f"train_step: x0 must be [B,{self.L}]")
        self._x0 = x0
        if noise is not None:
            rnd = self._randoms(noise, t, keep, B)
            rc = self.lib.sdrm_train_step(self._h, _ptr(x0), B, float(lr), _lib.RNG_EXPLICIT, C.byref(rnd), 0, 0,
                                          float(nd), _ptr(self._loss), _stream())
        else:
            rc = self.lib.sdrm_train_step(self._h, _ptr(x0), B, float(lr), _lib.RNG_PHILOX, None, int(seed), int(step),
                                          float(nd), _ptr(self._loss), _stream())
        self._check(rc, "sdrm_train_step")
        return self._loss

    @staticmethod
    def comm_available() -> bool:
        return bool(_lib.load().sdrm_comm_available())

    @staticmethod
    def comm_unique_id() -> bytes:
        buf = C.create_string_buffer(128)
        rc = _lib.load().sdrm_comm_unique_id(buf)
        if rc != 0:
            raise SdrmError(f"sdrm_comm_unique_id: {_lib.STATUS.get(rc, rc)} (librccl could not be loaded?)")
        return buf.raw

    def comm_init_rank(self, nranks: int, rank: int, unique_id: bytes):
        if len(unique_id) != 128:
            raise SdrmError("comm_init_rank: the unique id is 128 bytes")
        self._check(self.lib.sdrm_comm_init_rank(self._h, int(nranks), int(rank), C.c_char_p(unique_id)), "sdrm_comm_init_rank")
        return self

    def comm_info(self):
        n, r = C.c_int(), C.c_int()
        self._check(self.lib.sdrm_comm_info(self._h, C.byref(n), C.byref(r)), "sdrm_comm_info")
        return int(n.value), int(r.value)

    def train_step_sharded(self, x0, lr, row0=0, noise=None, t=None, keep=None, seed=0, step=0, nd=1.0):
        x0 = self._dev(x0, torch.float32)
        B = x0.shape[0]
        if x0.dim() != 2 or x0.shape[1] != self.L:
            raise SdrmError(f"train_step_sharded: x0 must be [B,{self.L}]")
        self._x0 = x0
        if noise is not None:
            rnd = self._randoms(noise, t, keep, B)
            rc = self.lib.sdrm_train_step_sharded(self._h, _ptr(x0), B, int(row0), float(lr), _lib.RNG_EXPLICIT, C.byref(rnd),
                                                  0, 0, float(nd), _ptr(self._loss), _stream())
        else:
            rc = self.lib.sdrm_train_step_sharded(self._h, _ptr(x0), B, int(row0), float(lr), _lib.RNG_PHILOX, None, int(seed),
                                                  int(step), float(nd), _ptr(self._loss), _stream())
        self._check(rc, "sdrm_train_step_sharded")
        return self._loss

    def train_outputs(self, B):
        out = torch.empty(3, B, self.L, dtype=torch.float32, device=self.device)
        self._check(self.lib.sdrm_get_train_outputs(self._h, _ptr(out), _stream()), "sdrm_get_train_outputs")
        return out

    def preacts(self, layer, B):
        out = torch.empty(3, B, self.W, dtype=torch.float32, device=self.device)
        self._check(self.lib.sdrm_get_preacts(self._h, int(layer), _ptr(out), _stream()), "sdrm_get_preacts")
        return out

    def launch_count(self):
        return int(self.lib.sdrm_launch_count(self._h))

    def profile_begin(self, capacity=4096, only=None):
        cls = -1
        if only is not None:
            names = [self.lib.sdrm_profile_name(c).decode() for c in range(self.lib.sdrm_profile_classes())]
            cls = names.index(only)
        self._check(self.lib.sdrm_profile_only(self._h, cls), "sdrm_profile_only")
        self._check(self.lib.sdrm_profile_begin(self._h, int(capacity)), "sdrm_profile_begin")

    def profile_end(self):
        self._check(self.lib.sdrm_profile_end(self._h, _stream()), "sdrm_profile_end")
        out = {}
        for c in range(self.lib.sdrm_profile_classes()):
            ms, n, fl = C.c_double(), C.c_int64(), C.c_double()
            self._check(self.lib.sdrm_profile_get(self._h, c, C.byref(ms), C.byref(n), C.byref(fl)), "sdrm_profile_get")
            if n.value:
                out[self.lib.sdrm_profile_name(c).decode()] = (ms.value, int(n.value), fl.value)
        return out

    def forward(self, x, t, keep=None, seed=0, step=0, row0=0):
        x = self._dev(x, torch.float32)
        t = self._dev(t, torch.int64)
        n = x.shape[0]
        out = torch.empty(n, self.L, dtype=torch.float32, device=self.device)
        if keep is not None:
            keep = self._dev(keep, torch.uint8)
            rc = self.lib.sdrm_forward(self._h, _ptr(x), _ptr(t), n, _lib.RNG_EXPLICIT, _ptr(keep), 0, 0, 0, _ptr(out),
                                       _stream())
        else:
            rc = self.lib.sdrm_forward(self._h, _ptr(x), _ptr(t), n, _lib.RNG_PHILOX, None, int(seed), int(step),
                                       int(row0), _ptr(out), _stream())
        self._check(rc, "sdrm_forward")
        self._keepalive = (x, t, keep)
        return out

    def sample(self, n, nd=1.0, multires=False, xT=None, z=None, keep=None, Tj=None, seed=0, call_id=0, row0=0,
               return_Tj=False):
        out = torch.empty(n, self.L, dtype=torch.float32, device=self.device)
        tj_out = torch.zeros(n, dtype=torch.int64, device=self.device) if (multires and return_Tj) else None
        if xT is not None:
            xT, z, keep = self._dev(xT, torch.float32), self._dev(z, torch.float32), self._dev(keep, torch.uint8)
            Tj = None if Tj is None else self._dev(Tj, torch.int64)
            if tuple(z.shape) != (self.T + 1, n, self.L) or tuple(keep.shape) != (self.T + 1, n, self.L):
                raise SdrmError("sample: z and keep must be [T+1,n,L]")
            rc = self.lib.sdrm_sample(self._h, n, float(nd), int(bool(multires)), _lib.RNG_EXPLICIT, _ptr(xT), _ptr(z),
                                      _ptr(keep), _ptr(Tj), 0, 0, 0, _ptr(out), _ptr(tj_out), _stream())
        else:
            rc = self.lib.sdrm_sample(self._h, n, float(nd), int(bool(multires)), _lib.RNG_PHILOX, None, None, None,
                                      None, int(seed), int(call_id), int(row0), _ptr(out), _ptr(tj_out), _stream())
        self._check(rc, "sdrm_sample")
        self._keepalive = (xT, z, keep, Tj)
        return (out, tj_out) if return_Tj else out

    def sample_begin(self, n, nd=1.0, multires=False, seed=0, call_id=0, row0=0):
        self._check(self.lib.sdrm_sample_begin(self._h, int(n), float(nd), int(bool(multires)), _lib.RNG_PHILOX, None,
                                               None, None, None, int(seed), int(call_id), int(row0), None, _stream()),
                    "sdrm_sample_begin")
        self._sample_n = int(n)

    def sample_steps(self, count):
        self._check(self.lib.sdrm_sample_steps(self._h, int(count), _stream()), "sdrm_sample_steps")
        return int(self.lib.sdrm_sample_remaining(self._h))

    def sample_end(self):
        out = torch.empty(self._sample_n, self.L, dtype=torch.float32, device=self.device)
        self._check(self.lib.sdrm_sample_end(self._h, _ptr(out), _stream()), "sdrm_sample_end")
        return out

    def reverse_step(self, x, i, z, keep):
        x = self._dev(x, torch.float32).clone()
        z = None if z is None else self._dev(z, torch.float32)
        keep = self._dev(keep, torch.uint8)
        self._check(self.lib.sdrm_reverse_step(self._h, _ptr(x), x.shape[0], int(i), _ptr(z), _ptr(keep), _stream()),
                    "sdrm_reverse_step")
        self._keepalive = (z, keep)
        return x

    def equal_sparsity(self, raw, sparsity, return_threshold=False):
        raw = self._dev(raw, torch.float32)
        out = torch.empty(raw.shape, dtype=torch.uint8, device=self.device)
        thr = torch.empty((), dtype=torch.float32, device=self.device)
        self._check(self.lib.sdrm_equal_sparsity(self._h, _ptr(raw), raw.numel(), float(sparsity), _ptr(out), _ptr(thr),
                                                 _stream()), "sdrm_equal_sparsity")
        return (out, thr) if return_threshold else out

    def _decoder(self, w1, b1, w2, b2):
        w1, b1, w2, b2 = (self._dev(t.detach() if isinstance(t, torch.Tensor) else t, torch.float32) for t in (w1, b1, w2, b2))
        hidden, latent = w1.shape
# ... 83 lines not shown
```

Baseline: 9023 denoising-steps/s.

## Add segmented time-embedding gradient kernel and rebalance strip-owned wgrad scheduling

```diff
diff --git a/include/sdrm_hip_debug.h b/include/sdrm_hip_debug.h
--- a/include/sdrm_hip_debug.h
+++ b/include/sdrm_hip_debug.h
@@ -22,6 +22,7 @@
 int sdrm_debug_set_sample_persist(sdrm_engine* e, int mode);
 int sdrm_debug_split_skew(sdrm_engine* e, unsigned skew);
 int sdrm_debug_set_wgrad_strips(sdrm_engine* e, int on);
+int sdrm_debug_set_temb_seg(sdrm_engine* e, int on);
 int sdrm_debug_set_dgrad_rows(sdrm_engine* e, int mode);
 int sdrm_debug_rowchain_available(const sdrm_engine* e);
 int sdrm_debug_set_fused_reverse(sdrm_engine* e, int mode);
diff --git a/sdrm_amd/_lib.py b/sdrm_amd/_lib.py
--- a/sdrm_amd/_lib.py
+++ b/sdrm_amd/_lib.py
@@ -97,6 +97,7 @@
     "sdrm_debug_rowchain_available": (c_int, [c_void_p]),
     "sdrm_debug_set_wgrad_strips": (c_int, [c_void_p, c_int]),
     "sdrm_debug_set_dgrad_rows": (c_int, [c_void_p, c_int]),
+    "sdrm_debug_set_temb_seg": (c_int, [c_void_p, c_int]),
     "sdrm_debug_comm_handle": (c_void_p, [c_void_p]),
     "sdrm_debug_plan_wgrad": (c_int, [c_int, c_int, c_int, C.POINTER(c_int), C.POINTER(c_int)]),
     "sdrm_debug_gemm_time": (c_int, [c_int, c_int, c_int, c_int, c_int, c_int, C.POINTER(c_float), c_void_p]),
diff --git a/sdrm_amd/csrc/sdrm_hip.hip b/sdrm_amd/csrc/sdrm_hip.hip
--- a/sdrm_amd/csrc/sdrm_hip.hip
+++ b/sdrm_amd/csrc/sdrm_hip.hip
@@ -28,6 +28,7 @@
 #include "tail.h"
 #include "dgrad_rows.h"
 #include "wgrad2.h"
+#include "temb_seg.h"
 
 using namespace sdrm;
 
@@ -36,6 +37,7 @@
 constexpr int BM = 64;
 constexpr int S_MAX = 64;
 constexpr int LOSS_BLOCKS = 256;
+constexpr int CHIP_CUS = 256;
 
 inline int round_up(int v, int m) { return (v + m - 1) / m * m; }
 
@@ -56,6 +58,7 @@
   int ar_buckets = 1;
   int dgrad_rows = 1;
   int strips = 1;
+  int temb_seg = 0;
   int rows48 = 1;
   int rows48_share = 7;
   int smp_persist = 1;
@@ -94,6 +97,8 @@
   bool cur_act = false;
   int ones_col = -1;
   bool bwd_strips = false;
+  int bwd_seg_ranges = 0;
+  float *Mslab = nullptr;
   float *temb = nullptr, *tembP = nullptr, *B0tab = nullptr;
   float *sched = nullptr;
   float *Us = nullptr;
@@ -480,9 +485,26 @@
     e->prof_flops.push_back(flops);
     HIP_TRY(e, hipEventRecord(e->prof_ev[2 * slot], st));
   }
-  SDRM_LAUNCH(e, (k_wgrad_strips<NT>), dim3((unsigned)(a.units * a.slices)), dim3(NTHREADS), 0, st, a);
+  SDRM_LAUNCH(e, (k_wgrad_strips<NT>), dim3((unsigned)wg2_grid(a)), dim3(NTHREADS), 0, st, a);
   HIP_TRY(e, hipGetLastError());
   if (rec) HIP_TRY(e, hipEventRecord(e->prof_ev[2 * slot + 1], st));
+  return SDRM_OK;
+}
+
+bool use_temb_seg(const sdrm_engine* e) {
+  return e->cur_grouped && e->Mslab && e->tune.temb_seg > 0 && e->LP % 32 == 0 && e->LP / 32 >= WG2_MIN_KTILES;
+}
+
+int launch_temb_seg(sdrm_engine* e, hipStream_t st) {
+  SegArgs a{};
+  a.dpre = dpre_buf(e, 0); a.ld = e->WP; a.tdev = e->tdev; a.tembP = e->tembP; a.TP = e->TP; a.Mslab = e->Mslab; a.WP = e->WP;
+  a.B = e->cur_B; a.G = e->cur_rows / RC_ROWS; a.T = e->T;
+  static_assert(RC_ROWS == SEG_GROUP_ROWS && RC_USERS == SEG_GROUP_USERS, "k_temb_seg walks the row-owned forward's row groups");
+  int ranges = 0;
+  a.gpr = seg_plan(a.G, e->WP / SEG_COLS, CHIP_CUS, &ranges);
+  SDRM_LAUNCH(e, k_temb_seg, dim3((unsigned)(ranges * (e->WP / SEG_COLS))), dim3(SEG_THREADS), seg_lds_floats(e->T, e->TP) * sizeof(float), st, a);
+  HIP_TRY(e, hipGetLastError());
+  e->bwd_seg_ranges = ranges;
   return SDRM_OK;
 }
 
@@ -490,24 +512,25 @@
   const int H = e->H;
   Wg2Args a{};
   int ktiles[WG2_MAX_PROBLEMS], n = 0;
-  auto problem = [&](const float* A, int lda, const float* B, int ldb, float* slab, int kin, size_t slab_rows) {
-    a.p[n].A = A; a.p[n].lda = lda; a.p[n].B = B; a.p[n].ldb = ldb; a.p[n].slab = slab; a.p[n].ldc = kin;
-    a.p[n].slab_stride = slab_rows * (size_t)kin;
+  auto problem = [&](const float* A, int lda, const float* B, int ldb, float* slab, int ldc, int kin, size_t slab_rows) {
+    a.p[n].A = A; a.p[n].lda = lda; a.p[n].B = B; a.p[n].ldb = ldb; a.p[n].slab = slab; a.p[n].ldc = ldc;
+    a.p[n].slab_stride = slab_rows * (size_t)ldc;
     ktiles[n++] = kin / 32;
   };
   auto actk = [&](int k) { return e->act + (size_t)k * e->MPmax * e->WP; };
-  problem(dpre_buf(e, 0), e->WP, e->U, e->K0, e->slab0, e->K0, (size_t)e->WP);
-  problem(e->dY, e->LP, actk(H), e->WP, e->slabO, e->WP, (size_t)e->LP);
-  const int units = [&] { int t = e->K0 / 32 + (H + 1) * (e->WP / 32); return (t + 3) / 4; }();
-  int S = 256 / units;
-  if (S < 1) S = 1;
-  if (S > S_MAX) S = S_MAX;
+  const bool seg = use_temb_seg(e);
+  if (seg)
+    if (int rc = launch_temb_seg(e, st)) return rc;
+  problem(dpre_buf(e, 0), e->WP, e->U, e->K0, e->slab0, e->K0, seg ? e->LP : e->K0, (size_t)e->WP);
+  problem(e->dY, e->LP, actk(H), e->WP, e->slabO, e->WP, e->WP, (size_t)e->LP);
   MP = e->cur_rows;
+  const int nstrips = ktiles[0] + (H + 1) * (e->WP / 32);
+  const int S = wg2_slices(nstrips, MP, CHIP_CUS, S_MAX, e->tune.wgrad_slices);
   const int kchunk = round_up((MP + S - 1) / S, WG2_BK);
   const int slices = (MP + kchunk - 1) / kchunk;
   for (int k = H; k >= 1; --k)
-    problem(dpre_buf(e, k), e->WP, actk(k - 1), e->WP, e->slabH + (size_t)(k - 1) * slices * e->WP * e->WP, e->WP, (size_t)e->WP);
-  if (wg2_plan(ktiles, n, a) != units) return fail(e, SDRM_ERR_SHAPE, "strip-owned weight gradients: plan does not fit");
+    problem(dpre_buf(e, k), e->WP, actk(k - 1), e->WP, e->slabH + (size_t)(k - 1) * slices * e->WP * e->WP, e->WP, e->WP, (size_t)e->WP);
+  if (wg2_plan(ktiles, n, a) != nstrips) return fail(e, SDRM_ERR_SHAPE, "strip-owned weight gradients: plan does not fit");
   a.slices = slices; a.rows = MP; a.kchunk = kchunk;
   e->bwd_S0 = e->bwd_SH = e->bwd_SO = slices;
   e->bwd_strips = true;
@@ -1077,6 +1100,12 @@
 int sdrm_debug_set_wgrad_strips(sdrm_engine* e, int on) {
   if (!e) return SDRM_ERR_ARG;
   e->tune.strips = on ? 1 : 0;
+  return SDRM_OK;
+}
+
+int sdrm_debug_set_temb_seg(sdrm_engine* e, int on) {
+  if (!e) return SDRM_ERR_ARG;
+  e->tune.temb_seg = on ? 1 : 0;
   return SDRM_OK;
 }
 
@@ -1194,6 +1223,7 @@
   if (const char* env = std::getenv("SDRM_SAMPLE_PERSIST")) e->tune.smp_persist = std::atoi(env);
   if (const char* env = std::getenv("SDRM_ROWS48_SHARE")) e->tune.rows48_share = std::atoi(env);
   if (const char* env = std::getenv("SDRM_WGRAD_STRIPS")) e->tune.strips = std::atoi(env);
+  if (const char* env = std::getenv("SDRM_TEMB_SEG")) e->tune.temb_seg = std::atoi(env);
   if (const char* env = std::getenv("SDRM_DGRAD_ROWS")) e->tune.dgrad_rows = std::atoi(env);
   e->L = L; e->W = W; e->T = T; e->H = H; e->max_rows = max_rows; e->device = device_id;
   e->LP = round_up(L, 32); e->WP = round_up(W, 32); e->TP = round_up(T + 1, 32); e->K0 = e->LP + e->TP;
@@ -1298,6 +1328,10 @@
   }
   HIP_TRY(e, dalloc(&e->Mred, (size_t)W * e->TP)); HIP_TRY(e, dalloc(&e->snap, (size_t)T * T + T + (size_t)W * T));
   HIP_TRY(e, allow_full_lds((const void*)k_tail_emb));
+  if (seg_lds_floats(T, e->TP) * sizeof(float) <= (size_t)LDS_MAX_BYTES && e->WP <= 352) {
+    HIP_TRY(e, dalloc(&e->Mslab, (size_t)SEG_R_MAX * e->WP * e->TP));
+    HIP_TRY(e, allow_full_lds((const void*)k_temb_seg));
+  }
   HIP_TRY(e, dalloc(&e->tdev, max_rows)); HIP_TRY(e, dalloc(&e->Tj_dev, max_rows)); HIP_TRY(e, dalloc(&e->rowid_dev, max_rows));
   HIP_TRY(e, hipEventCreateWithFlags(&e->ev_fork, hipEventDisableTiming));
   HIP_TRY(e, hipEventCreateWithFlags(&e->ev_hold, hipEventDisableTiming));
@@ -1318,7 +1352,7 @@
   (void)hipSetDevice(e->device);
   void* bufs[] = {e->p, e->m, e->v, e->g, e->W0c, e->b0c, e->Whc, e->bhc, e->Woc, e->boc, e->temb, e->tembP, e->B0tab,
                   e->sched, e->U, e->pre, e->Y, e->dY, e->dA, e->X, e->slab0, e->slabH, e->slabO, e->db0s,
-                  e->dbHs, e->dbOs, e->alpha_part, e->loss_part, e->sums, e->Mred, e->snap, e->WeP, e->W0eP, e->tdev, e->Tj_dev, e->rowid_dev, e->rev_dev, e->Us, e->WhcT, e->WocT, e->sel, e->one_dev, e->feed_flag, e->smp_w, e->W0f, e->Whf, e->Wof, e->act, e->WhfT, e->WofT, e->smp_pre, e->smp_Y};
+                  e->dbHs, e->dbOs, e->alpha_part, e->loss_part, e->sums, e->Mred, e->Mslab, e->snap, e->WeP, e->W0eP, e->tdev, e->Tj_dev, e->rowid_dev, e->rev_dev, e->Us, e->WhcT, e->WocT, e->sel, e->one_dev, e->feed_flag, e->smp_w, e->W0f, e->Whf, e->Wof, e->act, e->WhfT, e->WofT, e->smp_pre, e->smp_Y};
   for (void* b : bufs)
     if (b) (void)hipFree(b);
   if (e->xcntF) (void)hipFree(e->xcntF);
@@ -1542,7 +1576,7 @@
 
 int backward_chain(sdrm_engine* e, const double* sums, float* loss, hipStream_t st, bool with_wgrad0) {
   const int B = e->cur_B, MP = e->cur_MP, H = e->H;
-  e->bwd_strips = false;
+  e->bwd_strips = false; e->bwd_seg_ranges = 0;
   SeedArgs sa{};
   sa.sums = e->fold_sums ? nullptr : (sums ? sums : e->sums); sa.Y = e->Y; sa.x0 = e->cur_x0; sa.dY = e->dY; sa.loss = loss;
   sa.B = B; sa.L = e->L; sa.LP = e->LP; sa.MP = MP; sa.grouped = (e->cur_sk || e->cur_g16) ? 2 : (e->cur_grouped ? 1 : 0);
@@ -1726,7 +1760,8 @@
     }
     vec(e->off_b0, W, e->slab0, e->K0, (size_t)e->WP * e->K0, e->db0s, (size_t)e->WP, S0, e->b0c);
     {
-      TailJob& j = mat(0, W, T, 0, e->slab0 + e->LP, e->K0, (size_t)e->WP * e->K0, S0);
+      TailJob& j = e->bwd_seg_ranges > 0 ? mat(0, W, T, 0, e->Mslab, e->TP, (size_t)e->WP * e->TP, e->bwd_seg_ranges)
+                                         : mat(0, W, T, 0, e->slab0 + e->LP, e->K0, (size_t)e->WP * e->K0, S0);
       j.red = e->Mred; j.red_ld = e->TP;
     }
     snap(e->off_we, 1, T * T + T, 0, e->snap, 0);
diff --git a/sdrm_amd/csrc/temb_seg.h b/sdrm_amd/csrc/temb_seg.h
--- /dev/null
+++ b/sdrm_amd/csrc/temb_seg.h
@@ -0,0 +1,143 @@
+#pragma once
+#include <hip/hip_runtime.h>
+#include <stdint.h>
+
+namespace sdrm {
+
+constexpr int SEG_THREADS = 256;
+constexpr int SEG_COLS = 32;
+constexpr int SEG_LANES = 8;
+constexpr int SEG_UPL = 4;
+constexpr int SEG_CH = 4;
+constexpr int SEG_GROUP_USERS = 32, SEG_GROUP_ROWS = 96;
+constexpr int SEG_R_MAX = 32;
+
+typedef float seg_f32x16 __attribute__((ext_vector_type(16)));
+static_assert(SEG_COLS == 32, "one 32-row MFMA tile of columns per work-group");
+
+struct SegArgs {
+  const float* dpre; int ld;
+  const int* tdev;
+  const float* tembP; int TP;
+  float* Mslab; int WP;
+  int B, G, T;
+  int gpr;
+};
+
+__host__ __device__ inline size_t seg_lds_floats(int T, int TP) {
+  return (size_t)SEG_LANES * (T + 1) * SEG_COLS + (size_t)(T + 1) * TP;
+}
+
+__global__ __launch_bounds__(SEG_THREADS, 1) void k_temb_seg(const SegArgs a) {
+  extern __shared__ __attribute__((aligned(16))) float ssh[];
+  const int tid = threadIdx.x, c = tid & (SEG_COLS - 1), k = tid >> 5;
+  const int nt = a.T + 1;
+  const int ncb = a.WP / SEG_COLS;
+  const int r = (int)blockIdx.x / ncb, cb = (int)blockIdx.x - r * ncb;
+  float* Sk = ssh + (size_t)k * nt * SEG_COLS + c;
+  float* tsh = ssh + (size_t)SEG_LANES * nt * SEG_COLS;
+
+  const int g_begin = r * a.gpr, g_end = min(g_begin + a.gpr, a.G);
+  const float* col = a.dpre + cb * SEG_COLS + c;
+  struct Set { float x[SEG_CH][SEG_UPL][3]; int t[SEG_CH][SEG_UPL]; int g0; };
+  Set s0, s1;
+  auto load = [&](Set& s, int g0) __attribute__((always_inline)) {
+#pragma unroll
+    for (int j = 0; j < SEG_CH; ++j)
+#pragma unroll
+      for (int u = 0; u < SEG_UPL; ++u) {
+        const int g = g0 + j, ug = k + SEG_LANES * u, usr = SEG_GROUP_USERS * g + ug;
+        const int gc = min(g, a.G - 1);
+        s.t[j][u] = a.tdev[min(usr, a.B - 1)];
+#pragma unroll
+        for (int p = 0; p < 3; ++p) s.x[j][u][p] = col[((size_t)SEG_GROUP_ROWS * gc + SEG_GROUP_USERS * p + ug) * a.ld];
+      }
+    s.g0 = g0;
+  };
+  auto add = [&](const Set& s) __attribute__((always_inline)) {
+#pragma unroll
+    for (int j = 0; j < SEG_CH; ++j) {
+      int t[SEG_UPL]; float d[SEG_UPL], o[SEG_UPL], v[SEG_UPL];
+#pragma unroll
+      for (int u = 0; u < SEG_UPL; ++u) {
+        const int g = s.g0 + j, usr = SEG_GROUP_USERS * g + k + SEG_LANES * u;
+        const bool ok = g < g_end && usr < a.B;
+        t[u] = ok ? min(max(s.t[j][u], 0), a.T) : 0;
+        d[u] = ok ? (s.x[j][u][0] + s.x[j][u][1]) + s.x[j][u][2] : 0.f;
+        o[u] = Sk[t[u] * SEG_COLS];
+      }
+#pragma unroll
+      for (int u = 0; u < SEG_UPL; ++u) {
+        float base = o[u];
+#pragma unroll
+        for (int q = 0; q < u; ++q)
+          if (t[q] == t[u]) base = v[q];
+        v[u] = base + d[u];
+      }
+#pragma unroll
+      for (int u = 0; u < SEG_UPL; ++u) Sk[t[u] * SEG_COLS] = v[u];
+    }
+  };
+  load(s0, g_begin);
+  for (int f0 = 0; f0 < nt * a.TP / 4; f0 += 8 * SEG_THREADS) {
+    float4 tv[8];
+#pragma unroll
+    for (int u = 0; u < 8; ++u) {
+      const int f = f0 + u * SEG_THREADS + tid;
+      tv[u] = f < nt * a.TP / 4 ? reinterpret_cast<const float4*>(a.tembP)[f] : make_float4(0.f, 0.f, 0.f, 0.f);
+    }
+#pragma unroll
+    for (int u = 0; u < 8; ++u) {
+      const int f = f0 + u * SEG_THREADS + tid;
+      if (f < nt * a.TP / 4) reinterpret_cast<float4*>(tsh)[f] = tv[u];
+    }
+  }
+  for (int f = tid; f < SEG_LANES * nt * SEG_COLS; f += SEG_THREADS) ssh[f] = 0.f;
+  __syncthreads();
+  for (int g0 = g_begin; g0 < g_end; g0 += 2 * SEG_CH) {
+    load(s1, g0 + SEG_CH);
+    add(s0);
+    load(s0, g0 + 2 * SEG_CH);
+    if (g0 + SEG_CH < g_end) add(s1);
+  }
+  __syncthreads();
+  for (int f = tid; f < nt * SEG_COLS; f += SEG_THREADS) {
+    float v = ssh[f];
+#pragma unroll
+    for (int q = 1; q < SEG_LANES; ++q) v += ssh[(size_t)q * nt * SEG_COLS + f];
+    ssh[f] = v;
+  }
+  __syncthreads();
+  const int lane = tid & 63, wave = tid >> 6, l31 = lane & 31, lhi = lane >> 5;
+  for (int tile = wave; tile < a.TP / 32; tile += SEG_THREADS / 64) {
+    seg_f32x16 acc;
+#pragma unroll
+    for (int r16 = 0; r16 < 16; ++r16) acc[r16] = 0.f;
+    for (int g0 = 0; g0 < (nt + 1) / 2; g0 += 4) {
+      float av[4], bv[4];
+#pragma unroll
+      for (int j = 0; j < 4; ++j) {
+        const int t = 2 * (g0 + j) + lhi;
+        av[j] = t < nt ? ssh[t * SEG_COLS + l31] : 0.f;
+        bv[j] = t < nt ? tsh[(size_t)t * a.TP + 32 * tile + l31] : 0.f;
+      }
+#pragma unroll
+      for (int j = 0; j < 4; ++j) acc = __builtin_amdgcn_mfma_f32_32x32x2f32(av[j], bv[j], acc, 0, 0, 0);
+    }
+    float* out = a.Mslab + ((size_t)r * a.WP + cb * SEG_COLS + 4 * lhi) * a.TP + 32 * tile + l31;
+#pragma unroll
+    for (int r16 = 0; r16 < 16; ++r16) out[(size_t)((r16 & 3) + 8 * (r16 >> 2)) * a.TP] = acc[r16];
+  }
+}
+
+inline int seg_plan(int G, int ncb, int cus, int* ranges) {
+  int R = cus / (ncb > 0 ? ncb : 1);
+  if (R > SEG_R_MAX) R = SEG_R_MAX;
+  if (R > G) R = G;
+  if (R < 1) R = 1;
+  const int gpr = (G + R - 1) / R;
+  *ranges = (G + gpr - 1) / gpr;
+  return gpr;
+}
+
+}
diff --git a/sdrm_amd/csrc/wgrad2.h b/sdrm_amd/csrc/wgrad2.h
--- a/sdrm_amd/csrc/wgrad2.h
+++ b/sdrm_amd/csrc/wgrad2.h
@@ -4,31 +4,13 @@
 
 #include "bufres.h"
 #include "gemm.h"
+#include "wgrad2_plan.h"
 
 #ifndef WG2_DIAG
 #define WG2_DIAG 0
 #endif
 
 namespace sdrm {
-
-constexpr int WG2_MAX_PROBLEMS = 8;
-constexpr int WG2_MAX_UNITS = 32;
-constexpr int WG2_BK = 16;
-
-struct Wg2Problem {
-  const float* A; int lda;
-  const float* B; int ldb;
-  float* slab; int ldc;
-  size_t slab_stride;
-};
-
-struct Wg2Strip { int8_t problem; int8_t ktile; };
-
-struct Wg2Args {
-  Wg2Problem p[WG2_MAX_PROBLEMS];
-  Wg2Strip strip[WG2_MAX_UNITS][4];
-  int units, slices, rows, kchunk;
-};
 
 __device__ __forceinline__ Wg2Problem wg2_problem(const Wg2Args& a, int idx) {
   Wg2Problem r = a.p[0];
@@ -43,7 +25,7 @@
   static constexpr int WP = 32 * NT, LDA = WP + 4, LDB = 32 + 4;
   static constexpr int A_TILE = WG2_BK * LDA, B_TILE = WG2_BK * LDB;
   static constexpr int STAGE = 2 * A_TILE + 4 * B_TILE;
-  static constexpr size_t LDS_BYTES = 2 * (size_t)STAGE * 4;
+  static constexpr size_t LDS_BYTES = (2 * (size_t)STAGE + B_TILE) * 4;
   static constexpr int NA4 = WG2_BK * WP / 4, NB4 = 4 * WG2_BK * 32 / 4;
   static constexpr int NLA = (NA4 + NTHREADS - 1) / NTHREADS, NLB = NB4 / NTHREADS;
   static_assert(NLB == 2, "two B blocks per half work-group");
@@ -54,41 +36,54 @@
 __global__ __launch_bounds__(NTHREADS, 1) void k_wgrad_strips(const Wg2Args a) {
   typedef Wg2Cfg<NT> C;
   constexpr int WP = C::WP, LDA = C::LDA, LDB = C::LDB, BK = WG2_BK;
-  __shared__ __attribute__((aligned(16))) float smem[2 * C::STAGE];
+  __shared__ __attribute__((aligned(16))) float smem[2 * C::STAGE + C::B_TILE];
   const int tid = threadIdx.x, lane = tid & 63;
   const int wave = __builtin_amdgcn_readfirstlane(tid >> 6);
   const int l31 = lane & 31, lhi = lane >> 5;
-  const int logical = xcd_remap((int)blockIdx.x, a.units * a.slices);
-  const int slice = logical / a.units, unit = logical - slice * a.units;
-  const int m_begin = slice * a.kchunk, m_end = min(m_begin + a.kchunk, a.rows);
-  const int nt = (m_end - m_begin) / BK;
-
-  const Wg2Strip st = a.strip[unit][wave];
-  const int pa = a.strip[unit][0].problem;
-  int pb = pa;
-#pragma unroll
-  for (int w = 1; w < 4; ++w)
-    if (a.strip[unit][w].problem >= 0) pb = a.strip[unit][w].problem;
-  const bool two = pb != pa;
-  const int ai = (st.problem == pa || st.problem < 0) ? 0 : 1;
-  const bool active = st.problem >= 0;
+  const int npairs = a.nstrips * a.slices;
+  const int logical = xcd_remap((int)blockIdx.x, (npairs + 3) >> 2);
+  const int q0 = 4 * logical, wl = min(3, npairs - 1 - q0);
+  const int slice_a = q0 / a.nstrips, i0 = q0 - slice_a * a.nstrips;
+  auto pair_wrap = [&](int w) __attribute__((always_inline)) { return i0 + w >= a.nstrips; };
+  auto pair_slice = [&](int w) __attribute__((always_inline)) { return slice_a + (pair_wrap(w) ? 1 : 0); };
+  auto pair_strip = [&](int w) __attribute__((always_inline)) { return a.strip[i0 + w - (pair_wrap(w) ? a.nstrips : 0)]; };
+  const int slice_b = pair_slice(wl);
+  const Wg2Strip st_a = pair_strip(0), st_b = pair_strip(wl);
+  const bool active = wave <= wl;
+  const int ww = active ? wave : 0;
+  const int slice = pair_slice(ww);
+  const Wg2Strip st = pair_strip(ww);
+  const int pa = st_a.problem, pb = st_b.problem;
+  const bool two = pb != pa || slice_b != slice_a;
+  const int ai = (st.problem == pa && slice == slice_a) ? 0 : 1;
+  auto slice_steps = [&](int s) __attribute__((always_inline)) { return (min(s * a.kchunk + a.kchunk, a.rows) - s * a.kchunk) / BK; };
+  const int m_begin_a = slice_a * a.kchunk, m_begin_b = slice_b * a.kchunk;
+  const int nt_a = slice_steps(slice_a), nt_b = slice_steps(slice_b);
+  const int nt = max(nt_a, nt_b);
+  const int nt_w = ai ? nt_b : nt_a;
 
   constexpr int QA = WP / 4;
   const Wg2Problem Pa = wg2_problem(a, pa), Pb = wg2_problem(a, pb);
   const int lda_a = Pa.lda, lda_b = Pb.lda;
-  auto span = [&](int ld, int skip) __attribute__((always_inline)) {
+  auto span = [&](int m_begin, int ld, int skip) __attribute__((always_inline)) {
     const size_t b = ((size_t)(a.rows - m_begin) * (size_t)ld - (size_t)skip) * 4;
     return (uint32_t)(b < 0xffffffffull ? b : 0xffffffffull);
   };
-  const brsrc Ra = make_brsrc(Pa.A + (size_t)m_begin * lda_a, span(lda_a, 0)), Rb = make_brsrc(Pb.A + (size_t)m_begin * lda_b, span(lda_b, 0));
-  brsrc RB0, RB1; int Bld[2];
+  const brsrc Ra = make_brsrc(Pa.A + (size_t)m_begin_a * lda_a, span(m_begin_a, lda_a, 0));
+  const brsrc Rb = make_brsrc(Pb.A + (size_t)m_begin_b * lda_b, span(m_begin_b, lda_b, 0));
+  brsrc RB0, RB1; int Bld[2]; bool Bsl[2];
   {
-    const Wg2Strip s0 = a.strip[unit][(wave >> 1)], s1 = a.strip[unit][(wave >> 1) + 2];
-    const Wg2Problem P0 = wg2_problem(a, s0.problem < 0 ? pa : s0.problem), P1 = wg2_problem(a, s1.problem < 0 ? pa : s1.problem);
+    const int j0 = wave >> 1, j1 = j0 + 2;
+    const int g0 = j0 <= wl ? j0 : 0, g1 = j1 <= wl ? j1 : 0;
+    const int sl0 = pair_slice(g0), sl1 = pair_slice(g1);
+    const Wg2Strip s0 = pair_strip(g0), s1 = pair_strip(g1);
+    const Wg2Problem P0 = wg2_problem(a, s0.problem), P1 = wg2_problem(a, s1.problem);
     Bld[0] = P0.ldb; Bld[1] = P1.ldb;
-    const int c0 = 32 * (s0.problem < 0 ? 0 : s0.ktile), c1 = 32 * (s1.problem < 0 ? 0 : s1.ktile);
-    RB0 = make_brsrc(P0.B + (size_t)m_begin * P0.ldb + c0, span(P0.ldb, c0));
-    RB1 = make_brsrc(P1.B + (size_t)m_begin * P1.ldb + c1, span(P1.ldb, c1));
+    Bsl[0] = sl0 != slice_a; Bsl[1] = sl1 != slice_a;
+    const int c0 = 32 * s0.ktile, c1 = 32 * s1.ktile;
+    const int mb0 = sl0 * a.kchunk, mb1 = sl1 * a.kchunk;
+    RB0 = make_brsrc(P0.B + (size_t)mb0 * P0.ldb + c0, span(mb0, P0.ldb, c0));
+    RB1 = make_brsrc(P1.B + (size_t)mb1 * P1.ldb + c1, span(mb1, P1.ldb, c1));
   }
   struct RSet { float4 a[C::NLA], a2[C::NLA], b[C::NLB]; };
   RSet r0, r1, r2;
@@ -115,13 +110,14 @@
 #pragma unroll
   for (int j = 0; j < 2; ++j) voB[j] = (uint32_t)((rowB * Bld[j] + 4 * quadB) * 4);
   auto as4 = [](f32x4_b v) __attribute__((always_inline)) { return make_float4(v[0], v[1], v[2], v[3]); };
-  auto gload_piece = [&](auto two_tag, RSet& r, int m0, int k) __attribute__((always_inline)) {
+  auto gload_piece = [&](auto two_tag, RSet& r, int step, int k) __attribute__((always_inline)) {
     constexpr bool TWO = decltype(two_tag)::value;
     constexpr int NA = TWO ? 2 * C::NLA : C::NLA;
-    if (k < C::NLA) r.a[k] = as4(bload4(Ra, voA[k], (uint32_t)((m0 - m_begin) * lda_a) * 4u));
-    else if (TWO && k < NA) r.a2[k - C::NLA] = as4(bload4(Rb, voA2[k - C::NLA], (uint32_t)((m0 - m_begin) * lda_b) * 4u));
-    else if (k == NA) r.b[0] = as4(bload4(RB0, voB[0], (uint32_t)((m0 - m_begin) * Bld[0]) * 4u));
-    else if (k == NA + 1) r.b[1] = as4(bload4(RB1, voB[1], (uint32_t)((m0 - m_begin) * Bld[1]) * 4u));
+    const int ra = min(step, nt_a - 1) * BK, rb = TWO ? min(step, nt_b - 1) * BK : ra;
+    if (k < C::NLA) r.a[k] = as4(bload4(Ra, voA[k], (uint32_t)(ra * lda_a) * 4u));
+    else if (TWO && k < NA) r.a2[k - C::NLA] = as4(bload4(Rb, voA2[k - C::NLA], (uint32_t)(rb * lda_b) * 4u));
+    else if (k == NA) r.b[0] = as4(bload4(RB0, voB[0], (uint32_t)((TWO && Bsl[0] ? rb : ra) * Bld[0]) * 4u));
+    else if (k == NA + 1) r.b[1] = as4(bload4(RB1, voB[1], (uint32_t)((TWO && Bsl[1] ? rb : ra) * Bld[1]) * 4u));
   };
   auto lstore_piece = [&](auto two_tag, const RSet& r, float* S, int k) __attribute__((always_inline)) {
     constexpr bool TWO = decltype(two_tag)::value;
@@ -133,9 +129,8 @@
   };
   auto gload = [&](auto two_tag, RSet& r, int step) __attribute__((always_inline)) {
     constexpr int NPC = (decltype(two_tag)::value ? 2 * C::NLA : C::NLA) + C::NLB;
-    const int m0 = m_begin + min(step, nt - 1) * BK;
-#pragma unroll
-    for (int k = 0; k < NPC; ++k) gload_piece(two_tag, r, m0, k);
+#pragma unroll
+    for (int k = 0; k < NPC; ++k) gload_piece(two_tag, r, step, k);
   };
   auto lstore = [&](auto two_tag, const RSet& r, int stage) __attribute__((always_inline)) {
     constexpr int NPC = (decltype(two_tag)::value ? 2 * C::NLA : C::NLA) + C::NLB;
@@ -151,6 +146,7 @@
 
   const int aoff = ai * C::A_TILE + lhi * LDA + l31;
   const int boff = 2 * C::A_TILE + wave * C::B_TILE + lhi * LDB + l31;
+  const int zoff = 2 * C::STAGE + lhi * LDB + l31;
 
   auto kstep = [&](auto two_tag, int i, RSet& nx) __attribute__((always_inline)) {
     constexpr int NPC = (decltype(two_tag)::value ? 2 * C::NLA : C::NLA) + C::NLB;
@@ -159,11 +155,11 @@
     static_assert(NPC <= HALF, "more staging pieces than MFMA slots");
     const float* S = smem + (i & 1) * C::STAGE;
     float* Sn = smem + ((i + 1) & 1) * C::STAGE;
-    const int m4 = m_begin + min(i + 4, nt - 1) * BK;
+    const float* SB = (decltype(two_tag)::value && i >= nt_w) ? smem + zoff : S + boff;
     float fa0[NT], fa1[NT], fb0 = 0.f, fb1 = 0.f;
 #pragma unroll
     for (int t = 0; t < NT; ++t) fa0[t] = S[aoff + 32 * t];
-    fb0 = S[boff];
+    fb0 = SB[0];
 #pragma unroll
     for (int g = 0; g < BK / 2; ++g) {
       float (&ca)[NT] = (g & 1) ? fa1 : fa0;
@@ -174,7 +170,7 @@
       for (int t = 0; t < NT; ++t) {
         if (!(WG2_DIAG & 1)) acc[t] = __builtin_amdgcn_mfma_f32_32x32x2f32(ca[t], cb, acc[t], 0, 0, 0);
         if (g + 1 < BK / 2 && !(WG2_DIAG & 8)) {
-          if (t == 0) nb = S[boff + 2 * (g + 1) * LDB];
+          if (t == 0) nb = SB[2 * (g + 1) * LDB];
           na[t] = S[aoff + 2 * (g + 1) * LDA + 32 * t];
         }
         const int slot = g * NT + t;
@@ -182,7 +178,7 @@
           if (slot % STRIDE == 0 && slot / STRIDE < NPC && !(WG2_DIAG & 2)) lstore_piece(two_tag, nx, Sn, slot / STRIDE);
         } else {
           const int s2 = slot - HALF;
-          if (s2 % STRIDE == 0 && s2 / STRIDE < NPC && !(WG2_DIAG & 4)) gload_piece(two_tag, nx, m4, s2 / STRIDE);
+          if (s2 % STRIDE == 0 && s2 / STRIDE < NPC && !(WG2_DIAG & 4)) gload_piece(two_tag, nx, i + 4, s2 / STRIDE);
         }
         __builtin_amdgcn_sched_barrier(0);
       }
@@ -193,6 +189,8 @@
     gload(two_tag, r0, 0);
     lstore(two_tag, r0, 0);
     gload(two_tag, r1, 1); gload(two_tag, r2, 2); gload(two_tag, r0, 3);
+    if (decltype(two_tag)::value)
+      for (int f = tid; f < C::B_TILE; f += NTHREADS) smem[2 * C::STAGE + f] = 0.f;
     __syncthreads();
     int i = 0;
     for (; i + 2 < nt; i += 3) {
@@ -200,8 +198,10 @@
       kstep(two_tag, i + 1, r2);
       kstep(two_tag, i + 2, r0);
     }
-    if (i < nt) kstep(two_tag, i, r1);
-    if (i + 1 < nt) kstep(two_tag, i + 1, r2);
+    if (i < nt) {
+      kstep(two_tag, i, r1);
+      if (i + 1 < nt) kstep(two_tag, i + 1, r2);
+    }
   };
   if (nt > 0) {
     if (two) run(std::true_type{});
@@ -217,20 +217,4 @@
     for (int r = 0; r < 16; ++r) dst[(size_t)(32 * t + (r & 3) + 8 * (r >> 2)) * P.ldc] = acc[t][r];
 }
 
-inline int wg2_plan(const int* ktiles, int nproblems, Wg2Args& a) {
-  int n = 0;
-  for (int p = 0; p < nproblems; ++p) n += ktiles[p];
-  const int units = (n + 3) / 4;
-  if (nproblems > WG2_MAX_PROBLEMS || units > WG2_MAX_UNITS) return 0;
-  int u = 0, w = 0;
-  for (int p = 0; p < nproblems; ++p)
-    for (int k = 0; k < ktiles[p]; ++k) {
-      a.strip[u][w].problem = (int8_t)p; a.strip[u][w].ktile = (int8_t)k;
-      if (++w == 4) { w = 0; ++u; }
-    }
-  for (; w > 0 && w < 4; ++w) { a.strip[u][w].problem = -1; a.strip[u][w].ktile = 0; }
-  a.units = units;
-  return units;
 }
-
-}
diff --git a/sdrm_amd/csrc/wgrad2_plan.h b/sdrm_amd/csrc/wgrad2_plan.h
--- /dev/null
+++ b/sdrm_amd/csrc/wgrad2_plan.h
@@ -0,0 +1,54 @@
+#pragma once
+#include <stddef.h>
+#include <stdint.h>
+
+namespace sdrm {
+
+constexpr int WG2_MAX_PROBLEMS = 8;
+constexpr int WG2_MAX_STRIPS = 128;
+constexpr int WG2_MIN_KTILES = 3;
+constexpr int WG2_BK = 16;
+
+struct Wg2Problem {
+  const float* A; int lda;
+  const float* B; int ldb;
+  float* slab; int ldc;
+  size_t slab_stride;
+};
+
+struct Wg2Strip { int8_t problem; int8_t ktile; };
+
+struct Wg2Args {
+  Wg2Problem p[WG2_MAX_PROBLEMS];
+  Wg2Strip strip[WG2_MAX_STRIPS];
+  int nstrips, slices, rows, kchunk;
+};
+
+inline int wg2_plan(const int* ktiles, int nproblems, Wg2Args& a) {
+  int n = 0;
+  for (int p = 0; p < nproblems; ++p) {
+    if (ktiles[p] < WG2_MIN_KTILES) return 0;
+    n += ktiles[p];
+  }
+  if (nproblems > WG2_MAX_PROBLEMS || n > WG2_MAX_STRIPS || n <= 4) return 0;
+  int i = 0;
+  for (int p = 0; p < nproblems; ++p)
+    for (int k = 0; k < ktiles[p]; ++k) { a.strip[i].problem = (int8_t)p; a.strip[i].ktile = (int8_t)k; ++i; }
+  a.nstrips = n;
+  return n;
+}
+
+inline int wg2_slices(int nstrips, int rows, int cus, int smax, int forced) {
+  int S = forced > 0 ? forced : (4 * cus) / nstrips;
+  if (S > smax) S = smax;
+  if (S > rows / WG2_BK) S = rows / WG2_BK;
+  return S < 1 ? 1 : S;
+}
+inline int wg2_grid(const Wg2Args& a) { return (a.nstrips * a.slices + 3) / 4; }
+
+inline int wg2_logical(int id, int n) {
+  const int q = n >> 3, r = n & 7, x = id & 7, s = id >> 3;
+  return (x < r ? x * (q + 1) : r * (q + 1) + (x - r) * q) + s;
+}
+
+}
diff --git a/sdrm_amd/engine.py b/sdrm_amd/engine.py
--- a/sdrm_amd/engine.py
+++ b/sdrm_amd/engine.py
@@ -92,7 +92,10 @@
         return t.contiguous()
 
     def debug_set(self, tile=None, skinny=None, fused_reverse=None, chains=None, nt32_rows=None, nt32_rows_train=None,
-                  gradient_buckets=None, rowchain=None, wgrad_strips=None, dgrad_rows=None, rows48=None, rows48_split=None, sample_persist=None, rows48_share=None):
+                  gradient_buckets=None, rowchain=None, wgrad_strips=None, dgrad_rows=None, rows48=None, rows48_split=None, sample_persist=None, rows48_share=None,
+                  temb_seg=None):
+        if temb_seg is not None:
+            self._check(self.lib.sdrm_debug_set_temb_seg(self._h, int(bool(temb_seg))), "sdrm_debug_set_temb_seg")
         if rowchain is not None:
             self._check(self.lib.sdrm_debug_set_rowchain(self._h, int(rowchain)), "sdrm_debug_set_rowchain")
         if rows48_share is not None:
```

Result: no change. 8999 denoising-steps/s (median of 3 runs) (-0.3%).
